# ttanida/rgrg

Measured on AMD Instinct MI355X. Metric: images/sec full 29-region report gen, 512x512 CXR, greedy max_len=128, higher is better.
Workload: dtype bf16; 1 GPU; full_model.generate() batch=32/GPU, 29 regions, greedy max_len=128, bf16 autocast: 16-bit detector, 16-bit decode GEMMs + K/V cache, hipGraph-captured decode step (BASELINE configs[2]); global_batch=32, parallelism=single GPU, weights=seeded random init (rgrg_amd.synth, profile bench), hipGraph_decode=True

## Files before the change

include/rgrg_hip.h:

```cpp
#ifndef RGRG_HIP_H_
#define RGRG_HIP_H_

#include <stdint.h>

#ifdef __cplusplus
extern "C" {
#endif

#define RGRG_OK 0
#define RGRG_EINVAL (-1)
#define RGRG_EHIP (-2)
#define RGRG_ESTATE (-3)

#define RGRG_ACT_NONE 0
#define RGRG_ACT_RELU 1
#define RGRG_ACT_GELU_NEW 2

const char* rgrg_last_error(void);
int rgrg_abi_version(void);
int rgrg_device_arch(int dev, char* buf, int buflen);

int rgrg_linear_f32(const float* A, const float* W, const float* scale, const float* shift, const float* R,
                    float* Y, int M, int N, int K, int ldy, int act, int splitk, float* ws, void* stream);
int rgrg_conv2d_nhwc_f32(const float* X, const float* W, const float* scale, const float* shift, const float* R,
// ... 30 lines not shown
typedef struct rgrg_decoder_layer_weights {
    const float *ln1_g, *ln1_b, *ln2_g, *ln2_b;
    const float *c_attn_w, *c_attn_b;
    const float *attn_proj_w, *attn_proj_b;
    const float *c_fc_w, *c_fc_b;
    const float *mlp_proj_w, *mlp_proj_b;
} rgrg_decoder_layer_weights;

typedef struct rgrg_decoder_weights {
    int n_layer, d_model, n_head, vocab;
    const float* wte;
    const float *lnf_g, *lnf_b;
    const float *fst0_w, *fst0_b, *fst2_w, *fst2_b;
    const float *ukv_w, *ukv_b;
    const rgrg_decoder_layer_weights* layers;
} rgrg_decoder_weights;

typedef struct rgrg_decoder rgrg_decoder;

int rgrg_decoder_create(const rgrg_decoder_weights* w, int max_seqs, int max_len, rgrg_decoder** out);
int rgrg_decoder_create_with_cache(const rgrg_decoder_weights* w, int max_seqs, int max_len, void* kv_cache, size_t kv_cache_bytes,
                                   rgrg_decoder** out);
size_t rgrg_decoder_kv_cache_bytes(int n_layer, int max_seqs, int max_len);
void rgrg_decoder_destroy(rgrg_decoder* d);
int rgrg_decoder_generate(rgrg_decoder* d, const float* feats, int S, int max_length, int64_t* out_ids,
                          int out_ld, int* out_len, int use_graph, void* stream);
int rgrg_decoder_sample(rgrg_decoder* d, const float* feats, int S, int max_length, float temperature, int top_k, float top_p,
                        uint64_t seed, int64_t* out_ids, int out_ld, float* out_logprobs, int* out_len, int use_graph,
                        void* stream);
int rgrg_sample_logits_f32(const float* logits, int64_t ld, int S, int V, float temperature, int top_k, float top_p,
                           uint64_t seed, int step, int row0, int* out_tok, float* out_logprob, void* stream);
int rgrg_decoder_beam_search(rgrg_decoder* d, const float* feats, int S, int num_beams, int max_length,
                             int early_stopping, float length_penalty, int num_return_sequences, int64_t* out_ids,
                             int out_ld, int* out_len, void* stream);
int rgrg_decoder_set_precision(rgrg_decoder* d, int mode);
int rgrg_decoder_set_kv_format(rgrg_decoder* d, int fmt);
int rgrg_decoder_kv_format_in_use(rgrg_decoder* d, int rows);
int rgrg_decoder_set_lm_positions(rgrg_decoder* d, const int64_t* pos, int64_t n);
int rgrg_decoder_lm_forward(rgrg_decoder* d, const float* feats, const int64_t* input_ids, const float* attention_mask,
                            int S, int T, float* logits_out, float* loss_out, void* stream);
int rgrg_decoder_lm_loss_grad(rgrg_decoder* d, const float* feats, const int64_t* input_ids, const float* attention_mask,
                              int S, int T, float loss_scale, float dropout_p, uint64_t dropout_seed, float* loss_out,
                              float* grad_ukv_w, float* grad_ukv_b, float* grad_fst0_w, float* grad_fst0_b, float* grad_fst2_w,
                              float* grad_fst2_b, void* stream);
int rgrg_decoder_time_train_gemms(rgrg_decoder* d, int S, int T, int iters, float* ms_per_step, double* flops_per_step,
                                  int* launches_per_step);
int rgrg_dropout_mask_f32(uint64_t seed, uint32_t stream_id, float p, int64_t n, int row_len, float* out, void* stream);
int rgrg_decoder_forward_cached(rgrg_decoder* d, const float* feats, const int64_t* input_ids, const int64_t* position_ids,
                                const float* attention_mask,
                                int S, int T, int past_len, float* logits_out, void* stream);
int rgrg_decoder_cache_plane(rgrg_decoder* d, int layer, int kv, void** ptr, int* max_seqs, int* slots, int* is_bf16);
int rgrg_decoder_take_id_error(rgrg_decoder* d, int* pending);
int rgrg_decoder_refresh_trainable(rgrg_decoder* d, void* stream);
int rgrg_transpose_pad_f32(const float* src, float* dst, int rows, int cols, int rows_padded, void* stream);
int rgrg_colsum_f32(const float* src, float* out, int rows, int cols, void* stream);
int rgrg_relu_backward_f32(float* d, const float* h, int64_t n, void* stream);
int rgrg_bce_with_logits_masked_backward_f32(const float* logits, const uint8_t* mask, const uint8_t* target, float pos_weight,
                                             int n, float scale, float* dlogits, int ld, void* stream);
int rgrg_adamw_step_f32(float* param, const float* grad, float* exp_avg, float* exp_avg_sq, int64_t n, float lr, float beta1,
                        float beta2, float eps, float weight_decay, int step, float grad_scale, void* stream);
int rgrg_adamw_multi_step_f32(const void* items, int n_items, float lr, float beta1, float beta2, float eps,
                              float weight_decay, int step, float grad_scale, void* stream);
int rgrg_f32_to_bf16(const float* src, uint16_t* dst, int64_t n, int fp16, void* stream);
int rgrg_bf16_to_f32(const uint16_t* src, float* dst, int64_t n, int fp16, void* stream);
int rgrg_conv2d_nhwc_bf16(const uint16_t* X16, const uint16_t* Wb, const float* shift, const uint16_t* R16, float* Y,
                          uint16_t* Y16, int B, int H, int Wd, int Cin, int Cout, int KH, int KW, int stride, int pad,
                          int act, int fp16, void* stream);
int rgrg_linear_bf16w_f32(const float* A, const uint16_t* Wb, const float* shift, const float* R, float* Y, int M,
                          int N, int K, int ldy, int act, int fp16, void* stream);
int rgrg_linear_bf16_f32(const uint16_t* A16, const uint16_t* Wb, const float* shift, const float* R, float* Y,
                         uint16_t* Y16, int M, int N, int K, int ldy, int act, int fp16, void* stream);
int rgrg_debug_linear_bf16_tile(const uint16_t* A16, const uint16_t* Wb, const float* shift, const float* R, float* Y,
                                int M, int N, int K, int ldy, int act, int tile, int lda, int ldw, int fp16, void* stream);
int rgrg_debug_linear_bf16_train(const uint16_t* A16, const uint16_t* Wb, const float* shift, const float* R, float* Y,
                                 uint16_t* Y16, uint16_t* Ypre16, const uint16_t* G16, int M, int N, int K, int ldy, int act,
                                 int tile, int fp16, void* stream);
int rgrg_debug_linear_bf16_argmax(const uint16_t* A16, const uint16_t* Wb, const float* shift, int M, int N, int K,
                                  float* cand_val, int* cand_idx, int fp16, void* stream);
int rgrg_debug_ln_fold16(const float* w, const float* gain, const float* beta, const float* bias, uint16_t* wb, float* colsum,
                         float* shift, int N, int K, int fp16, void* stream);
int rgrg_debug_linear_bf16_ln(const uint16_t* A16, const uint16_t* Wb, const float* shift, const float* R, float* Y,
                              uint16_t* Yb16, float* stats_out, const float* ln_stats, const float* ln_colsum, int M, int N,
                              int K, int ldy, int act, int fp16, void* stream);
int rgrg_debug_linear_bf16_ln_kp(const uint16_t* A16, const uint16_t* Wb, const float* shift, const float* R, float* Y,
                                 uint16_t* Y16, uint16_t* Yb16, float* stats_out, const float* ln_stats, const float* ln_colsum,
                                 int M, int N, int K, int ldy, int act, int fp16, int kp, void* stream);
int rgrg_debug_attn_decode(const float* qkv, int ld_qkv, void* kcache, void* vcache, const int* step_dev, float* out,
                           uint16_t* out16, int S, int H, int T_slots, const int* src, const float* kmask, int kv16, int fp16,
                           int ni, int frag_out, int max_workgroups, void* stream);
int rgrg_debug_attn_decode_kv8(const float* qkv, int ld_qkv, uint8_t* kcache, uint8_t* vcache, const int* step_dev, float* out,
                               uint16_t* out16, int S, int H, int T_slots, const int* src, const float* kmask, int fp16,
                               int max_workgroups, void* stream);
int rgrg_debug_attn_prefill(const float* qkv, const float* ukv, int ld_ukv, int kcol, const float* am, float* out, uint16_t* out16,
                            float* lse, int S, int H, int T, int variant, uint64_t seed, uint32_t stream_id, float p, int fp16,
                            void* stream);
int rgrg_debug_attn_backward_f32(const float* qkv, const float* ukv, int ld_ukv, int kcol, const float* am, const float* d_att,
                                 const float* att, const float* lse, float* delta, float* d_qkv, float* d_ukv, uint16_t* d_qkv16,
                                 int S, int H, int T, uint64_t seed, uint32_t stream_id, float p, int fp16, float ukv_scale,
                                 void* stream);
int rgrg_debug_attn_train16(int backward, const uint16_t* qkv16, const uint16_t* ukv16, int ld_ukv, int kcol, const float* am,
                            uint16_t* att16, float* lse, const uint16_t* d_att16, uint16_t* d_qkv16, float* d_ukv, int S, int H,
                            int T, uint64_t seed, uint32_t stream_id, float p, float ukv_scale, int fp16, void* stream);
int rgrg_box_match_f32(const float* gt, const int* gt_count, int G, const float* boxes, int64_t box_image_stride,
                       const int* box_count, int B, int N, float high, float low, int allow_low_quality, int* matched,
                       int* ws_best_per_gt, void* stream);
int rgrg_balanced_sample(const int* matched, const int64_t* gt_labels, int G, const int* box_count, const float* keys,
                         uint64_t seed, int stage, int B, int n, int batch, int max_pos, uint32_t* ws_keys, uint8_t* mask,
                         int* list, int* count, void* stream);
int rgrg_rpn_loss_sampled_f32(const float* rpn_out, int ld, int anchors_per_cell, const int* matched, const float* gt, int G,
                              const float* anchors, const uint8_t* mask, const int* list, const int* count, int B, int A,
                              int batch, float* out2, void* stream);
int rgrg_roi_add_gt_f32(const float* props, const int* counts, int P, const float* gt, const int* gt_count, int G, int B,
                        float* boxes, int* box_count, void* stream);
int rgrg_roi_gather_samples_f32(const float* boxes, const int* matched, const float* gt, const int64_t* gt_labels,
                                const int* gt_count, int G, const int* list, const int* count, int B, int N, int K, float wx,
                                float wy, float ww, float wh, float* props_s, int* offsets, int64_t* labels_flat,
                                float* reg_targets, void* stream);
int rgrg_fastrcnn_loss_f32(const float* pred, int ld, int num_classes, const int64_t* labels, const float* reg_targets, int N,
                           float* out2, void* stream);

int rgrg_decoder_copy_last_logits(rgrg_decoder* d, float* dst, int S, void* stream);
int rgrg_decoder_time_step_parts(rgrg_decoder* d, int S, int nkeys, int iters, int one_range, float* ms_gemm, float* ms_attn,
                                 double* gemm_flops, double* gemm_weight_bytes, double* kv_bytes, int* gemm_launches);
int rgrg_decoder_trace_step(rgrg_decoder* d, int S, int nkeys, int iters, float* recs, int max_recs, int* n_out);
int rgrg_decoder_attention_only(rgrg_decoder* d, int S, int nkeys, int iters, void* stream);
int rgrg_decoder_row_limit(rgrg_decoder* d);
int rgrg_debug_chain(int n, int mode, int blocks, float* us_per_kernel);

#ifdef __cplusplus
}
#endif
#endif
```

rgrg_amd/_hip.py:

```python
from __future__ import annotations

import ctypes as C
import os
from typing import Optional

from . import build as _build

c_float_p = C.c_void_p
_i, _f, _p = C.c_int, C.c_float, C.c_void_p

ACT_NONE, ACT_RELU, ACT_GELU_NEW = 0, 1, 2
ABI_VERSION = 24


class RgrgHipError(RuntimeError):
    pass


class DecoderLayerWeights(C.Structure):
    _fields_ = [(n, _p) for n in ("ln1_g", "ln1_b", "ln2_g", "ln2_b", "c_attn_w", "c_attn_b", "attn_proj_w",
                                  "attn_proj_b", "c_fc_w", "c_fc_b", "mlp_proj_w", "mlp_proj_b")]


class DecoderWeights(C.Structure):
    _fields_ = [("n_layer", _i), ("d_model", _i), ("n_head", _i), ("vocab", _i), ("wte", _p), ("lnf_g", _p),
                ("lnf_b", _p), ("fst0_w", _p), ("fst0_b", _p), ("fst2_w", _p), ("fst2_b", _p), ("ukv_w", _p),
                ("ukv_b", _p), ("layers", C.POINTER(DecoderLayerWeights))]


SIGNATURES = {
    "rgrg_last_error": (C.c_char_p, []),
    "rgrg_abi_version": (_i, []),
    "rgrg_device_arch": (_i, [_i, C.c_char_p, _i]),
    "rgrg_linear_f32": (_i, [_p, _p, _p, _p, _p, _p, _i, _i, _i, _i, _i, _i, _p, _p]),
    "rgrg_conv2d_nhwc_f32": (_i, [_p, _p, _p, _p, _p, _p, _i, _i, _i, _i, _i, _i, _i, _i, _i, _i, _i, _p, _p]),
    "rgrg_stem_conv7x7_f32": (_i, [_p, _p, _p, _p, _p, _i, _i, _i, _p]),
    "rgrg_maxpool3x3s2_nhwc_f32": (_i, [_p, _p, _i, _i, _i, _i, _p]),
    "rgrg_rpn_proposals_f32": (_i, [_p, _p, _p, _p, _p, _i, _i, _i, _i, _i, _f, _f, _f, _f, _p]),
    "rgrg_roi_align_avgpool_f32": (_i, [_p, _p, _p, _p, _p, _i, _i, _i, _i, _i, _i, _f, _p]),
    "rgrg_roi_align_avgpool_bf16maps": (_i, [_p, _p, _p, _p, _p, _i, _i, _i, _i, _i, _i, _f, _i, _p]),
    "rgrg_top1_per_class_f32": (_i, [_p, _i, _p, _p, _p, _p, _p, _p, _p, _i, _i, _i, _f, _f, _p]),
    "rgrg_select_regions_f32": (_i, [_p, _p, _f, _p, _p, _p, _i, _p]),
    "rgrg_bce_with_logits_masked_f32": (_i, [_p, _p, _p, C.c_float, _i, _p, _p]),
    "rgrg_preprocess_u8_f32": (_i, [_p, _i, _i, _i, _i, _i, C.c_float, C.c_float, _p, _p]),
    "rgrg_gather_rows_f32": (_i, [_p, _p, _p, _i, _i, _p]),
    "rgrg_decoder_create": (_i, [C.POINTER(DecoderWeights), _i, _i, C.POINTER(_p)]),
    "rgrg_decoder_create_with_cache": (_i, [C.POINTER(DecoderWeights), _i, _i, _p, C.c_size_t, C.POINTER(_p)]),
    "rgrg_decoder_kv_cache_bytes": (C.c_size_t, [_i, _i, _i]),
    "rgrg_decoder_destroy": (None, [_p]),
    "rgrg_decoder_generate": (_i, [_p, _p, _i, _i, _p, _i, C.POINTER(_i), _i, _p]),
    "rgrg_decoder_sample": (_i, [_p, _p, _i, _i, _f, _i, _f, C.c_uint64, _p, _i, _p, C.POINTER(_i), _i, _p]),
    "rgrg_sample_logits_f32": (_i, [_p, C.c_int64, _i, _i, _f, _i, _f, C.c_uint64, _i, _i, _p, _p, _p]),
    "rgrg_decoder_beam_search": (_i, [_p, _p, _i, _i, _i, _i, _f, _i, _p, _i, C.POINTER(_i), _p]),
    "rgrg_decoder_set_precision": (_i, [_p, _i]),
    "rgrg_decoder_set_kv_format": (_i, [_p, _i]),
    "rgrg_decoder_kv_format_in_use": (_i, [_p, _i]),
    "rgrg_decoder_lm_forward": (_i, [_p, _p, _p, _p, _i, _i, _p, _p, _p]),
    "rgrg_decoder_lm_loss_grad": (_i, [_p, _p, _p, _p, _i, _i, C.c_float, C.c_float, C.c_uint64, _p, _p, _p, _p, _p, _p, _p, _p]),
    "rgrg_dropout_mask_f32": (_i, [C.c_uint64, C.c_uint32, C.c_float, C.c_int64, _i, _p, _p]),
    "rgrg_decoder_refresh_trainable": (_i, [_p, _p]),
    "rgrg_decoder_take_id_error": (_i, [_p, C.POINTER(_i)]),
    "rgrg_decoder_forward_cached": (_i, [_p, _p, _p, _p, _p, _i, _i, _i, _p, _p]),
    "rgrg_decoder_cache_plane": (_i, [_p, _i, _i, C.POINTER(C.c_void_p), C.POINTER(_i), C.POINTER(_i), C.POINTER(_i)]),
    "rgrg_transpose_pad_f32": (_i, [_p, _p, _i, _i, _i, _p]),
    "rgrg_colsum_f32": (_i, [_p, _p, _i, _i, _p]),
    "rgrg_relu_backward_f32": (_i, [_p, _p, C.c_int64, _p]),
    "rgrg_bce_with_logits_masked_backward_f32": (_i, [_p, _p, _p, C.c_float, _i, C.c_float, _p, _i, _p]),
    "rgrg_adamw_step_f32": (_i, [_p, _p, _p, _p, C.c_int64, C.c_float, C.c_float, C.c_float, C.c_float, C.c_float, _i, C.c_float, _p]),
    "rgrg_adamw_multi_step_f32": (_i, [_p, _i, C.c_float, C.c_float, C.c_float, C.c_float, C.c_float, _i, C.c_float, _p]),
    "rgrg_f32_to_bf16": (_i, [_p, _p, C.c_int64, _i, _p]),
    "rgrg_bf16_to_f32": (_i, [_p, _p, C.c_int64, _i, _p]),
    "rgrg_conv2d_nhwc_bf16": (_i, [_p, _p, _p, _p, _p, _p, _i, _i, _i, _i, _i, _i, _i, _i, _i, _i, _i, _p]),
    "rgrg_linear_bf16w_f32": (_i, [_p, _p, _p, _p, _p, _i, _i, _i, _i, _i, _i, _p]),
    "rgrg_linear_bf16_f32": (_i, [_p, _p, _p, _p, _p, _p, _i, _i, _i, _i, _i, _i, _p]),
    "rgrg_debug_linear_bf16_tile": (_i, [_p, _p, _p, _p, _p, _i, _i, _i, _i, _i, _i, _i, _i, _i, _p]),
    "rgrg_debug_linear_bf16_train": (_i, [_p, _p, _p, _p, _p, _p, _p, _p, _i, _i, _i, _i, _i, _i, _i, _p]),
    "rgrg_debug_linear_bf16_argmax": (_i, [_p, _p, _p, _i, _i, _i, _p, _p, _i, _p]),
    "rgrg_debug_ln_fold16": (_i, [_p, _p, _p, _p, _p, _p, _p, _i, _i, _i, _p]),
    "rgrg_debug_linear_bf16_ln": (_i, [_p, _p, _p, _p, _p, _p, _p, _p, _p, _i, _i, _i, _i, _i, _i, _p]),
    "rgrg_debug_linear_bf16_ln_kp": (_i, [_p, _p, _p, _p, _p, _p, _p, _p, _p, _p, _i, _i, _i, _i, _i, _i, _i, _p]),
    "rgrg_debug_attn_decode": (_i, [_p, _i, _p, _p, _p, _p, _p, _i, _i, _i, _p, _p, _i, _i, _i, _i, _i, _p]),
    "rgrg_debug_attn_decode_kv8": (_i, [_p, _i, _p, _p, _p, _p, _p, _i, _i, _i, _p, _p, _i, _i, _p]),
    "rgrg_debug_attn_prefill": (_i, [_p, _p, _i, _i, _p, _p, _p, _p, _i, _i, _i, _i, C.c_uint64, C.c_uint32, _f, _i, _p]),
    "rgrg_debug_attn_backward_f32": (_i, [_p, _p, _i, _i, _p, _p, _p, _p, _p, _p, _p, _p, _i, _i, _i, C.c_uint64, C.c_uint32, _f,
                                          _i, _f, _p]),
    "rgrg_debug_attn_train16": (_i, [_i, _p, _p, _i, _i, _p, _p, _p, _p, _p, _p, _i, _i, _i, C.c_uint64, C.c_uint32, _f, _f, _i, _p]),
    "rgrg_decoder_copy_last_logits": (_i, [_p, _p, _i, _p]),
    "rgrg_box_match_f32": (_i, [_p, _p, _i, _p, C.c_int64, _p, _i, _i, _f, _f, _i, _p, _p, _p]),
    "rgrg_balanced_sample": (_i, [_p, _p, _i, _p, _p, C.c_uint64, _i, _i, _i, _i, _i, _p, _p, _p, _p, _p]),
    "rgrg_rpn_loss_sampled_f32": (_i, [_p, _i, _i, _p, _p, _i, _p, _p, _p, _p, _i, _i, _i, _p, _p]),
    "rgrg_roi_add_gt_f32": (_i, [_p, _p, _i, _p, _p, _i, _i, _p, _p, _p]),
    "rgrg_roi_gather_samples_f32": (_i, [_p, _p, _p, _p, _p, _i, _p, _p, _i, _i, _i, _f, _f, _f, _f, _p, _p, _p, _p, _p]),
    "rgrg_fastrcnn_loss_f32": (_i, [_p, _i, _i, _p, _p, _i, _p, _p]),
    "rgrg_decoder_trace_step": (_i, [_p, _i, _i, _i, _p, _i, C.POINTER(_i)]),
    "rgrg_decoder_attention_only": (_i, [_p, _i, _i, _i, _p]),
    "rgrg_decoder_row_limit": (_i, [_p]),
    "rgrg_decoder_set_lm_positions": (_i, [_p, _p, C.c_int64]),
    "rgrg_decoder_time_step_parts": (_i, [_p, _i, _i, _i, _i, C.POINTER(_f), C.POINTER(_f), C.POINTER(C.c_double),
                                          C.POINTER(C.c_double), C.POINTER(C.c_double), C.POINTER(_i)]),
    "rgrg_decoder_time_train_gemms": (_i, [_p, _i, _i, _i, C.POINTER(_f), C.POINTER(C.c_double), C.POINTER(_i)]),
    "rgrg_debug_chain": (_i, [_i, _i, _i, C.POINTER(_f)]),
}

_lib: Optional[C.CDLL] = None


def library_path() -> str:
    return _build.LIB_PATH


def load() -> C.CDLL:
    global _lib
    if _lib is not None:
        return _lib
    path = library_path()
    if _build.is_stale():
        try:
            _build.build_library()
        except Exception as e:
            if not os.path.exists(path):
                raise RgrgHipError(f"librgrg_hip.so is missing and could not be built: {e}") from e
    try:
        lib = C.CDLL(path)
    except OSError as e:
        raise RgrgHipError(f"cannot load {path}: {e} (the RGRG HIP path has no CPU fallback)") from e
    for name, (res, args) in SIGNATURES.items():
        fn = getattr(lib, name)
        fn.restype = res
        fn.argtypes = args
    got = lib.rgrg_abi_version()
    if got != ABI_VERSION:
        raise RgrgHipError(f"{path} has ABI version {got}, this package expects {ABI_VERSION}: rebuild it "
                           "(python -m rgrg_amd.build)")
    _lib = lib
    return lib


def autocast_mode() -> int:
    import torch
    if not torch.is_autocast_enabled("cuda"):
        return 0
    dt = torch.get_autocast_dtype("cuda")
    return 1 if dt == torch.bfloat16 else (2 if dt == torch.float16 else 0)


def check(rc: int, what: str = "") -> None:
    if rc != 0:
        msg = load().rgrg_last_error()
        raise RgrgHipError(f"{what} failed (code {rc}): {msg.decode() if msg else '?'}")


def ptr(t) -> Optional[int]:
    if t is None:
        return None
    assert t.is_contiguous(), "rgrg_hip expects dense tensors"
    return t.data_ptr()
```

rgrg_amd/csrc/decoder.hip:

```cpp
#include <math.h>
#include <stdlib.h>

#include <algorithm>
#include <type_traits>
#include <cmath>
#include <vector>

#include "decoder_internal.h"

namespace rgrg {

int skinny_max_rows() {
    static int v = -1;
    if (v < 0) { const char* e = getenv("RGRG_SKINNY_MAX_ROWS"); v = e ? atoi(e) : SKINNY_MAX_ROWS;
        if (v > SKINNY_MAX_ROWS) v = SKINNY_MAX_ROWS; if (v < 32) v = 32; }
    return v;
}

__global__ __launch_bounds__(256) void pack_weights_kernel(const float* __restrict__ W, float* __restrict__ P, int N,
                                                           int K, int NT) {
    const size_t total = (size_t)NT * (K / 8) * 64;
    for (size_t o = (size_t)blockIdx.x * blockDim.x + threadIdx.x; o < total; o += (size_t)gridDim.x * blockDim.x) {
        const int l = (int)(o & 63);
        const size_t t = o >> 6;
// ... 363 lines not shown
    __shared__ float pm[16], pl[16];
    __shared__ __attribute__((aligned(16))) float pacc[16][64];
    const int lane = threadIdx.x & 63, wave = threadIdx.x >> 6;
    const int s = blockIdx.x / H, hd = blockIdx.x - s * H;
    const int t = *step, nkeys = t + 2, slot = t + 1;
    const int g = lane >> 4, d4 = lane & 15;
    const float* row = qkv + (size_t)s * ld_qkv;
    const int D = H * 64;
    const int* srow = HAS_SRC ? src + (size_t)s * T : nullptr;
    constexpr int ATT_CHUNK = 16 * ATT_NI;
    const f32x4 q4 = *reinterpret_cast<const f32x4*>(row + hd * 64 + d4 * 4);
    const f32x4 k4 = *reinterpret_cast<const f32x4*>(row + D + hd * 64 + d4 * 4);
    const f32x4 v4 = *reinterpret_cast<const f32x4*>(row + 2 * D + hd * 64 + d4 * 4);
    float m = -INFINITY, l = 0.f;
    f32x4 acc = {0.f, 0.f, 0.f, 0.f};
#define ATT_CHUNK_CALL(NI_, BASE_) attn_chunk<HAS_SRC, NI_, HAS_MASK>(kc, vc, srow, s, hd, H, T, BASE_, nkeys, slot, wave, g, d4, q4, k4, v4, m, l, acc, kmask)
    if constexpr (ATT_NI == 9) {
        int base = 0;
        for (; nkeys - base > ATT_CHUNK; base += ATT_CHUNK) ATT_CHUNK_CALL(9, base);
        switch ((nkeys - base + 15) >> 4) {
            case 1: ATT_CHUNK_CALL(1, base); break;
            case 2: ATT_CHUNK_CALL(2, base); break;
            case 3: ATT_CHUNK_CALL(3, base); break;
            case 4: ATT_CHUNK_CALL(4, base); break;
            case 5: ATT_CHUNK_CALL(5, base); break;
            case 6: ATT_CHUNK_CALL(6, base); break;
            case 7: ATT_CHUNK_CALL(7, base); break;
            case 8: ATT_CHUNK_CALL(8, base); break;
            default: ATT_CHUNK_CALL(9, base); break;
        }
    } else {
        for (int base = 0; base < nkeys; base += ATT_CHUNK) ATT_CHUNK_CALL(ATT_NI, base);
    }
#undef ATT_CHUNK_CALL
    if (wave == 0 && g == 0) {
        *reinterpret_cast<f32x4*>(kc + (((size_t)s * H + hd) * T + slot) * 64 + d4 * 4) = k4;
        *reinterpret_cast<f32x4*>(vc + (((size_t)s * H + hd) * T + slot) * 64 + d4 * 4) = v4;
    }
    const int grp = wave * 4 + g;
    if (d4 == 0) { pm[grp] = m; pl[grp] = l; }
    *reinterpret_cast<f32x4*>(&pacc[grp][d4 * 4]) = acc;
    __syncthreads();
    if (threadIdx.x < 64) {
        float M = pm[0];
#pragma unroll
        for (int k = 1; k < 16; ++k) M = fmaxf(M, pm[k]);
        float L = 0.f, o = 0.f;
#pragma unroll
        for (int k = 0; k < 16; ++k) {
            const float wgt = expf(pm[k] - M);
            L += pl[k] * wgt;
            o += pacc[k][threadIdx.x] * wgt;
        }
        out[frag_out ? frag_off(s, hd * 64 + threadIdx.x, D) : (size_t)s * D + hd * 64 + threadIdx.x] = o / L;
    }
}

typedef unsigned short u16;
typedef unsigned int u32x4 __attribute__((ext_vector_type(4)));
template <bool F16>
__device__ __forceinline__ float pair_lo(unsigned u) {
    if constexpr (F16) return f16_bits_to_f32(u & 0xffffu);
    else return __uint_as_float(u << 16);
}
template <bool F16>
__device__ __forceinline__ float pair_hi(unsigned u) {
    if constexpr (F16) return f16_bits_to_f32(u >> 16);
    else return __uint_as_float(u & 0xffff0000u);
}

struct Kv16Row {
    f32x4 q0, q1, k0, k1, v0, v1;
};
template <bool F16>
__device__ __forceinline__ u32x4 kv16_pack_round(const f32x4& lo, const f32x4& hi) {
    u32x4 o;
    o[0] = to16<F16>(lo[0]) | (to16<F16>(lo[1]) << 16);
    o[1] = to16<F16>(lo[2]) | (to16<F16>(lo[3]) << 16);
    o[2] = to16<F16>(hi[0]) | (to16<F16>(hi[1]) << 16);
    o[3] = to16<F16>(hi[2]) | (to16<F16>(hi[3]) << 16);
    return o;
}

template <int NI, bool HAS_SRC, bool FIRST, bool F16>
__device__ __forceinline__ void kv16_wave_chunk(const __amdgpu_buffer_rsrc_t kc, const __amdgpu_buffer_rsrc_t vc, const int* __restrict__ srow,
                                                int s, int hd, int H, int T, int base, int nkeys, int slot, int g, int d8,
                                                Kv16Row& r, float (&q)[8], u32x4& kn16, u32x4& vn16, float& m, float& l, float (&acc)[8]) {
    int rowi[NI];
#pragma unroll
    for (int i = 0; i < NI; ++i) rowi[i] = HAS_SRC ? srow[min(base + i * 8 + g, nkeys - 1)] : s;
    u32x4 kk[NI], vv[NI];
#pragma unroll
    for (int i = 0; i < NI; ++i) {
        const int jc = min(base + i * 8 + g, nkeys - 1);
        const unsigned off = ((unsigned)((rowi[i] * H + hd) * T + jc) * 64u + (unsigned)d8 * 8u) * 2u;
        kk[i] = __builtin_bit_cast(u32x4, __builtin_amdgcn_raw_buffer_load_b128(kc, (int)off, 0, 2));
        vv[i] = __builtin_bit_cast(u32x4, __builtin_amdgcn_raw_buffer_load_b128(vc, (int)off, 0, 2));
    }
    __builtin_amdgcn_sched_barrier(0);
    if constexpr (FIRST) {
#pragma unroll
        for (int e = 0; e < 4; ++e)
            asm volatile("" : "+v"(r.q0[e]), "+v"(r.q1[e]), "+v"(r.k0[e]), "+v"(r.k1[e]), "+v"(r.v0[e]), "+v"(r.v1[e]));
#pragma unroll
        for (int e = 0; e < 4; ++e) { q[e] = r.q0[e]; q[4 + e] = r.q1[e]; }
        kn16 = kv16_pack_round<F16>(r.k0, r.k1);
        vn16 = kv16_pack_round<F16>(r.v0, r.v1);
    }
    float sc[NI];
    float cmax = -INFINITY;
#pragma unroll
    for (int i = 0; i < NI; ++i) {
        const int j = base + i * 8 + g;
        if (j == slot) { kk[i] = kn16; vv[i] = vn16; }
        float dot = 0.f;
#pragma unroll
        for (int e = 0; e < 4; ++e)
            dot += q[2 * e] * pair_lo<F16>(kk[i][e]) + q[2 * e + 1] * pair_hi<F16>(kk[i][e]);
        dot += dpp_get<0xB1, 0xf>(dot);
        dot += dpp_get<0x4E, 0xf>(dot);
        dot += dpp_get<0x141, 0xf>(dot);
        sc[i] = j < nkeys ? dot / 8.0f : -INFINITY;
        cmax = fmaxf(cmax, sc[i]);
    }
    const float m_new = fmaxf(m, cmax);
    const float scale = (m == -INFINITY) ? 0.f : expf(m - m_new);
    const bool any = m_new != -INFINITY;
    l *= scale;
#pragma unroll
    for (int e = 0; e < 8; ++e) acc[e] *= scale;
#pragma unroll
    for (int i = 0; i < NI; ++i) {
        const int j = base + i * 8 + g;
        const float pj = (j < nkeys && any) ? expf(sc[i] - m_new) : 0.f;
        l += pj;
#pragma unroll
        for (int e = 0; e < 4; ++e) {
            const unsigned u = j < nkeys ? vv[i][e] : 0u;
            acc[2 * e] += pj * pair_lo<F16>(u);
            acc[2 * e + 1] += pj * pair_hi<F16>(u);
        }
    }
    m = m_new;
}

template <bool HAS_SRC, bool F16>
__global__ __launch_bounds__(256) void attn_decode_kv16_wave_kernel(const float* __restrict__ qkv, int ld_qkv,
                                                                    u16* __restrict__ kc, u16* __restrict__ vc,
                                                                    const int* __restrict__ step, float* __restrict__ out,
                                                                    int S, int H, int T, const int* __restrict__ src,
                                                                    u16* __restrict__ out16) {
    const int lane = threadIdx.x & 63;
    const int t = *step, nkeys = t + 2, slot = t + 1;
    const int g = lane >> 3, d8 = lane & 7;
    const int D = H * 64;
    const __amdgpu_buffer_rsrc_t rk = dx_rsrc(kc), rv = dx_rsrc(vc);
    for (int item = blockIdx.x * 4 + (threadIdx.x >> 6); item < S * H; item += gridDim.x * 4) {
    const int s = item / H, hd = item - s * H;
    const float* row = qkv + (size_t)s * ld_qkv;
    const int* srow = HAS_SRC ? src + (size_t)s * T : nullptr;
    Kv16Row r;
    r.q0 = *reinterpret_cast<const f32x4*>(row + hd * 64 + d8 * 8);
    r.q1 = *reinterpret_cast<const f32x4*>(row + hd * 64 + d8 * 8 + 4);
    r.k0 = *reinterpret_cast<const f32x4*>(row + D + hd * 64 + d8 * 8);
    r.k1 = *reinterpret_cast<const f32x4*>(row + D + hd * 64 + d8 * 8 + 4);
    r.v0 = *reinterpret_cast<const f32x4*>(row + 2 * D + hd * 64 + d8 * 8);
    r.v1 = *reinterpret_cast<const f32x4*>(row + 2 * D + hd * 64 + d8 * 8 + 4);
    float m = -INFINITY, l = 0.f, acc[8], q[8];
    u32x4 kn16, vn16;
#pragma unroll
    for (int e = 0; e < 8; ++e) acc[e] = 0.f;
#define KV16_CHUNK(NI_, FIRST_, BASE_) \
    kv16_wave_chunk<NI_, HAS_SRC, FIRST_, F16>(rk, rv, srow, s, hd, H, T, BASE_, nkeys, slot, g, d8, r, q, kn16, vn16, m, l, acc)
#define KV16_TAIL(FIRST_, BASE_, REM_)                                                                   \
    switch (((REM_) + 7) >> 3) {                                                                         \
        case 1: KV16_CHUNK(1, FIRST_, BASE_); break;                                                     \
        case 2: KV16_CHUNK(2, FIRST_, BASE_); break;                                                     \
        case 3: KV16_CHUNK(3, FIRST_, BASE_); break;                                                     \
        case 4: KV16_CHUNK(4, FIRST_, BASE_); break;                                                     \
        case 5: KV16_CHUNK(5, FIRST_, BASE_); break;                                                     \
        case 6: KV16_CHUNK(6, FIRST_, BASE_); break;                                                     \
        case 7: KV16_CHUNK(7, FIRST_, BASE_); break;                                                     \
        case 8: KV16_CHUNK(8, FIRST_, BASE_); break;                                                     \
        default: KV16_CHUNK(9, FIRST_, BASE_); break;                                                    \
    }
    if (nkeys > 72) {
        KV16_CHUNK(9, true, 0);
        int base = 72;
        for (; nkeys - base > 72; base += 72) KV16_CHUNK(9, false, base);
        KV16_TAIL(false, base, nkeys - base)
    } else {
        KV16_TAIL(true, 0, nkeys)
    }
#undef KV16_TAIL
#undef KV16_CHUNK
    if (g == 0) {
        const size_t o = (((size_t)s * H + hd) * T + slot) * 64 + d8 * 8;
        *reinterpret_cast<u32x4*>(kc + o) = kn16;
        *reinterpret_cast<u32x4*>(vc + o) = vn16;
    }
    float M = fmaxf(m, dpp_get<0x128, 0xf>(m));
    M = fmaxf(M, __shfl_xor(M, 16, 64));
    M = fmaxf(M, __shfl_xor(M, 32, 64));
    const float wgt = (m == -INFINITY) ? 0.f : expf(m - M);
    l *= wgt;
    l += dpp_get<0x128, 0xf>(l);
    l += __shfl_xor(l, 16, 64);
    l += __shfl_xor(l, 32, 64);
#pragma unroll
    for (int e = 0; e < 8; ++e) {
        float o = acc[e] * wgt;
        o += dpp_get<0x128, 0xf>(o);
        o += __shfl_xor(o, 16, 64);
        o += __shfl_xor(o, 32, 64);
        acc[e] = o / l;
    }
    if (g == 0) {
        const size_t o = (size_t)s * D + hd * 64 + d8 * 8;
        if (out16) {
            u32x4 pk;
#pragma unroll
            for (int i = 0; i < 4; ++i) pk[i] = to16<F16>(acc[2 * i]) | (to16<F16>(acc[2 * i + 1]) << 16);
            *reinterpret_cast<u32x4*>(out16 + o) = pk;
        } else {
            *reinterpret_cast<f32x4*>(out + o) = f32x4{acc[0], acc[1], acc[2], acc[3]};
            *reinterpret_cast<f32x4*>(out + o + 4) = f32x4{acc[4], acc[5], acc[6], acc[7]};
        }
    }
    }
}

template <typename KV>
__global__ __launch_bounds__(256) void kv_slot0_kernel(const float* __restrict__ ukv, int ld, KV* __restrict__ kv_all,
                                                       size_t layer_stride, size_t kv_stride, int S, int H, int T,
                                                       int L, int row_mul, int f16) {
    const int D = H * 64;
    const size_t total = (size_t)L * 2 * S * D;
    for (size_t i = (size_t)blockIdx.x * blockDim.x + threadIdx.x; i < total; i += (size_t)gridDim.x * blockDim.x) {
        const int d = (int)(i % D);
        size_t r = i / D;
        const int s = (int)(r % S);
        r /= S;
        const int kv = (int)(r & 1), l = (int)(r >> 1);
        const int hd = d >> 6, e = d & 63;
        const float val = ukv[(size_t)s * ld + ((size_t)l * 2 + kv) * D + d];
        const size_t o = (size_t)l * layer_stride + (size_t)kv * kv_stride + (((size_t)s * row_mul * H + hd) * T) * 64 + e;
        if constexpr (sizeof(KV) == 1) kv_all[o] = (KV)f32_to_e4m3_bits(val);
        else if constexpr (sizeof(KV) == 2) kv_all[o] = (KV)to16_rt(val, f16);
        else kv_all[o] = val;
    }
}

constexpr int ARGMAX_U = 13;
__global__ __launch_bounds__(256) void argmax_update_kernel(const float* __restrict__ cand_val, const int* __restrict__ cand_idx,
                                                            int NT, long long* __restrict__ ids, int ld_ids,
                                                            int* __restrict__ finished, int* __restrict__ step,
                                                            int* __restrict__ done_len, int* __restrict__ sync, int S) {
    __shared__ float bv[4];
    __shared__ int bi[4];
    const int row = blockIdx.x, tid = threadIdx.x, lane = tid & 63, wave = tid >> 6;
    const int t = *step;
    const float* cv = cand_val + (size_t)row * NT;
    const int* cx = cand_idx + (size_t)row * NT;
    float v[ARGMAX_U];
    int ci[ARGMAX_U];
#pragma unroll
    for (int u = 0; u < ARGMAX_U; ++u) {
        const int i = min(tid + 256 * u, NT - 1);
        v[u] = cv[i];
        ci[u] = cx[i];
    }
    float best = -INFINITY;
    int idx = 0x7fffffff;
#pragma unroll
    for (int u = 0; u < ARGMAX_U; ++u)
        if (tid + 256 * u < NT && (v[u] > best || (v[u] == best && ci[u] < idx))) { best = v[u]; idx = ci[u]; }
    for (int i = tid + 256 * ARGMAX_U; i < NT; i += 256) {
        const float w = cv[i];
        const int wi = cx[i];
        if (w > best || (w == best && wi < idx)) { best = w; idx = wi; }
    }
    for (int o = 32; o > 0; o >>= 1) {
// ... 174 lines not shown
    return n > skinny_max_rows() ? skinny_max_rows() : n;
}
static int decode_row_limit(const rgrg_decoder* d) { return d->bf16_gemms ? skinny_max_rows16(d->w16_fused) : skinny_max_rows(); }
static bool kv_is_bf16(const rgrg_decoder* d, int rows) { return d->bf16_gemms && rows > decode_row_limit(d); }
static KvFormat kv_format(const rgrg_decoder* d, int rows) {
    if (!kv_is_bf16(d, rows)) return KV_F32;
    return d->kv8 ? KV_E4M3 : (d->f16() ? KV_F16 : KV_BF16);
}

int linear(rgrg_decoder* d, const Lin& l, const float* X, const float* R, float* Y, int M, int ldy, int act,
           bool count, const unsigned short* X16, unsigned short* Y16, const GemmLnFold* ln) {
    if (M <= skinny_max_rows() && l.packed && !l.direct) {
        SkinnyArgs a{X, l.packed, l.b, R, Y, d->part, M, l.K, l.N, l.NT, l.KS, ldy, act};
        int rc = launch_skinny_any(a, d->stream);
        if (rc) return rc;
        if (l.KS > 1) {
            const int total = M * l.N;
            hipLaunchKernelGGL(skinny_reduce_kernel, dim3((total + 255) / 256), dim3(256), 0, d->stream, a);
            RGRG_LAUNCH_CHECK();
        }
        if (count) {
            d->gemm_bytes_per_step += (size_t)l.N * l.K * sizeof(float);
            d->gemm_flops_per_step += 2.0 * M * l.N * l.K;
            d->gemm_launches_per_step += 1;
        }
        return RGRG_OK;
    }
    if (count) {
        d->gemm_flops_per_step += 2.0 * M * l.N * l.K;
        d->gemm_launches_per_step += 1;
    }
    if (d->bf16_gemms && l.wb && l.K % 256 == 0) {
        if (count) d->gemm_bytes_per_step += (size_t)l.N * l.K * 2;
        if (ln && ln->ln_colsum) {
            if (!l.wb_ln || !X16) { set_error("decoder: folded LayerNorm weights missing"); return RGRG_EINVAL; }
            GemmLnFold f = *ln;
            f.ln_colsum = l.cs16;
            f.kp = (d->kp_gemms == 1 || d->kp_gemms == 3) ? 1 : 0;
            return launch_gemm_bf16w_ex(nullptr, X16, l.wb_ln, l.c2_16, R, Y16 ? nullptr : Y, Y16, M, l.N, l.K, ldy, act, d->stream, d->f16(), &f);
        }
        if (ln && ln->Yb16 && d->sk_ws && M <= d->rows) {
            int ks = l.K >= 2048 ? d->sk_mlp : d->sk_attn;
            if (ks < 0) ks = (d->step_rows > 0 && d->step_rows <= 256) ? (l.K >= 2048 ? 4 : 2) : 1;
            if (ks > 1) {
                GemmLnFold f = *ln;
                const size_t r0 = d->xn16 ? (size_t)(reinterpret_cast<const unsigned short*>(ln->Yb16) - d->xn16) / (size_t)d->D : 0;
                const size_t tile0 = (r0 / 64) * (size_t)(l.N / 64);
                f.ksplit = ks; f.sk_ws = d->sk_ws + tile0 * 4 * 4096; f.sk_cnt = d->sk_cnt + tile0;
                return launch_gemm_bf16w_ex(nullptr, X16, l.wb, l.b, R, Y16 ? nullptr : Y, Y16, M, l.N, l.K, ldy, act, d->stream, d->f16(), &f);
            }
        }
        if (ln && ln->Yb16 && X16 && (d->kp_gemms == 1 || d->kp_gemms == 2)) {
            GemmLnFold f = *ln;
            f.kp = 1;
            return launch_gemm_bf16w_ex(nullptr, X16, l.wb, l.b, R, Y16 ? nullptr : Y, Y16, M, l.N, l.K, ldy, act, d->stream, d->f16(), &f);
        }
        return launch_gemm_bf16w_ex(X16 ? nullptr : X, X16, l.wb, l.b, R, Y16 ? nullptr : Y, Y16, M, l.N, l.K, ldy, act, d->stream, d->f16(), ln);
    }
    if (count) d->gemm_bytes_per_step += (size_t)l.N * l.K * sizeof(float);
    return launch_gemm_dense(X, l.w, l.b, R, Y, M, l.N, l.K, ldy, act, d->gemm_ws, d->gemm_ws_floats, d->stream);
}


static bool lm_head_cand_path(const rgrg_decoder* d, int S) {
    return S > decode_row_limit(d) && kv_is_bf16(d, S) && d->xn16 && d->lm_head.wb && d->lm_head.K % 256 == 0 &&
           gemm_bf16_cand_epilogue_ok(S, d->lm_head.N, d->lm_head.K);
}

struct AttnDecodeLaunch {
    const float* qkv; int ld_qkv;
    void *kc, *vc;
    size_t plane_elems;
    const int* step;
    float* out; unsigned short* out16;
    int S, H, T;
    const int* src;
    const float* kmask;
    KvFormat fmt;
    int f16;
    int ni;
    int frag_out;
    int max_wgs;
    hipStream_t st;
};
static int launch_attn_decode(const AttnDecodeLaunch& a) {
    if (a.kmask && (a.fmt != KV_F32 || a.src)) {
        set_error("decode attention: the padding mask exists only in the fp32 kernel without an ancestor table (%s)",
                  a.fmt == KV_E4M3 ? "e4m3 K/V cache" : a.fmt != KV_F32 ? "16-bit K/V cache" : "beam search");
        return RGRG_EINVAL;
    }
    if (a.fmt != KV_F32) {
        const size_t plane_bytes = a.plane_elems * (a.fmt == KV_E4M3 ? 1 : sizeof(u16));
        if ((a.H & 3) != 0) {
            set_error("decode attention: %d heads - the %s K/V cache kernel takes 4 heads per workgroup, the head count must be a multiple of 4",
                      a.H, a.fmt == KV_E4M3 ? "e4m3" : "16-bit");
            return RGRG_EINVAL;
        }
        if (plane_bytes >= ((size_t)1 << 31)) {
            set_error("decoder: the %s K/V cache plane of one layer (%zu bytes) exceeds the 2 GiB the attention kernel addresses: "
                      "lower the batch or max_length", a.fmt == KV_E4M3 ? "e4m3" : "16-bit", plane_bytes);
            return RGRG_EINVAL;
        }
        const int wgs = a.S * a.H / 4;
        const dim3 wgrid(a.max_wgs > 0 ? std::min(wgs, a.max_wgs) : wgs), wblk(256);
        if (a.fmt == KV_E4M3)
            return launch_attn_decode_kv8(a.qkv, a.ld_qkv, static_cast<uint8_t*>(a.kc), static_cast<uint8_t*>(a.vc), a.step, a.out, a.out16,
                                          a.S, a.H, a.T, a.src, a.f16, (int)wgrid.x, a.st);
#define KV16_LAUNCH(SRC_, F16_) hipLaunchKernelGGL((attn_decode_kv16_wave_kernel<SRC_, F16_>), wgrid, wblk, 0, a.st, a.qkv, a.ld_qkv, \
                                                  static_cast<u16*>(a.kc), static_cast<u16*>(a.vc), a.step, a.out, a.S, a.H, a.T, a.src, a.out16)
        if (a.src) { if (a.f16) KV16_LAUNCH(true, true); else KV16_LAUNCH(true, false); }
        else { if (a.f16) KV16_LAUNCH(false, true); else KV16_LAUNCH(false, false); }
#undef KV16_LAUNCH
    } else {
        const dim3 grid(a.S * a.H), blk(256);
        const int ni = a.ni ? a.ni : (a.S * a.H <= 4096 ? 9 : 2);
        if (ni != 9 && ni != 2) { set_error("decode attention: %d keys per group, the kernel is built for 9 and 2", ni); return RGRG_EINVAL; }
#define ATT_LAUNCH(SRC_, NI_, MASK_) hipLaunchKernelGGL((attn_decode_kernel<SRC_, NI_, MASK_>), grid, blk, 0, a.st, a.qkv, a.ld_qkv, static_cast<float*>(a.kc), \
                                                       static_cast<float*>(a.vc), a.step, a.out, a.S, a.H, a.T, a.src, a.frag_out, a.kmask)
        if (a.kmask) {
            if (ni == 9) ATT_LAUNCH(false, 9, true); else ATT_LAUNCH(false, 2, true);
        } else if (ni == 9) { if (a.src) ATT_LAUNCH(true, 9, false); else ATT_LAUNCH(false, 9, false); }
        else { if (a.src) ATT_LAUNCH(true, 2, false); else ATT_LAUNCH(false, 2, false); }
#undef ATT_LAUNCH
    }
    RGRG_LAUNCH_CHECK();
    return RGRG_OK;
}

static int launch_attention(rgrg_decoder* d, int l, int S, const int* src, unsigned short* att16, int frag_out = 0, int r0 = 0) {
    const int D = d->D;
    AttnDecodeLaunch a{};
    a.ld_qkv = 3 * D; a.step = d->step; a.S = S; a.H = d->H; a.T = d->T; a.src = src; a.kmask = d->key_mask_cur;
    a.frag_out = frag_out; a.st = d->stream; a.plane_elems = d->kv_kv_stride;
    a.fmt = kv_format(d, S);
    if (a.fmt != KV_F32) {
        static const int cap = [] { const char* e = getenv("RGRG_ATTN_WGS_PER_CU"); return e ? atoi(e) : 0; }();
        const size_t esz = a.fmt == KV_E4M3 ? 1 : sizeof(u16);
        unsigned char* kcr = reinterpret_cast<unsigned char*>(d->kv) + ((size_t)l * d->kv_layer_stride + (size_t)r0 * d->H * d->T * 64) * esz;
        a.f16 = d->f16(); a.max_wgs = cap > 0 ? cap * 256 : 0;
        a.qkv = d->qkv + (size_t)r0 * 3 * D; a.kc = kcr; a.vc = kcr + d->kv_kv_stride * esz;
        a.out = d->att + (size_t)r0 * D; a.out16 = att16;
    } else {
        float* kc = d->kv + (size_t)l * d->kv_layer_stride;
        a.qkv = d->qkv; a.kc = kc; a.vc = kc + d->kv_kv_stride; a.out = d->att;
    }
    return launch_attn_decode(a);
}

static int direct_linear(rgrg_decoder* d, const Lin& l, DirectArgs a, int mode, int M, bool count, bool cand = false) {
    if (!l.direct) { set_error("direct_linear: layer was not packed for the fused plan"); return RGRG_EINVAL; }
    if (l.lnf && mode == DX_PLAIN && !a.Xf) { set_error("direct_linear: missing operand"); return RGRG_EINVAL; }
    a.P = l.packed; a.bias = l.lnf ? l.c2 : l.b; a.c1 = l.c1;
    a.M = M; a.K = l.K; a.N = l.N; a.NT = l.NT; a.KS = l.KS;
    if (l.KS > 1) a.part_out = d->part;
    if (cand) { a.cand_val = d->cand_val; a.cand_idx = d->cand_idx; }
    const int mt = (M + PAD_ROWS - 1) / PAD_ROWS;
    const int w16 = (d->bf16_gemms && d->w16_fused && mt > 1 && l.packed16 && l.packed16_f16 == d->f16() && (!l.lnf || l.c1_16)) ? (d->f16() ? 2 : 1) : 0;
    if (w16) { a.P = reinterpret_cast<const float*>(l.packed16); if (l.lnf) a.c1 = l.c1_16; }
    const dim3 grid(l.NT, l.KS), blk(64 * SK_WAVES);
    hipStream_t st = d->stream;
    if (l.lnf && mode == DX_COMBINE4 && l.NT > 512 && mt == 1 && l.K == DK_SLICE) {
        hipLaunchKernelGGL((rgrg_lm_head_wave_f32<DX_COMBINE4>), dim3(256), blk, LMH_LDS, st, a);
    } else if (!l.lnf && mode == DX_PLAIN && l.KS == 1 && mt == 1 && l.NT <= 64 && M > 16 && !cand) {
        hipLaunchKernelGGL(rgrg_skinny_direct_half_f32, dim3(l.NT, 2), blk, 0, st, a);
    } else {
#define DX_LAUNCH(MT_, MODE_, LNF_)                                                                                          \
    do {                                                                                                                      \
        if constexpr (MT_ > 1) {                                                                                              \
            if (w16 == 1) { hipLaunchKernelGGL((rgrg_skinny_direct_f32<MT_, MODE_, LNF_, 1>), grid, blk, 0, st, a); break; }  \
            if (w16 == 2) { hipLaunchKernelGGL((rgrg_skinny_direct_f32<MT_, MODE_, LNF_, 2>), grid, blk, 0, st, a); break; }  \
        }                                                                                                                     \
        hipLaunchKernelGGL((rgrg_skinny_direct_f32<MT_, MODE_, LNF_>), grid, blk, 0, st, a);                                  \
    } while (0)
#define DX_MODES(MT_)                                                                        \
    do {                                                                                     \
        if (!l.lnf && mode == DX_PLAIN) DX_LAUNCH(MT_, DX_PLAIN, false);                     \
        else if (l.lnf && mode == DX_PLAIN) DX_LAUNCH(MT_, DX_PLAIN, true);                  \
        else if (l.lnf && mode == DX_COMBINE4) DX_LAUNCH(MT_, DX_COMBINE4, true);            \
        else if (l.lnf && mode == DX_EMBED) DX_LAUNCH(MT_, DX_EMBED, true);                  \
        else if (l.lnf && mode == DX_EMBED_TOK) DX_LAUNCH(MT_, DX_EMBED_TOK, true);          \
        else if (l.lnf && mode == DX_EMBED_TOKPOS) DX_LAUNCH(MT_, DX_EMBED_TOKPOS, true);    \
        else { set_error("direct_linear: unsupported mode %d (lnf %d)", mode, (int)l.lnf); return RGRG_EINVAL; } \
    } while (0)
        if (mt == 1) DX_MODES(1);
        else if (mt == 2) DX_MODES(2);
        else if (mt == 3) DX_MODES(3);
        else if (mt == 4) DX_MODES(4);
        else { set_error("direct_linear: %d rows exceed 4 row tiles", M); return RGRG_EINVAL; }
#undef DX_MODES
#undef DX_LAUNCH
    }
    RGRG_LAUNCH_CHECK();
    if (count) {
        d->gemm_bytes_per_step += (size_t)l.N * l.K * (w16 ? 2 : sizeof(float));
        d->gemm_flops_per_step += 2.0 * M * l.N * l.K;
        d->gemm_launches_per_step += 1;
    }
    return RGRG_OK;
}

static int enqueue_layer_gemms(rgrg_decoder* d, int l, int S, bool count, const int* tok_override, const float* cur, float* nxt,
                               int part) {
    const LayerW& w = d->layers[l];
    const int D = d->D;
    int rc;
    if (part == 0) {
        DirectArgs a{};
        a.xout = nxt; a.Y = d->qkv; a.ldy = 3 * D; a.act = RGRG_ACT_NONE;
        int mode;
        if (l == 0) {
            a.wte = d->wte; a.ids = d->ids; a.ld_ids = d->max_len; a.step = d->step; a.tok_override = tok_override;
            a.pos_override = d->pos_override_cur;
            mode = tok_override ? (d->pos_override_cur ? DX_EMBED_TOKPOS : DX_EMBED_TOK) : DX_EMBED;
        } else {
// ... 6 lines not shown
    p.Xf = d->att; p.Rf = nxt; p.Yf = nxt; p.act = RGRG_ACT_NONE;
    p.zero_acc = d->part;
    if ((rc = direct_linear(d, w.attn_proj, p, DX_PLAIN, S, count))) return rc;
    DirectArgs f{};
    f.Xf = nxt; f.Yf = d->ff; f.act = RGRG_ACT_GELU_NEW;
    if ((rc = direct_linear(d, w.c_fc, f, DX_PLAIN, S, count))) return rc;
    DirectArgs m{};
    m.Xf = d->ff; m.act = RGRG_ACT_NONE;
    return direct_linear(d, w.mlp_proj, m, DX_PLAIN, S, count);
}

static int enqueue_step_fused(rgrg_decoder* d, int S, bool count, const int* tok_override, const int* src, bool beam) {
    if (count) { d->gemm_bytes_per_step = 0; d->gemm_flops_per_step = 0.0; d->gemm_launches_per_step = 0; }
    hipStream_t st = d->stream;
    int rc;
    float* cur = d->x;
    float* nxt = d->x2;
    for (int l = 0; l < d->n_layer; ++l) {
        if ((rc = enqueue_layer_gemms(d, l, S, count, tok_override, cur, nxt, 0))) return rc;
        if ((rc = launch_attention(d, l, S, src, nullptr, 1))) return rc;
        if ((rc = enqueue_layer_gemms(d, l, S, count, tok_override, cur, nxt, 1))) return rc;
        float* tmp = cur; cur = nxt; nxt = tmp;
    }
    DirectArgs h{};
    h.Xf = cur; h.part = d->part; h.Y = d->logits; h.ldy = d->ld_logits; h.act = RGRG_ACT_NONE;
    if ((rc = direct_linear(d, d->lm_head, h, DX_COMBINE4, S, count, !beam))) return rc;
    if (beam) return RGRG_OK;
    hipLaunchKernelGGL(argmax_update_kernel, dim3(S), dim3(256), 0, st, d->cand_val, d->cand_idx, d->lm_head.NT, d->ids,
                       d->max_len, d->finished, d->step, d->done_len, d->sync, S);
    RGRG_LAUNCH_CHECK();
    return RGRG_OK;
}

static int range_bounds(int S, int want, int (&bounds)[MAX_CHAINS + 1]) {
    int nr = want < 1 ? 1 : (want > MAX_CHAINS ? MAX_CHAINS : want);
    const int tiles = (S + 63) / 64;
    for (; nr > 1; --nr) {
        int least = S;
        for (int i = 0; i <= nr; ++i) {
            bounds[i] = std::min(S, ((tiles * i + nr - 1) / nr) * 64);
            if (i) least = std::min(least, bounds[i] - bounds[i - 1]);
        }
        if (least > SKINNY_MAX_ROWS) break;
    }
    if (nr <= 1) { nr = 1; bounds[0] = 0; bounds[1] = S; }
    return nr;
}
template <class F>
static int run_row_ranges(rgrg_decoder* d, int S, int chains, F&& fn) {
    int bounds[MAX_CHAINS + 1];
    const int nr = range_bounds(S, chains < 0 ? -chains : chains, bounds);
    if (nr <= 1) return fn(0, S);
    if (chains > 0) {
        RGRG_HIP(hipEventRecord(d->ev_fork, d->stream));
        for (int i = 1; i < nr; ++i) RGRG_HIP(hipStreamWaitEvent(d->streams_x[i - 1], d->ev_fork, 0));
    }
    int rc = RGRG_OK;
    for (int i = 0; i < nr && !rc; ++i) {
        if (bounds[i + 1] <= bounds[i]) continue;
        if (chains > 0 && i > 0) std::swap(d->stream, d->streams_x[i - 1]);
        rc = fn(bounds[i], bounds[i + 1] - bounds[i]);
        if (chains > 0 && i > 0) std::swap(d->stream, d->streams_x[i - 1]);
    }
    if (chains > 0)
        for (int i = 1; i < nr; ++i) {
            RGRG_HIP(hipEventRecord(d->ev_join[i - 1], d->streams_x[i - 1]));
            RGRG_HIP(hipStreamWaitEvent(d->stream, d->ev_join[i - 1], 0));
        }
    return rc;
}
static int step_chains(const rgrg_decoder* d, int S, bool greedy, bool fold) {
    return (greedy && fold && S >= 512 && (d->chains < 0 || d->streams_x[0])) ? d->chains : 1;
}

static int trace_mark(rgrg_decoder* d, int r0, int tag) {
    if (!d->trace) return RGRG_OK;
    hipEvent_t e;
    RGRG_HIP(hipEventCreate(&e));
    RGRG_HIP(hipEventRecord(e, d->stream));
    d->trace->push_back({e, r0, tag});
    return RGRG_OK;
}

int enqueue_step(rgrg_decoder* d, int S, bool count, const int* tok_override, const int* src, bool beam) {
    if (S <= decode_row_limit(d)) return enqueue_step_fused(d, S, count, tok_override, src, beam);
    if (count) { d->gemm_bytes_per_step = 0; d->gemm_flops_per_step = 0.0; d->gemm_launches_per_step = 0; }
    d->step_rows = S;
    hipStream_t st = d->stream;
    const int D = d->D;
    int rc;
    unsigned short* xn16 = (kv_is_bf16(d, S) && d->xn16) ? d->xn16 : nullptr;
    unsigned short* att16 = xn16 ? d->att16 : nullptr;
    unsigned short* ff16 = xn16 ? d->ff16 : nullptr;
    const bool fold = xn16 && d->ln_fold && d->ln_stat && d->layers[0].c_attn.wb_ln && D == 1024;
    static const float cons_tag = 0.f;
    GemmLnFold prod{}, cons{};
    prod.Yb16 = xn16; prod.stats_out = d->ln_stat;
    cons.ln_stats = d->ln_stat; cons.ln_colsum = &cons_tag;
    const GemmLnFold* pf = fold ? &prod : nullptr;
    const GemmLnFold* cf = fold ? &cons : nullptr;
    auto run_rows = [&](int r0, int rows) -> int {
        hipStream_t rs = d->stream;
        const size_t o = (size_t)r0 * D;
        float* x = d->x + o; float* xn = d->xn + o;
        unsigned short* xn16r = xn16 ? xn16 + o : nullptr;
        unsigned short* att16r = att16 ? att16 + o : nullptr;
        unsigned short* ff16r = ff16 ? ff16 + 4 * o : nullptr;
        float* statr = d->ln_stat ? d->ln_stat + (size_t)r0 * 32 : nullptr;
        GemmLnFold prod_r = prod, cons_r = cons;
        prod_r.Yb16 = xn16r; prod_r.stats_out = statr; cons_r.ln_stats = statr;
        const GemmLnFold* pfr = fold ? &prod_r : nullptr;
        const GemmLnFold* cfr = fold ? &cons_r : nullptr;
        hipLaunchKernelGGL(embed_ln_kernel, dim3(rows), dim3(256), 0, rs, d->wte, d->ids + (size_t)r0 * d->max_len, d->max_len, d->step,
                           d->layers[0].ln1_g, d->layers[0].ln1_b, x, xn, D, tok_override ? tok_override + r0 : nullptr, xn16r, d->f16(),
                           d->pos_override_cur ? d->pos_override_cur + r0 : nullptr, fold ? statr : (float*)nullptr);
        RGRG_LAUNCH_CHECK();
        int rc2;
        if ((rc2 = trace_mark(d, r0, 1000))) return rc2;
        for (int l = 0; l < d->n_layer; ++l) {
            const LayerW& w = d->layers[l];
            const float* ng = (l + 1 < d->n_layer) ? d->layers[l + 1].ln1_g : d->lnf_g;
            const float* nb = (l + 1 < d->n_layer) ? d->layers[l + 1].ln1_b : d->lnf_b;
            if ((rc2 = linear(d, w.c_attn, xn, nullptr, d->qkv + 3 * o, rows, 3 * D, RGRG_ACT_NONE, count, xn16r, nullptr, cfr))) return rc2;
            if ((rc2 = trace_mark(d, r0, l * 8 + 0))) return rc2;
            if ((rc2 = launch_attention(d, l, rows, src ? src + (size_t)r0 * d->T : nullptr, att16r, 0, r0))) return rc2;
            if ((rc2 = trace_mark(d, r0, l * 8 + 1))) return rc2;
            if ((rc2 = linear(d, w.attn_proj, d->att + o, x, x, rows, D, RGRG_ACT_NONE, count, att16r, nullptr, pfr))) return rc2;
            if ((rc2 = trace_mark(d, r0, l * 8 + 2))) return rc2;
            if (!fold) {
                if ((rc2 = launch_ln_rows(x, w.ln2_g, w.ln2_b, xn, D, xn16r, d->f16(), rows, rs))) return rc2;
            }
            if ((rc2 = linear(d, w.c_fc, xn, nullptr, d->ff + 4 * o, rows, 4 * D, RGRG_ACT_GELU_NEW, count, xn16r, ff16r, cfr))) return rc2;
            if ((rc2 = trace_mark(d, r0, l * 8 + 3))) return rc2;
            if ((rc2 = linear(d, w.mlp_proj, d->ff + 4 * o, x, x, rows, D, RGRG_ACT_NONE, count, ff16r, nullptr, pfr))) return rc2;
            if ((rc2 = trace_mark(d, r0, l * 8 + 4))) return rc2;
            if (!fold || l + 1 == d->n_layer) {
                if ((rc2 = launch_ln_rows(x, ng, nb, xn, D, xn16r, d->f16(), rows, rs))) return rc2;
                if ((rc2 = trace_mark(d, r0, 1001))) return rc2;
            }
        }
        return RGRG_OK;
    };
    if ((rc = run_row_ranges(d, S, step_chains(d, S, !beam && !tok_override && !src, fold), run_rows))) return rc;
    if (!beam && xn16 && lm_head_cand_path(d, S)) {
        GemmLnFold ce{};
        ce.cand_val = d->cand_val; ce.cand_idx = d->cand_idx;
        if ((rc = linear(d, d->lm_head, d->xn, nullptr, nullptr, S, d->ld_logits, RGRG_ACT_NONE, count, xn16, nullptr, &ce))) return rc;
        if ((rc = trace_mark(d, 0, 1002))) return rc;
        hipLaunchKernelGGL(argmax_update_kernel, dim3(S), dim3(256), 0, st, d->cand_val, d->cand_idx, (d->lm_head.N + 255) / 256, d->ids,
                           d->max_len, d->finished, d->step, d->done_len, d->sync, S);
        RGRG_LAUNCH_CHECK();
        return trace_mark(d, 0, 1003);
    }
    if ((rc = linear(d, d->lm_head, d->xn, nullptr, d->logits, S, d->ld_logits, RGRG_ACT_NONE, count, xn16))) return rc;
    if (beam) return RGRG_OK;
    const int cand_nt = (d->V + 31) / 32;
    hipLaunchKernelGGL(logits_candidates_kernel, dim3(4, S), dim3(256), 0, st, d->logits, d->ld_logits, d->V,
                       cand_nt, d->cand_val, d->cand_idx);
    RGRG_LAUNCH_CHECK();
    hipLaunchKernelGGL(argmax_update_kernel, dim3(S), dim3(256), 0, st, d->cand_val, d->cand_idx, cand_nt, d->ids,
                       d->max_len, d->finished, d->step, d->done_len, d->sync, S);
    RGRG_LAUNCH_CHECK();
    return RGRG_OK;
}

int enqueue_prefill(rgrg_decoder* d, const float* feats, int S, int row_mul) {
    hipStream_t st = d->stream;
    const int D = d->D;
    hipLaunchKernelGGL(decode_reset_kernel, dim3(64), dim3(256), 0, st, d->ids, d->max_len, d->finished, d->step,
                       d->done_len, d->sync, S, d->max_len);
    RGRG_LAUNCH_CHECK();
    RGRG_HIP(hipMemcpyAsync(d->feats, feats, (size_t)S * D * sizeof(float), hipMemcpyDeviceToDevice, st));
    int rc;
    if ((rc = linear(d, d->fst0, d->feats, nullptr, d->h1, S, D, RGRG_ACT_RELU, false))) return rc;
    if ((rc = linear(d, d->fst2, d->h1, nullptr, d->img, S, D, RGRG_ACT_NONE, false))) return rc;
    if ((rc = linear(d, d->ukv, d->img, nullptr, d->ukv_out, S, d->ld_ukv, RGRG_ACT_NONE, false))) return rc;
    const KvFormat fmt = kv_format(d, S * row_mul);
    if (fmt == KV_E4M3)
        hipLaunchKernelGGL(kv_slot0_kernel<uint8_t>, dim3(1024), dim3(256), 0, st, d->ukv_out, d->ld_ukv,
                           reinterpret_cast<uint8_t*>(d->kv), d->kv_layer_stride, d->kv_kv_stride, S, d->H, d->T, d->n_layer, row_mul, 0);
    else if (fmt != KV_F32)
        hipLaunchKernelGGL(kv_slot0_kernel<u16>, dim3(1024), dim3(256), 0, st, d->ukv_out, d->ld_ukv,
                           reinterpret_cast<u16*>(d->kv), d->kv_layer_stride, d->kv_kv_stride, S, d->H, d->T, d->n_layer, row_mul, d->f16());
    else
        hipLaunchKernelGGL(kv_slot0_kernel<float>, dim3(1024), dim3(256), 0, st, d->ukv_out, d->ld_ukv, d->kv,
                           d->kv_layer_stride, d->kv_kv_stride, S, d->H, d->T, d->n_layer, row_mul, 0);
    RGRG_LAUNCH_CHECK();
    return RGRG_OK;
}

}

using namespace rgrg;

extern "C" size_t rgrg_decoder_kv_cache_bytes(int n_layer, int max_seqs, int max_len) {
    return (size_t)n_layer * 2 * (size_t)max_seqs * 16 * (size_t)(max_len + 1) * 64 * sizeof(float);
}

extern "C" int rgrg_decoder_create(const rgrg_decoder_weights* w, int max_seqs, int max_len, rgrg_decoder** out) {
    return rgrg_decoder_create_with_cache(w, max_seqs, max_len, nullptr, 0, out);
}

extern "C" int rgrg_decoder_create_with_cache(const rgrg_decoder_weights* w, int max_seqs, int max_len, void* kv_cache, size_t kv_cache_bytes,
                                              rgrg_decoder** out) {
    RGRG_CHECK_ARG(w && out && max_seqs > 0 && max_seqs < 65536 && max_len >= 2 && max_len <= 1024);
    RGRG_CHECK_ARG(w->d_model == 1024 && w->n_head == 16 && w->n_layer > 0 && w->vocab > 0 && w->layers);
    int rc = init_gemm_attrs();
    if (rc) return rc;
    if ((rc = init_skinny_attrs())) return rc;
    RGRG_HIP(hipDeviceSynchronize());
    rgrg_decoder* d = new rgrg_decoder();
    d->n_layer = w->n_layer; d->D = w->d_model; d->H = w->n_head; d->V = w->vocab;
    d->max_seqs = max_seqs; d->max_len = max_len; d->T = max_len + 1;
    d->rows = ((max_seqs + PAD_ROWS - 1) / PAD_ROWS) * PAD_ROWS;
    d->wte = w->wte; d->lnf_g = w->lnf_g; d->lnf_b = w->lnf_b;
    const int D = d->D;
#define TRY(x) do { rc = (x); if (rc) { rgrg_decoder_destroy(d); return rc; } } while (0)
    if (hipStreamCreateWithFlags(&d->stream, hipStreamNonBlocking) != hipSuccess ||
        hipEventCreateWithFlags(&d->ev_in, hipEventDisableTiming) != hipSuccess) {
        set_error("decoder: stream/event creation failed");
        delete d;
        return RGRG_EHIP;
    }
    if (const char* e = getenv("RGRG_GEMM_KP")) d->kp_gemms = atoi(e);
    if (const char* e = getenv("RGRG_W16_FUSED")) d->w16_fused = atoi(e) != 0;
    if (const char* e = getenv("RGRG_DECODE_CHAINS")) {
        const int v = atoi(e);
        d->chains = (v >= -MAX_CHAINS && v <= MAX_CHAINS && v != 0 && v != -1) ? v : 1;
    }
    if (d->chains > 1) {
        bool ok = hipEventCreateWithFlags(&d->ev_fork, hipEventDisableTiming) == hipSuccess;
        for (int i = 0; ok && i < d->chains - 1; ++i)
            ok = hipStreamCreateWithFlags(&d->streams_x[i], hipStreamNonBlocking) == hipSuccess &&
                 hipEventCreateWithFlags(&d->ev_join[i], hipEventDisableTiming) == hipSuccess;
        if (!ok) {
            set_error("decoder: stream/event creation failed");
            rgrg_decoder_destroy(d);
            return RGRG_EHIP;
        }
    }
    if (hipHostMalloc((void**)&d->h_id_error, sizeof(int), 0) == hipSuccess) *d->h_id_error = 0;
    if (hipHostMalloc((void**)&d->h_done, 3 * sizeof(int), 0) != hipSuccess ||
        hipEventCreateWithFlags(&d->ev_poll[0], hipEventDisableTiming) != hipSuccess ||
        hipEventCreateWithFlags(&d->ev_poll[1], hipEventDisableTiming) != hipSuccess) {
        set_error("decoder: hipHostMalloc failed");
        delete d;
        return RGRG_EHIP;
    }
    TRY(make_lin(d, d->fst0, w->fst0_w, w->fst0_b, D, D, true));
    TRY(make_lin(d, d->fst2, w->fst2_w, w->fst2_b, D, D, true));
    TRY(make_lin(d, d->ukv, w->ukv_w, w->ukv_b, w->n_layer * 2 * D, D, true));
    TRY(make_lin(d, d->lm_head, w->wte, nullptr, w->vocab, D, true, true, w->lnf_g, w->lnf_b));
    d->layers.resize(w->n_layer);
    for (int l = 0; l < w->n_layer; ++l) {
        const rgrg_decoder_layer_weights& s = w->layers[l];
        LayerW& t = d->layers[l];
        t.ln1_g = s.ln1_g; t.ln1_b = s.ln1_b; t.ln2_g = s.ln2_g; t.ln2_b = s.ln2_b;
        TRY(make_lin(d, t.c_attn, s.c_attn_w, s.c_attn_b, 3 * D, D, true, true, s.ln1_g, s.ln1_b));
        TRY(make_lin(d, t.attn_proj, s.attn_proj_w, s.attn_proj_b, D, D, true, true));
        TRY(make_lin(d, t.c_fc, s.c_fc_w, s.c_fc_b, 4 * D, D, true, true, s.ln2_g, s.ln2_b));
        TRY(make_lin(d, t.mlp_proj, s.mlp_proj_w, s.mlp_proj_b, D, 4 * D, true, true));
    }
    const size_t R = d->rows;
    d->ld_logits = d->lm_head.NT * d->lm_head.ntile;
    d->ld_ukv = d->ukv.N;
    TRY(dmalloc(d, (void**)&d->feats, R * D * 4, true));
    TRY(dmalloc(d, (void**)&d->h1, R * D * 4, true));
    TRY(dmalloc(d, (void**)&d->img, R * D * 4, true));
    TRY(dmalloc(d, (void**)&d->ukv_out, R * d->ld_ukv * 4, true));
    TRY(dmalloc(d, (void**)&d->x, R * D * 4, true));
    TRY(dmalloc(d, (void**)&d->x2, R * D * 4, true));
    TRY(dmalloc(d, (void**)&d->xn, R * D * 4, true));
    TRY(dmalloc(d, (void**)&d->qkv, R * 3 * D * 4, true));
    TRY(dmalloc(d, (void**)&d->att, R * D * 4, true));
    TRY(dmalloc(d, (void**)&d->ff, R * 4 * D * 4, true));
    TRY(dmalloc(d, (void**)&d->logits, R * d->ld_logits * 4, true));
    TRY(dmalloc(d, (void**)&d->part, (size_t)(SKINNY_MAX_ROWS / PAD_ROWS) * 8 * PAD_ROWS * D * 4, true));
    d->kv_kv_stride = (size_t)d->max_seqs * d->H * d->T * 64;
    d->kv_layer_stride = 2 * d->kv_kv_stride;
    if (kv_cache) {
        if (kv_cache_bytes < (size_t)d->n_layer * d->kv_layer_stride * 4) {
            set_error("decoder: the caller's K/V cache holds %zu bytes, %zu needed", kv_cache_bytes, (size_t)d->n_layer * d->kv_layer_stride * 4);
            rgrg_decoder_destroy(d);
            return RGRG_EINVAL;
        }
        d->kv = static_cast<float*>(kv_cache);
    } else {
        TRY(dmalloc(d, (void**)&d->kv, (size_t)d->n_layer * d->kv_layer_stride * 4, true));
    }
    TRY(dmalloc(d, (void**)&d->ids, R * max_len * sizeof(long long), true));
    TRY(dmalloc(d, (void**)&d->next, R * 4, true));
    TRY(dmalloc(d, (void**)&d->finished, R * 4, true));
    TRY(dmalloc(d, (void**)&d->step, 4, true));
    TRY(dmalloc(d, (void**)&d->done_len, 4, true));
    TRY(dmalloc(d, (void**)&d->sync, 64, true));
    TRY(dmalloc(d, (void**)&d->id_error, 8, true));
    TRY(dmalloc(d, (void**)&d->cand_val, R * d->lm_head.NT * 4, true));
    TRY(dmalloc(d, (void**)&d->cand_idx, R * d->lm_head.NT * 4, true));
    TRY(dmalloc(d, (void**)&d->src_a, R * d->T * 4, true));
    TRY(dmalloc(d, (void**)&d->src_b, R * d->T * 4, true));
    TRY(dmalloc(d, (void**)&d->beam_tok, R * 4, true));
    TRY(dmalloc(d, (void**)&d->row_pos, R * 4, true));
    TRY(dmalloc(d, (void**)&d->beam_parent, R * 4, true));
    TRY(dmalloc(d, (void**)&d->beam_scores, R * 4, true));
    TRY(dmalloc(d, (void**)&d->row_max, R * 4, true));
    TRY(dmalloc(d, (void**)&d->row_logsum, R * 4, true));
    TRY(dmalloc(d, (void**)&d->top_val, R * BEAM_K * 4, true));
    TRY(dmalloc(d, (void**)&d->top_tok, R * BEAM_K * 4, true));
// ... 156 lines not shown
    d->logits_stale_rows = 0;
    d->logits_valid = false;
    if (past_len == 0 && feats && (rc = enqueue_prefill(d, feats, S))) return rc;
    if (attention_mask) {
        if (!d->key_mask && (rc = dmalloc(d, (void**)&d->key_mask, (size_t)d->rows * d->T * sizeof(float), true))) return rc;
        hipLaunchKernelGGL(key_mask_kernel, dim3((S * d->T + 255) / 256), dim3(256), 0, st, attention_mask, past_len + T, S, d->T, d->key_mask);
        RGRG_LAUNCH_CHECK();
    }
    for (int j = 0; j < T; ++j) {
        hipLaunchKernelGGL(forward_cached_tokens_kernel, dim3((S + 255) / 256), dim3(256), 0, st,
                           reinterpret_cast<const long long*>(input_ids), reinterpret_cast<const long long*>(position_ids), T, j, S, d->V,
                           d->beam_tok, d->row_pos, d->step, past_len + j);
        RGRG_LAUNCH_CHECK();
        d->pos_override_cur = position_ids ? d->row_pos : nullptr;
        d->key_mask_cur = attention_mask ? d->key_mask : nullptr;
        rc = enqueue_step(d, S, false, d->beam_tok, nullptr, true);
        d->pos_override_cur = nullptr;
        d->key_mask_cur = nullptr;
        if (rc) return rc;
        RGRG_HIP(hipMemcpy2DAsync(logits_out + (size_t)j * d->V, (size_t)T * d->V * sizeof(float), d->logits,
                                  (size_t)d->ld_logits * sizeof(float), (size_t)d->V * sizeof(float), S, hipMemcpyDeviceToDevice, st));
    }
    hipLaunchKernelGGL(set_int_kernel, dim3(1), dim3(64), 0, st, d->step, past_len + T);
    RGRG_LAUNCH_CHECK();
    RGRG_HIP(hipEventRecord(d->ev_in, st));
    RGRG_HIP(hipStreamWaitEvent(caller, d->ev_in, 0));
    d->logits_valid = true;
    return RGRG_OK;
}

extern "C" int rgrg_decoder_cache_plane(rgrg_decoder* d, int layer, int kv, void** ptr, int* max_seqs, int* slots, int* is_bf16) {
    RGRG_CHECK_ARG(d && ptr && layer >= 0 && layer < d->n_layer && (kv == 0 || kv == 1));
    *ptr = d->kv + (size_t)layer * d->kv_layer_stride + (size_t)kv * d->kv_kv_stride;
    if (max_seqs) *max_seqs = d->max_seqs;
    if (slots) *slots = d->T;
    if (is_bf16) *is_bf16 = 0;
    return RGRG_OK;
}

extern "C" int rgrg_decoder_take_id_error(rgrg_decoder* d, int* pending) {
    RGRG_CHECK_ARG(d && pending);
    RGRG_HIP(hipStreamSynchronize(d->stream));
    *pending = (d->h_id_error && *d->h_id_error) ? 1 : 0;
    if (*pending) {
        *d->h_id_error = 0;
        RGRG_HIP(hipMemsetAsync(d->id_error, 0, 2 * sizeof(int), d->stream));
    }
    return RGRG_OK;
}

extern "C" int rgrg_decoder_refresh_trainable(rgrg_decoder* d, void* stream) {
    RGRG_CHECK_ARG(d);
    hipStream_t caller = as_stream(stream), st = d->stream;
    RGRG_HIP(hipEventRecord(d->ev_in, caller));
    RGRG_HIP(hipStreamWaitEvent(st, d->ev_in, 0));
    Lin* ls[] = {&d->fst0, &d->fst2, &d->ukv};
    for (Lin* l : ls) {
        if (l->packed) {
            hipLaunchKernelGGL(pack_weights_kernel, dim3(2048), dim3(256), 0, st, l->w, l->packed, l->N, l->K, l->NT);
            RGRG_LAUNCH_CHECK();
        }
        if (l->wT) {
            int rc = launch_transpose_pad(l->w, l->wT, l->N, l->K, pad256(l->N), st);
            if (rc) return rc;
        }
    }
    RGRG_HIP(hipEventRecord(d->ev_in, st));
    RGRG_HIP(hipStreamWaitEvent(caller, d->ev_in, 0));
    return RGRG_OK;
}

extern "C" int rgrg_debug_attn_decode(const float* qkv, int ld_qkv, void* kcache, void* vcache, const int* step_dev, float* out,
                                      uint16_t* out16, int S, int H, int T_slots, const int* src, const float* kmask, int kv16,
                                      int fp16, int ni, int frag_out, int max_workgroups, void* stream) {
    RGRG_CHECK_ARG(qkv && kcache && vcache && step_dev && S > 0 && H > 0 && T_slots >= 2 && ld_qkv >= 3 * H * 64);
    RGRG_CHECK_ARG(out || (kv16 && out16));
    RGRG_CHECK_ARG(kv16 || (!out16 && max_workgroups == 0));
    RGRG_CHECK_ARG(!kv16 || (ni == 0 && frag_out == 0));
    AttnDecodeLaunch a{};
    a.qkv = qkv; a.ld_qkv = ld_qkv; a.kc = kcache; a.vc = vcache; a.plane_elems = (size_t)S * H * T_slots * 64;
    a.step = step_dev; a.out = out; a.out16 = out16; a.S = S; a.H = H; a.T = T_slots; a.src = src; a.kmask = kmask;
    a.fmt = kv16 ? (fp16 ? KV_F16 : KV_BF16) : KV_F32; a.f16 = fp16 ? 1 : 0; a.ni = ni; a.frag_out = frag_out ? 1 : 0; a.max_wgs = max_workgroups;
    a.st = as_stream(stream);
    return launch_attn_decode(a);
}

extern "C" int rgrg_debug_attn_decode_kv8(const float* qkv, int ld_qkv, uint8_t* kcache, uint8_t* vcache, const int* step_dev, float* out,
                                          uint16_t* out16, int S, int H, int T_slots, const int* src, const float* kmask, int fp16,
                                          int max_workgroups, void* stream) {
    RGRG_CHECK_ARG(qkv && kcache && vcache && step_dev && S > 0 && H > 0 && T_slots >= 2 && ld_qkv >= 3 * H * 64 && (out || out16));
    AttnDecodeLaunch a{};
    a.qkv = qkv; a.ld_qkv = ld_qkv; a.kc = kcache; a.vc = vcache; a.plane_elems = (size_t)S * H * T_slots * 64;
    a.step = step_dev; a.out = out; a.out16 = out16; a.S = S; a.H = H; a.T = T_slots; a.src = src; a.kmask = kmask;
    a.fmt = KV_E4M3; a.f16 = fp16 ? 1 : 0; a.max_wgs = max_workgroups; a.st = as_stream(stream);
    return launch_attn_decode(a);
}

extern "C" int rgrg_debug_ln_fold16(const float* w, const float* gain, const float* beta, const float* bias, uint16_t* wb,
                                    float* colsum, float* shift, int N, int K, int fp16, void* stream) {
    RGRG_CHECK_ARG(w && gain && beta && wb && colsum && shift && N > 0 && K > 0);
    hipLaunchKernelGGL(ln_fold16_kernel, dim3((N + 3) / 4), dim3(256), 0, as_stream(stream), w, gain, beta, bias, wb, colsum, shift, N, K,
                       fp16 ? 1 : 0);
    RGRG_LAUNCH_CHECK();
    return RGRG_OK;
}

static int set_precision_impl(rgrg_decoder* d, int mode);
extern "C" int rgrg_decoder_set_precision(rgrg_decoder* d, int mode) {
    RGRG_CHECK_ARG(d && mode >= 0 && mode <= 2);
    if (mode == d->bf16_gemms) return RGRG_OK;
    const int prev = d->bf16_gemms;
    const int rc = set_precision_impl(d, mode);
    if (rc) {
        auto stale = [](Lin& l) { l.wb_f16 = -1; l.wb_ln_f16 = -1; l.wTb_f16 = -1; };
        stale(d->lm_head); stale(d->ukv); stale(d->fst2);
        for (auto& w : d->layers) { stale(w.c_attn); stale(w.attn_proj); stale(w.c_fc); stale(w.mlp_proj); }
        d->bf16_gemms = 0;
        (void)prev;
        for (auto& g : d->graphs) (void)hipGraphExecDestroy(g.exec);
        d->graphs.clear();
    }
    return rc;
}
static int set_precision_impl(rgrg_decoder* d, int mode) {
    d->logits_valid = false;
    const int prev = d->bf16_gemms;
    d->bf16_gemms = mode;
    if (mode) {
        int rc = init_gemm_bf16_attrs();
        if (rc) { d->bf16_gemms = prev; return rc; }
        auto mk = [&](Lin& l) -> int {
            if (l.wb && l.wb_f16 == d->f16()) return RGRG_OK;
            if (!l.wb) {
                int r = dmalloc(d, &l.wb, (size_t)l.N * l.K * 2, false);
                if (r) return r;
            }
            l.wb_f16 = d->f16();
            return convert_f32_to_bf16(l.w, l.wb, (size_t)l.N * l.K, d->stream, d->f16());
        };
        int rc2;
        RGRG_HIP(hipStreamSynchronize(d->stream));
        if (!d->xn16) {
            if ((rc2 = dmalloc(d, (void**)&d->xn16, (size_t)d->rows * d->D * 2, false)) ||
                (rc2 = dmalloc(d, (void**)&d->att16, (size_t)d->rows * d->D * 2, false)) ||
                (rc2 = dmalloc(d, (void**)&d->ff16, (size_t)d->rows * 4 * d->D * 2, false)))
                return rc2;
        }
        if ((rc2 = mk(d->lm_head))) return rc2;
        for (auto& w : d->layers) {
            if ((rc2 = mk(w.c_attn)) || (rc2 = mk(w.attn_proj)) || (rc2 = mk(w.c_fc)) || (rc2 = mk(w.mlp_proj))) return rc2;
        }
        if (d->w16_fused && d->rows > PAD_ROWS) {
            auto mk16 = [&](Lin& l) -> int {
                if (!l.direct || !l.packed || (l.packed16 && l.packed16_f16 == d->f16())) return RGRG_OK;
                const size_t n = (size_t)l.NT * 16 * l.K;
                int r;
                if (!l.packed16 && (r = dmalloc(d, &l.packed16, n * 2, false))) return r;
                if (l.lnf && !l.c1_16 && (r = dmalloc(d, (void**)&l.c1_16, (size_t)l.NT * 16 * sizeof(float), false))) return r;
                if ((r = convert_f32_to_bf16(l.packed, l.packed16, n, d->stream, d->f16()))) return r;
                if (l.lnf)
                    hipLaunchKernelGGL(packed16_colsum_kernel, dim3(l.NT), dim3(64), 0, d->stream, (const unsigned short*)l.packed16, l.c1_16, l.NT * 16, l.K,
                                       d->f16());
                l.packed16_f16 = d->f16();
                return RGRG_OK;
            };
            if ((rc2 = mk16(d->lm_head))) return rc2;
// ... 7 lines not shown
                if (l.wb_ln && l.wb_ln_f16 == d->f16()) return RGRG_OK;
                int r;
                if (!l.wb_ln && ((r = dmalloc(d, &l.wb_ln, (size_t)l.N * l.K * 2, false)) ||
                                 (r = dmalloc(d, (void**)&l.cs16, (size_t)l.N * sizeof(float), false)) ||
                                 (r = dmalloc(d, (void**)&l.c2_16, (size_t)l.N * sizeof(float), false))))
                    return r;
                l.wb_ln_f16 = d->f16();
                hipLaunchKernelGGL(ln_fold16_kernel, dim3((l.N + 3) / 4), dim3(256), 0, d->stream, l.w, g, be, l.b,
                                   reinterpret_cast<unsigned short*>(l.wb_ln), l.cs16, l.c2_16, l.N, l.K, d->f16());
                RGRG_LAUNCH_CHECK();
                return RGRG_OK;
            };
            if (!d->ln_stat && (rc2 = dmalloc(d, (void**)&d->ln_stat, (size_t)d->rows * 32 * sizeof(float), true))) return rc2;
            if (!d->sk_ws) {
                const size_t tiles = (size_t)((d->rows + 63) / 64) * (d->D / 64);
                const size_t small_rows = (size_t)((std::min(d->rows, 256) + 127) / 128) * 2;
                const size_t slabs = std::max(tiles * 4, small_rows * (size_t)(4 * d->D / 64) * 2), tickets = std::max(tiles, small_rows * (size_t)(4 * d->D / 64));
                if ((rc2 = dmalloc(d, (void**)&d->sk_ws, slabs * 4096 * sizeof(float), false)) ||
                    (rc2 = dmalloc(d, (void**)&d->sk_cnt, tickets * sizeof(unsigned), true)))
                    return rc2;
                const char* e1 = getenv("RGRG_SK_MLP");
                const char* e2 = getenv("RGRG_SK_ATTN");
                d->sk_mlp = e1 ? atoi(e1) : -1;
                d->sk_attn = e2 ? atoi(e2) : -1;
                if (d->sk_mlp == 0) d->sk_mlp = 1;
                if (d->sk_attn == 0) d->sk_attn = 1;
                if (d->sk_mlp > 4) d->sk_mlp = 4;
                if (d->sk_attn > 4) d->sk_attn = 4;
            }
            for (auto& w : d->layers) {
                if ((rc2 = mkln(w.c_attn, w.ln1_g, w.ln1_b)) || (rc2 = mkln(w.c_fc, w.ln2_g, w.ln2_b))) return rc2;
            }
        }
        RGRG_HIP(hipStreamSynchronize(d->stream));
    }
    for (auto& g : d->graphs) (void)hipGraphExecDestroy(g.exec);
    d->graphs.clear();
    return RGRG_OK;
}

extern "C" int rgrg_decoder_set_kv_format(rgrg_decoder* d, int fmt) {
    RGRG_CHECK_ARG(d && (fmt == 0 || fmt == 1));
    if (fmt == d->kv8) return RGRG_OK;
    RGRG_HIP(hipStreamSynchronize(d->stream));
    d->kv8 = fmt;
    d->logits_valid = false;
    for (auto& g : d->graphs) (void)hipGraphExecDestroy(g.exec);
    d->graphs.clear();
    return RGRG_OK;
}

extern "C" int rgrg_decoder_kv_format_in_use(rgrg_decoder* d, int rows) { return d && rows > 0 ? (int)kv_format(d, rows) : -1; }

extern "C" int rgrg_decoder_copy_last_logits(rgrg_decoder* d, float* dst, int S, void* stream) {
    RGRG_CHECK_ARG(d && dst && S > 0 && S <= d->max_seqs);
    if (!d->logits_valid) {
        set_error("decoder: no logits of a completed step to copy - the last generate / beam / cached call failed, or a timing hook or a "
                  "precision change has reused the decoder's work space since");
        return RGRG_EINVAL;
    }
    if (d->logits_stale_rows > 0) {
        const int rows = d->logits_stale_rows;
        RGRG_CHECK_ARG(S <= rows);
        int rc = linear(d, d->lm_head, d->xn, nullptr, d->logits, rows, d->ld_logits, RGRG_ACT_NONE, false, d->xn16);
        if (rc) return rc;
        RGRG_HIP(hipStreamSynchronize(d->stream));
        d->logits_stale_rows = 0;
    }
    RGRG_HIP(hipMemcpy2DAsync(dst, (size_t)d->V * 4, d->logits, (size_t)d->ld_logits * 4, (size_t)d->V * 4, S,
                              hipMemcpyDeviceToDevice, as_stream(stream)));
    RGRG_HIP(hipStreamSynchronize(as_stream(stream)));
    return RGRG_OK;
}

extern "C" int rgrg_decoder_row_limit(rgrg_decoder* d) { return d ? decode_row_limit(d) : -1; }

extern "C" int rgrg_decoder_attention_only(rgrg_decoder* d, int S, int nkeys, int iters, void* stream) {
    RGRG_CHECK_ARG(d && S > decode_row_limit(d) && S <= d->rows && nkeys >= 2 && nkeys <= d->T && iters > 0);
    hipStream_t keep = d->stream;
    d->stream = as_stream(stream);
    hipLaunchKernelGGL(set_int_kernel, dim3(1), dim3(64), 0, d->stream, d->step, nkeys - 2);
    int rc = RGRG_OK;
    unsigned short* att16 = (kv_is_bf16(d, S) && d->xn16) ? d->att16 : nullptr;
    for (int it = 0; it < iters && !rc; ++it)
        for (int l = 0; l < d->n_layer && !rc; ++l) rc = launch_attention(d, l, S, nullptr, att16, 0, 0);
    hipLaunchKernelGGL(set_int_kernel, dim3(1), dim3(64), 0, d->stream, d->step, 0);
    d->stream = keep;
    return rc;
}

extern "C" int rgrg_decoder_trace_step(rgrg_decoder* d, int S, int nkeys, int iters, float* recs, int max_recs, int* n_out) {
    RGRG_CHECK_ARG(d && S > decode_row_limit(d) && S <= d->rows && nkeys >= 2 && nkeys <= d->T && recs && n_out && iters >= 0);
    d->logits_valid = false;
    std::vector<rgrg_decoder::TraceMark> marks;
    hipEvent_t base;
    RGRG_HIP(hipEventCreate(&base));
    int rc = RGRG_OK;
    for (int it = 0; it <= iters && !rc; ++it) {
        hipLaunchKernelGGL(set_int_kernel, dim3(1), dim3(64), 0, d->stream, d->step, nkeys - 2);
        if (it == iters) { d->trace = &marks; RGRG_HIP(hipEventRecord(base, d->stream)); }
        rc = enqueue_step(d, S, false);
    }
    d->trace = nullptr;
    (void)hipStreamSynchronize(d->stream);
    int n = 0;
    for (auto& m : marks) {
        float ms = 0.f;
        if (!rc && n < max_recs && hipEventElapsedTime(&ms, base, m.ev) == hipSuccess) {
            recs[3 * n] = (float)m.r0; recs[3 * n + 1] = (float)m.tag; recs[3 * n + 2] = ms;
            ++n;
        }
        (void)hipEventDestroy(m.ev);
    }
    (void)hipEventDestroy(base);
    hipLaunchKernelGGL(set_int_kernel, dim3(1), dim3(64), 0, d->stream, d->step, 0);
    (void)hipStreamSynchronize(d->stream);
    *n_out = n;
    return rc;
}

extern "C" int rgrg_decoder_time_step_parts(rgrg_decoder* d, int S, int nkeys, int iters, int one_range, float* ms_gemm, float* ms_attn,
                                            double* gemm_flops, double* gemm_weight_bytes, double* kv_bytes,
                                            int* gemm_launches) {
    RGRG_CHECK_ARG(d && S > 0 && S <= d->max_seqs && nkeys >= 2 && nkeys <= d->T && iters > 0 && ms_gemm && ms_attn);
    d->logits_valid = false;
    const int keep_chains = d->chains;
    if (one_range) d->chains = 1;
    struct Restore { rgrg_decoder* d; int c; ~Restore() { d->chains = c; } } restore{d, keep_chains};
    hipEvent_t e0, e1;
    RGRG_HIP(hipEventCreate(&e0));
    RGRG_HIP(hipEventCreate(&e1));
    const int D = d->D;
    const bool fused = d->lm_head.direct && S <= decode_row_limit(d);
    const bool bf = kv_is_bf16(d, S);
    d->step_rows = S;
    unsigned short* xn16 = (bf && d->xn16) ? d->xn16 : nullptr;
    unsigned short* att16 = xn16 ? d->att16 : nullptr;
    unsigned short* ff16 = xn16 ? d->ff16 : nullptr;
    const bool fold = xn16 && d->ln_fold && d->ln_stat && d->layers[0].c_attn.wb_ln && D == 1024;
    static const float cons_tag = 0.f;
    GemmLnFold prod{}, cons{};
    prod.Yb16 = xn16; prod.stats_out = d->ln_stat;
    cons.ln_stats = d->ln_stat; cons.ln_colsum = &cons_tag;
    const GemmLnFold* pf = fold ? &prod : nullptr;
    const GemmLnFold* cf = fold ? &cons : nullptr;
    int rc = RGRG_OK;
    float tg = 0.f, ta = 0.f;
    d->gemm_bytes_per_step = 0; d->gemm_flops_per_step = 0.0; d->gemm_launches_per_step = 0;
    for (int it = -1; it < iters && !rc; ++it) {
        const bool c = it == -1;
        if (it == 0) RGRG_HIP(hipEventRecord(e0, d->stream));
        rc = run_row_ranges(d, S, fused ? 1 : step_chains(d, S, true, fold), [&](int r0, int rows) -> int {
            const size_t o = (size_t)r0 * D;
            GemmLnFold prod_r = prod, cons_r = cons;
            prod_r.Yb16 = xn16 ? xn16 + o : nullptr;
            prod_r.stats_out = d->ln_stat ? d->ln_stat + (size_t)r0 * 32 : nullptr;
            cons_r.ln_stats = prod_r.stats_out;
            const GemmLnFold* pfr = pf ? &prod_r : nullptr;
            const GemmLnFold* cfr = cf ? &cons_r : nullptr;
            unsigned short* xn16r = xn16 ? xn16 + o : nullptr;
            unsigned short* att16r = att16 ? att16 + o : nullptr;
            unsigned short* ff16r = ff16 ? ff16 + 4 * o : nullptr;
            int rc2 = RGRG_OK;
            for (int l = 0; l < d->n_layer && !rc2; ++l) {
                const LayerW& w = d->layers[l];
                if (fused) {
                    if ((rc2 = enqueue_layer_gemms(d, l ? l : 1, S, c, nullptr, d->x, d->x2, 0))) break;
                    if ((rc2 = enqueue_layer_gemms(d, l, S, c, nullptr, d->x, d->x2, 1))) break;
                    continue;
                }
                if ((rc2 = linear(d, w.c_attn, d->xn + o, nullptr, d->qkv + 3 * o, rows, 3 * D, RGRG_ACT_NONE, c, xn16r, nullptr, cfr))) break;
                if ((rc2 = linear(d, w.attn_proj, d->att + o, d->x + o, d->h1 + o, rows, D, RGRG_ACT_NONE, c, att16r, nullptr, pfr))) break;
                if ((rc2 = linear(d, w.c_fc, d->xn + o, nullptr, d->ff + 4 * o, rows, 4 * D, RGRG_ACT_GELU_NEW, c, xn16r, ff16r, cfr))) break;
                if ((rc2 = linear(d, w.mlp_proj, d->ff + 4 * o, d->x + o, d->h1 + o, rows, D, RGRG_ACT_NONE, c, ff16r, nullptr, pfr))) break;
            }
            return rc2;
        });
        if (!rc && fused) {
            DirectArgs h{};
            h.Xf = d->x; h.part = d->part; h.Y = d->logits; h.ldy = d->ld_logits; h.act = RGRG_ACT_NONE;
            rc = direct_linear(d, d->lm_head, h, DX_COMBINE4, S, c, true);
        } else if (!rc) {
            if (xn16 && lm_head_cand_path(d, S)) {
                GemmLnFold ce{};
                ce.cand_val = d->cand_val; ce.cand_idx = d->cand_idx;
                rc = linear(d, d->lm_head, d->xn, nullptr, nullptr, S, d->ld_logits, RGRG_ACT_NONE, c, xn16, nullptr, &ce);
            } else {
                rc = linear(d, d->lm_head, d->xn, nullptr, d->logits, S, d->ld_logits, RGRG_ACT_NONE, c, xn16);
            }
        }
    }
    if (!rc) {
        RGRG_HIP(hipEventRecord(e1, d->stream));
        RGRG_HIP(hipEventSynchronize(e1));
        RGRG_HIP(hipEventElapsedTime(&tg, e0, e1));
        hipLaunchKernelGGL(set_int_kernel, dim3(1), dim3(64), 0, d->stream, d->step, nkeys - 2);
        for (int it = -1; it < iters && !rc; ++it) {
            if (it == 0) RGRG_HIP(hipEventRecord(e0, d->stream));
            rc = run_row_ranges(d, S, fused ? 1 : step_chains(d, S, true, fold), [&](int r0, int rows) -> int {
                int rc2 = RGRG_OK;
                for (int l = 0; l < d->n_layer && !rc2; ++l)
                    rc2 = launch_attention(d, l, rows, nullptr, att16 ? att16 + (size_t)r0 * D : nullptr, fused ? 1 : 0, r0);
                return rc2;
            });
        }
        if (!rc) {
            RGRG_HIP(hipEventRecord(e1, d->stream));
            RGRG_HIP(hipEventSynchronize(e1));
            RGRG_HIP(hipEventElapsedTime(&ta, e0, e1));
        }
        hipLaunchKernelGGL(set_int_kernel, dim3(1), dim3(64), 0, d->stream, d->step, 0);
        (void)hipStreamSynchronize(d->stream);
    }
    (void)hipEventDestroy(e0);
    (void)hipEventDestroy(e1);
    if (rc) return rc;
    *ms_gemm = tg;
    *ms_attn = ta;
    if (gemm_flops) *gemm_flops = d->gemm_flops_per_step;
    if (gemm_weight_bytes) *gemm_weight_bytes = (double)d->gemm_bytes_per_step;
    if (kv_bytes) *kv_bytes = (double)d->n_layer * 2.0 * S * D * nkeys * (kv_format(d, S) == KV_E4M3 ? 1.0 : bf ? 2.0 : 4.0);
    if (gemm_launches) *gemm_launches = d->gemm_launches_per_step;
    return RGRG_OK;
}
```

rgrg_amd/csrc/decoder_internal.h:

```cpp
#pragma once
#include <vector>

#include "internal.h"

namespace rgrg {

constexpr int MAX_CHAINS = 4;
constexpr int PAD_ROWS = 32;
constexpr int SKINNY_MAX_ROWS = 128;
constexpr int BOS_ID = 50256, EOS_ID = 50256, PAD_ID = 50256;
constexpr int BEAM_K = 32;
enum KvFormat { KV_F32 = 0, KV_BF16 = 1, KV_F16 = 2, KV_E4M3 = 3 };
constexpr int KV8_CHUNK_KEYS = 144;

struct StepBook {
    long long* ids;
    int ld_ids;
    int *finished, *step, *done_len, *sync;
    int S;
};
#ifdef __HIPCC__
__device__ __forceinline__ int record_step_token(const StepBook& bk, int row, int t, int tok, bool* was_finished = nullptr) {
    int fin = bk.finished[row];
    if (was_finished) *was_finished = fin != 0;
// ... 52 lines not shown
    rgrg::Lin fst0, fst2, ukv, lm_head;
    std::vector<rgrg::LayerW> layers;
    float *feats, *h1, *img, *ukv_out, *x, *x2, *xn, *qkv, *att, *ff, *logits, *part, *kv, *cand_val, *gemm_ws;
    size_t gemm_ws_floats;
    int* cand_idx;
    size_t kv_layer_stride, kv_kv_stride;
    int ld_logits, ld_ukv;
    long long* ids;
    int *next, *finished, *step, *done_len, *sync;
    int *src_a, *src_b, *beam_tok, *beam_parent, *cand_tok, *cand_beam, *top_tok;
    float *beam_scores, *row_max, *row_logsum, *top_val, *cand_score;
    float *wide_val = nullptr, *wide_score = nullptr;
    int* wide_tok = nullptr;
    size_t wide_cap = 0;
    void* sample_prm = nullptr;
    float* sample_lp = nullptr;
    int* h_done;
    hipEvent_t ev_poll[2] = {nullptr, nullptr};
    int* id_error = nullptr;
    int* h_id_error = nullptr;
    hipStream_t stream;
    hipEvent_t ev_in;
    std::vector<rgrg::GraphEntry> graphs;
    std::vector<void*> allocs;
    size_t gemm_bytes_per_step = 0;
    double gemm_flops_per_step = 0.0;
    struct TfWork {
        float *x = nullptr, *xn = nullptr, *qkv = nullptr, *att = nullptr, *ff = nullptr, *logits = nullptr, *ws = nullptr,
              *row_loss = nullptr;
        int* row_valid = nullptr;
        size_t rows = 0, ws_floats = 0;
        const long long* pos = nullptr;
        int pos_rows = 1;
        void free() {
            float** fs[] = {&x, &xn, &qkv, &att, &ff, &logits, &ws, &row_loss};
            for (float** f : fs) { if (*f) (void)hipFree(*f); *f = nullptr; }
            if (row_valid) (void)hipFree(row_valid);
            row_valid = nullptr;
            rows = 0;
            ws_floats = 0;
        }
    } tf;
    struct TrWork {
        float *xs = nullptr, *qkv = nullptr, *ffpre = nullptr, *ff = nullptr, *dx = nullptr, *dbig = nullptr, *dxn = nullptr,
              *logits = nullptr, *dukv = nullptr, *t1 = nullptr, *t2 = nullptr, *dimg = nullptr, *dh1 = nullptr, *row_lse = nullptr,
              *att = nullptr, *lse = nullptr, *delta = nullptr;
        int* count = nullptr;
        size_t rows = 0, seqs = 0;
        unsigned short *xn16 = nullptr, *att16 = nullptr, *ff16 = nullptr, *ffpre16 = nullptr, *dx16 = nullptr, *dff16 = nullptr,
                       *dqkv16 = nullptr, *dl16 = nullptr;
        unsigned short *qkv16 = nullptr, *datt16 = nullptr, *ukv16 = nullptr;
        bool a16 = false;
        bool h16 = false;
        size_t chunk = 0;
        bool seen_a16 = false, seen_a32 = false, seen_h16 = false, seen_h32 = false, seen_h16_a32 = false;
        bool have_wT = false;
        void* a16_scratch = nullptr;
        size_t a16_bytes = 0;
        void free() {
            float** fs[] = {&xs, &qkv, &ffpre, &ff, &dx, &dbig, &dxn, &logits, &dukv, &t1, &t2, &dimg, &dh1, &row_lse, &att, &lse, &delta};
            for (float** f : fs) { if (*f) (void)hipFree(*f); *f = nullptr; }
            if (count) (void)hipFree(count);
            count = nullptr;
            unsigned short** hs[] = {&xn16, &att16, &ff16, &ffpre16, &dx16, &dff16, &dqkv16, &dl16, &qkv16, &datt16, &ukv16};
            for (unsigned short** h : hs) { if (*h) (void)hipFree(*h); *h = nullptr; }
            rows = seqs = 0;
            chunk = 0;
        }
    } tr;
    int bf16_gemms = 0;
    int f16() const { return bf16_gemms == 2 ? 1 : 0; }
    unsigned short *xn16 = nullptr, *att16 = nullptr, *ff16 = nullptr;
    float* sk_ws = nullptr;
    unsigned* sk_cnt = nullptr;
    int sk_attn = 0, sk_mlp = 0;
    int step_rows = 0;
    float* ln_stat = nullptr;
    bool ln_fold = true;
    float* key_mask = nullptr;
    const float* key_mask_cur = nullptr;
    struct TraceMark { hipEvent_t ev; int r0; int tag; };
    std::vector<TraceMark>* trace = nullptr;
    bool w16_fused = true;
    int kp_gemms = 2;
    int gemm_launches_per_step = 0;
    const int* pos_override_cur = nullptr;
    int* row_pos = nullptr;
    int logits_stale_rows = 0;
    bool logits_valid = false;
    hipStream_t streams_x[rgrg::MAX_CHAINS - 1] = {};
    hipEvent_t ev_fork = nullptr, ev_join[rgrg::MAX_CHAINS - 1] = {};
    int kv8 = 0;
    int chains = 4;
};

namespace rgrg {

inline int pad256(int n) { return (n + 255) / 256 * 256; }

int dmalloc(rgrg_decoder* d, void** p, size_t bytes, bool zero);
int skinny_max_rows();
int linear(rgrg_decoder* d, const Lin& l, const float* X, const float* R, float* Y, int M, int ldy, int act,
           bool count, const unsigned short* X16 = nullptr, unsigned short* Y16 = nullptr, const GemmLnFold* ln = nullptr);
int launch_ln_rows(const float* x, const float* g, const float* b, float* xn, int D, unsigned short* xn16, int f16, int rows,
                   hipStream_t st);
int enqueue_step(rgrg_decoder* d, int S, bool count, const int* tok_override = nullptr, const int* src = nullptr,
                 bool beam = false);
int enqueue_prefill(rgrg_decoder* d, const float* feats, int S, int row_mul = 1);
int decode_begin(rgrg_decoder* d, void* stream);
int launch_attn_decode_kv8(const float* qkv, int ld_qkv, uint8_t* kc, uint8_t* vc, const int* step, float* out, unsigned short* out16,
                           int S, int H, int T, const int* src, int f16, int workgroups, hipStream_t st);
int run_decode_loop(rgrg_decoder* d, const float* feats, int S, int limit, int graph_key, int (*step)(rgrg_decoder*, int, bool),
                    int use_graph, int64_t* out_ids, int out_ld, float* out_logprobs, int* out_len);

}
```

rgrg_amd/csrc/gemm_bf16.hip:

```cpp
#include "internal.h"

namespace rgrg {

typedef short bf16x8 __attribute__((ext_vector_type(8)));
typedef short bf16x4 __attribute__((ext_vector_type(4)));
typedef unsigned short u16;

struct GemmBf16Params {
    const float* A;
    const u16* A16;
    const u16* Wb;
    const float* shift;
    const float* R;
    float* Y;
    u16* Y16;
    int M, N, K, ldy, act;
    int lda = 0, ldw = 0;
    int cH = 0, cW = 0, cCin = 0, cKH = 0, cKW = 0, cStride = 1, cPad = 0, cOH = 0, cOW = 0;
    const u16* R16 = nullptr;
    int f16 = 0;
    u16* Yb16 = nullptr;
    float* stats_out = nullptr;
    const float* ln_stats = nullptr;
    const float* ln_colsum = nullptr;
    u16* Ypre16 = nullptr;
    const u16* G16 = nullptr;
    int gm = 0;
    int ksplit = 0;
    float* sk_ws = nullptr;
    unsigned* sk_cnt = nullptr;
    float* cand_val = nullptr;
    int* cand_idx = nullptr;
    int dbg = 0;
};

constexpr float LN_EPS16 = 1e-5f;

constexpr int BK16 = 64;
constexpr int LDB = (BK16 * 2 + 16) / 2;

template <bool F16>
__device__ __forceinline__ f32x16 mfma16(const bf16x8& a, const bf16x8& b, const f32x16& c) {
    if constexpr (F16) return __builtin_amdgcn_mfma_f32_32x32x16_f16(__builtin_bit_cast(f16x8, a), __builtin_bit_cast(f16x8, b), c, 0, 0, 0);
    else return __builtin_amdgcn_mfma_f32_32x32x16_bf16(a, b, c, 0, 0, 0);
}

template <int BM, int BN, int THREADS, bool A16, bool F16>
__global__ __launch_bounds__(THREADS) void gemm_bf16w_kernel(const GemmBf16Params p, const int mtiles, const int ntiles) {
    constexpr int WAVES = THREADS / 64, WN = WAVES / 2;
    constexpr int TM = BM / 2, TN = BN / WN;
    constexpr int MI = TM / 32, NI = TN / 32;
    constexpr int AL = BM * 8 / THREADS, BL = BN * 8 / THREADS;
    constexpr int RSTEP = THREADS / 8;
    constexpr int NS = 4;
    extern __shared__ __attribute__((aligned(16))) u16 smem16[];
    u16* As = smem16;
    u16* Bs = smem16 + 2 * BM * LDB;
    const int tid = threadIdx.x, lane = tid & 63, wave = tid >> 6;
    const int wm = wave / WN, wn = wave % WN;
    const int total = mtiles * ntiles;
    int t = blockIdx.x;
    if ((total & 7) == 0) t = (t & 7) * (total >> 3) + (t >> 3);
    const int tn = t / mtiles, tm = t - tn * mtiles;
    const int m0 = tm * BM, n0 = tn * BN;
    const int kchunk = tid & 7, lrow = tid >> 3;
    const int nk = p.K / BK16;

    const float* aptr[AL];
    const u16* aptr16[AL];
    const u16* bptr[BL];
#pragma unroll
    for (int i = 0; i < AL; ++i) {
        const int m = min(m0 + lrow + RSTEP * i, p.M - 1);
        aptr[i] = A16 ? nullptr : p.A + (size_t)m * p.K + kchunk * 4;
        aptr16[i] = A16 ? p.A16 + (size_t)m * p.K + kchunk * 8 : nullptr;
    }
#pragma unroll
    for (int i = 0; i < BL; ++i) {
        const int n = min(n0 + lrow + RSTEP * i, p.N - 1);
        bptr[i] = p.Wb + (size_t)n * p.K + kchunk * 8;
    }

    f32x4 ra[NS][AL][2];
    bf16x8 ra16[NS][AL];
    bf16x8 rb[NS][BL];
#define RGRG_LOAD_TILE(S, KT)                                                                    \
    {                                                                                            \
        const int koff = (KT) * BK16;                                                            \
        _Pragma("unroll") for (int i = 0; i < AL; ++i) {                                         \
            if constexpr (A16) {                                                                 \
                ra16[S][i] = *reinterpret_cast<const bf16x8*>(aptr16[i] + koff);                 \
            } else {                                                                             \
                ra[S][i][0] = *reinterpret_cast<const f32x4*>(aptr[i] + koff);                   \
                ra[S][i][1] = *reinterpret_cast<const f32x4*>(aptr[i] + koff + 32);              \
            }                                                                                    \
        }                                                                                        \
        _Pragma("unroll") for (int i = 0; i < BL; ++i)                                           \
            rb[S][i] = *reinterpret_cast<const bf16x8*>(bptr[i] + koff);                         \
    }
#define RGRG_STORE_ITEM(S, BUF, I)                                                               \
    {                                                                                            \
        if ((I) < AL) {                                                                          \
            constexpr int i = (I) < AL ? (I) : 0;                                                \
            if constexpr (A16) {                                                                 \
                *reinterpret_cast<bf16x8*>(&As[((BUF) * BM + lrow + RSTEP * i) * LDB + kchunk * 8]) = ra16[S][i]; \
            } else {                                                                             \
                bf16x4 lo, hi;                                                                   \
// ... 96 lines not shown
        }
}

typedef __attribute__((address_space(3))) void* lds_ptr_t;

__device__ __forceinline__ __amdgpu_buffer_rsrc_t bf16_rsrc(const void* p) {
    return __builtin_amdgcn_make_buffer_rsrc(const_cast<void*>(p), 0, 0x7fffffff, 0x00020000);
}

template <int N>
__device__ __forceinline__ void wait_vmcnt() {
    static_assert(N >= 0 && N < 64, "vmcnt is a 6-bit field");
    asm volatile("s_waitcnt vmcnt(%0)" ::"n"(N) : "memory");
}

__device__ __forceinline__ float gelu_new_fast(float x) {
    const float u = x * (1.0f + 0.044715f * x * x);
    return x * __builtin_amdgcn_rcpf(1.0f + __builtin_amdgcn_exp2f(-2.302208198f * u));
}
__device__ __forceinline__ float gelu_new_grad_fast(float x) {
    const float x2 = x * x;
    const float u = x * (1.0f + 0.044715f * x2);
    const float sg = __builtin_amdgcn_rcpf(1.0f + __builtin_amdgcn_exp2f(-2.302208198f * u));
    return sg + 2.0f * x * sg * (1.0f - sg) * 0.7978845608028654f * (1.0f + 0.134145f * x2);
}
__device__ __forceinline__ float apply_act_fast(float v, int act) {
    if (act == RGRG_ACT_RELU) return v > 0.f ? v : 0.f;
    if (act == RGRG_ACT_GELU_NEW) return gelu_new_fast(v);
    return v;
}

template <int BM, int LA, int LB, int TAG>
__device__ __forceinline__ void glds_issue(const u16* abase, const u16* wbase, unsigned char* sb,
                                           const int (&va)[LA], const int (&vb)[LB], int koff_a, int koff_w) {
    const __amdgpu_buffer_rsrc_t ra = bf16_rsrc(abase), rb = bf16_rsrc(wbase);
#pragma unroll
    for (int j = 0; j < LA; ++j)
        __builtin_amdgcn_raw_ptr_buffer_load_lds(ra, (lds_ptr_t)(sb + j * 4096), 16, va[j], koff_a, 0, 0);
#pragma unroll
    for (int j = 0; j < LB; ++j)
        __builtin_amdgcn_raw_ptr_buffer_load_lds(rb, (lds_ptr_t)(sb + BM * 128 + j * 4096), 16, vb[j], koff_w, 0, 0);
}

template <int MI, int NI, bool F16>
__device__ __forceinline__ void glds_compute(const unsigned char* sa, const unsigned char* sw, const int (&foff)[4],
                                             f32x16 (&acc)[MI][NI]) {
    bf16x8 a[2][MI], b[2][NI];
#pragma unroll
    for (int mi = 0; mi < MI; ++mi) a[0][mi] = *reinterpret_cast<const bf16x8*>(sa + mi * 4096 + foff[0]);
#pragma unroll
    for (int ni = 0; ni < NI; ++ni) b[0][ni] = *reinterpret_cast<const bf16x8*>(sw + ni * 4096 + foff[0]);
#pragma unroll
    for (int ks = 0; ks < 4; ++ks) {
        if (ks + 1 < 4) {
#pragma unroll
            for (int mi = 0; mi < MI; ++mi) a[(ks + 1) & 1][mi] = *reinterpret_cast<const bf16x8*>(sa + mi * 4096 + foff[ks + 1]);
#pragma unroll
            for (int ni = 0; ni < NI; ++ni) b[(ks + 1) & 1][ni] = *reinterpret_cast<const bf16x8*>(sw + ni * 4096 + foff[ks + 1]);
        }
#pragma unroll
        for (int mi = 0; mi < MI; ++mi)
#pragma unroll
            for (int ni = 0; ni < NI; ++ni)
                acc[mi][ni] = mfma16<F16>(a[ks & 1][mi], b[ks & 1][ni], acc[mi][ni]);
    }
    __builtin_amdgcn_sched_group_barrier(0x100, 2 * (MI + NI), 0);
    __builtin_amdgcn_sched_group_barrier(0x008, MI * NI, 0);
    __builtin_amdgcn_sched_group_barrier(0x100, MI + NI, 0);
    __builtin_amdgcn_sched_group_barrier(0x008, MI * NI, 0);
    __builtin_amdgcn_sched_group_barrier(0x100, MI + NI, 0);
    __builtin_amdgcn_sched_group_barrier(0x008, MI * NI, 0);
    __builtin_amdgcn_sched_group_barrier(0x008, MI * NI, 0);
}

template <int BM, int BN, int NST, bool CONV, bool F16, int LNF>
__global__ __launch_bounds__(256) void gemm_bf16_glds_kernel(const GemmBf16Params p, const int mtiles, const int ntiles) {
    constexpr int BK = 64;
    constexpr int MI = BM / 64, NI = BN / 64;
    constexpr int LA = BM / 32, LB = BN / 32;
    constexpr int LPW = LA + LB;
    constexpr int STAGE = (BM + BN) * 128;
    static_assert((NST - 2) * LPW < 64, "counted vmcnt out of range");
    static_assert(NST >= 2 && NST <= 4, "tail is written for up to 3 trailing tiles");
    extern __shared__ __attribute__((aligned(16))) unsigned char glds_smem[];
    const int tid = threadIdx.x, lane = tid & 63;
    const int wave = __builtin_amdgcn_readfirstlane(tid >> 6);
    const int wm = wave >> 1, wn = wave & 1;
    const int ks = (!CONV && p.ksplit > 1) ? p.ksplit : 1;
    int t = blockIdx.x;
    {
        const int total = mtiles * ntiles * ks, q = total >> 3, r = total & 7, x = t & 7, i = t >> 3;
        t = (x < r ? x * (q + 1) : r * (q + 1) + (x - r) * q) + i;
    }
    const int slice = t % ks, tile = t / ks;
    t = tile;
    int tn, tm;
    if (p.gm <= 0 || p.gm >= mtiles) {
        tn = t / mtiles; tm = t - tn * mtiles;
    } else {
        const int gsz = p.gm * ntiles, g = t / gsz, r = t - g * gsz;
        const int rows = min(p.gm, mtiles - g * p.gm);
        tn = r / rows; tm = g * p.gm + (r - tn * rows);
    }
    const int m0 = tm * BM, n0 = tn * BN;
    const int nk = p.K / BK / ks;
    const int lda = p.lda ? p.lda : p.K, ldw = p.ldw ? p.ldw : p.K;
    const u16* abase = CONV ? p.A16 - 128 : p.A16 + (size_t)m0 * lda + (size_t)slice * nk * BK;
    const u16* wbase = p.Wb + (size_t)n0 * ldw + (size_t)slice * nk * BK;
    const int lrow = lane >> 3, lch = lane & 7;
    int va[LA], vb[LB];
    int cy0[LA], cx0[LA], cpix[LA], cswz[LA];
#pragma unroll
    for (int j = 0; j < LA; ++j) {
        const int row = (j * 4 + wave) * 8 + lrow;
        if constexpr (CONV) {
            const int m = min(m0 + row, p.M - 1);
            const int b = m / (p.cOH * p.cOW), rem = m - b * (p.cOH * p.cOW);
            const int oy = rem / p.cOW, ox = rem - oy * p.cOW;
            cy0[j] = oy * p.cStride - p.cPad;
            cx0[j] = ox * p.cStride - p.cPad;
            cpix[j] = b * p.cH * p.cW;
            cswz[j] = (lch ^ ((row >> 1) & 7)) << 4;
            va[j] = 0;
        } else {
            va[j] = min(row, p.M - 1 - m0) * lda * 2 + ((lch ^ ((row >> 1) & 7)) << 4);
        }
    }
#pragma unroll
    for (int j = 0; j < LB; ++j) {
        const int row = (j * 4 + wave) * 8 + lrow;
        vb[j] = min(row, p.N - 1 - n0) * ldw * 2 + ((lch ^ ((row >> 1) & 7)) << 4);
    }
#define RGRG_GLDS_ISSUE(STAGE_, KT_)                                                                                   \
    {                                                                                                                  \
        if constexpr (CONV) {                                                                                          \
            const int kbeg_ = (KT_) * BK, tap_ = kbeg_ / p.cCin, c0_ = kbeg_ - tap_ * p.cCin;                          \
            const int kh_ = tap_ / p.cKW, kw_ = tap_ - kh_ * p.cKW;                                                    \
            _Pragma("unroll") for (int j = 0; j < LA; ++j) {                                                           \
                const int iy_ = cy0[j] + kh_, ix_ = cx0[j] + kw_;                                                      \
                const bool in_ = (unsigned)iy_ < (unsigned)p.cH && (unsigned)ix_ < (unsigned)p.cW;                     \
                va[j] = (in_ ? 256 + (cpix[j] + iy_ * p.cW + ix_) * p.cCin * 2 + c0_ * 2 : 0) + cswz[j];               \
            }                                                                                                          \
            glds_issue<BM, LA, LB, LNF * 64 + NST * 4 + 2 + (F16 ? 1 : 0)>(abase, wbase, glds_smem + (STAGE_) * STAGE + wave * 1024, va, vb, 0, (KT_) * (BK * 2)); \
        } else {                                                                                                       \
            glds_issue<BM, LA, LB, LNF * 64 + NST * 4 + (F16 ? 1 : 0)>(abase, wbase, glds_smem + (STAGE_) * STAGE + wave * 1024, va, vb, (KT_) * (BK * 2),       \
                                            (KT_) * (BK * 2));                                                         \
        }                                                                                                              \
    }
    const int frow = lane & 31, fh = lane >> 5, fsw = (frow >> 1) & 7;
    int foff[4];
#pragma unroll
    for (int ks = 0; ks < 4; ++ks) foff[ks] = frow * 128 + (((2 * ks + fh) ^ fsw) << 4);

    f32x16 acc[MI][NI];
#pragma unroll
    for (int mi = 0; mi < MI; ++mi)
#pragma unroll
        for (int ni = 0; ni < NI; ++ni)
#pragma unroll
            for (int r = 0; r < 16; ++r) acc[mi][ni][r] = 0.f;

    const int ccol = lane & 31, crow4 = 4 * (lane >> 5);
    float sh_pre[MI][NI], cs_pre[MI][NI];
#pragma unroll
    for (int mi = 0; mi < MI; ++mi)
#pragma unroll
        for (int ni = 0; ni < NI; ++ni) {
            const int colc = min(n0 + wn * (BN / 2) + ni * 32 + ccol, p.N - 1);
            sh_pre[mi][ni] = p.shift ? p.shift[colc] : 0.f;
            cs_pre[mi][ni] = LNF == 2 ? p.ln_colsum[colc] : 0.f;
        }
    constexpr bool PRE_R = MI * NI == 1 && LNF != 2;
    float rv_pre[16];
#pragma unroll
    for (int r = 0; r < 16; ++r) rv_pre[r] = 0.f;
    if constexpr (PRE_R) {
        if (p.R) {
            const int colc = min(n0 + wn * (BN / 2) + ccol, p.N - 1);
            const int rbase = m0 + wm * (BM / 2) + crow4;
#pragma unroll
            for (int r = 0; r < 16; ++r) {
                const int row = min(rbase + (r & 3) + 8 * (r >> 2), p.M - 1);
                rv_pre[r] = p.R[(size_t)row * p.ldy + colc];
            }
        }
    }

    constexpr int TPR = 256 / BM, PER = 16 / TPR;
    f32x4 lsq[PER / 2];
    if constexpr (LNF == 2) {
        const int srow = min(m0 + tid / TPR, p.M - 1);
        const f32x4* sp = reinterpret_cast<const f32x4*>(p.ln_stats + ((size_t)srow * 16 + (tid % TPR) * PER) * 2);
#pragma unroll
        for (int j = 0; j < PER / 2; ++j) lsq[j] = sp[j];
    }

#define RGRG_GLDS_COMPUTE(STAGE_)                                                                         \
    glds_compute<MI, NI, F16>(glds_smem + (STAGE_) * STAGE + wm * (BM / 2) * 128,                         \
                         glds_smem + (STAGE_) * STAGE + BM * 128 + wn * (BN / 2) * 128, foff, acc)

#pragma unroll
    for (int s = 0; s < NST - 1; ++s) RGRG_GLDS_ISSUE(s, s);
    int kt = 0, cur = 0, nxt = NST - 1;
    for (; kt + NST - 1 < nk; ++kt) {
        wait_vmcnt<(NST - 2) * LPW>();
        __builtin_amdgcn_s_barrier();
        __builtin_amdgcn_sched_barrier(0);
        RGRG_GLDS_ISSUE(nxt, kt + NST - 1);
        __builtin_amdgcn_sched_barrier(0);
        RGRG_GLDS_COMPUTE(cur);
        cur = cur + 1 == NST ? 0 : cur + 1;
        nxt = nxt + 1 == NST ? 0 : nxt + 1;
    }
#define RGRG_GLDS_TAIL(R)                                   \
    if constexpr (NST - 1 >= (R)) {                         \
        wait_vmcnt<((R) - 1) * LPW>();                      \
        __builtin_amdgcn_s_barrier();                       \
        __builtin_amdgcn_sched_barrier(0);                  \
        RGRG_GLDS_COMPUTE(cur);                             \
        cur = cur + 1 == NST ? 0 : cur + 1;                 \
    }
    RGRG_GLDS_TAIL(3) RGRG_GLDS_TAIL(2) RGRG_GLDS_TAIL(1)
#undef RGRG_GLDS_TAIL
#undef RGRG_GLDS_ISSUE
#undef RGRG_GLDS_COMPUTE

    if constexpr (!CONV) {
        if (ks > 1) {
            const __amdgpu_buffer_rsrc_t rs = bf16_rsrc(p.sk_ws + (size_t)tile * ks * (BM * BN));
            const int soff = slice * (BM * BN * 4);
#pragma unroll
            for (int mi = 0; mi < MI; ++mi)
#pragma unroll
                for (int ni = 0; ni < NI; ++ni)
#pragma unroll
                    for (int q = 0; q < 4; ++q)
                        __builtin_amdgcn_raw_buffer_store_b128(
                            __builtin_bit_cast(u32x4, f32x4{acc[mi][ni][4 * q], acc[mi][ni][4 * q + 1], acc[mi][ni][4 * q + 2], acc[mi][ni][4 * q + 3]}),
                            rs, (((mi * NI + ni) * 4 + q) * 256 + tid) * 16, soff, 16);
            asm volatile("s_waitcnt vmcnt(0)" ::: "memory");
            __syncthreads();
            unsigned* flag = reinterpret_cast<unsigned*>(glds_smem + NST * STAGE + BM * 8);
            if (tid == 0) *flag = __hip_atomic_fetch_add(p.sk_cnt + tile, 1u, __ATOMIC_RELAXED, __HIP_MEMORY_SCOPE_AGENT);
            __syncthreads();
            if (*flag != (unsigned)(ks - 1)) return;
            if (tid == 0) __hip_atomic_store(p.sk_cnt + tile, 0u, __ATOMIC_RELAXED, __HIP_MEMORY_SCOPE_AGENT);
#pragma unroll
            for (int mi = 0; mi < MI; ++mi)
#pragma unroll
                for (int ni = 0; ni < NI; ++ni)
#pragma unroll
                    for (int q = 0; q < 4; ++q) {
                        f32x4 tot = {0.f, 0.f, 0.f, 0.f};
                        for (int sl = 0; sl < ks; ++sl) {
                            f32x4 v = __builtin_bit_cast(f32x4, __builtin_amdgcn_raw_buffer_load_b128(rs, (((mi * NI + ni) * 4 + q) * 256 + tid) * 16,
                                                                                                         sl * (BM * BN * 4), 16));
                            if (sl == slice) v = f32x4{acc[mi][ni][4 * q], acc[mi][ni][4 * q + 1], acc[mi][ni][4 * q + 2], acc[mi][ni][4 * q + 3]};
                            tot += v;
                        }
#pragma unroll
                        for (int e = 0; e < 4; ++e) acc[mi][ni][4 * q + e] = tot[e];
                    }
        }
    }

    float2* row_stat = reinterpret_cast<float2*>(glds_smem + NST * STAGE);
    if constexpr (LNF == 2) {
        static_assert(PER == 4 || PER == 8, "slot reduction is written for 64- and 128-row tiles");
        float ls1 = 0.f, ls2 = 0.f;
#pragma unroll
        for (int j0 = 0; j0 < PER / 2; j0 += 2) {
            float g1 = 0.f, g2 = 0.f;
#pragma unroll
            for (int j = j0; j < j0 + 2; ++j) { g1 += lsq[j][0]; g2 += lsq[j][1]; g1 += lsq[j][2]; g2 += lsq[j][3]; }
            if (j0 == 0) { ls1 = g1; ls2 = g2; } else { ls1 += g1; ls2 += g2; }
        }
#pragma unroll
        for (int o = 1; o < TPR; o <<= 1) { ls1 += __shfl_xor(ls1, o, 64); ls2 += __shfl_xor(ls2, o, 64); }
        const float mean = ls1 * (1.0f / 1024.0f);
        const float var = fmaxf(ls2 * (1.0f / 1024.0f) - mean * mean, 0.f);
        if (tid % TPR == 0) row_stat[tid / TPR] = make_float2(mean, 1.0f / sqrtf(var + LN_EPS16));
        __syncthreads();
    }

    float blk1[MI], blk2[MI];
#pragma unroll
    for (int mi = 0; mi < MI; ++mi) { blk1[mi] = 0.f; blk2[mi] = 0.f; }
#pragma unroll
    for (int mi = 0; mi < MI; ++mi)
#pragma unroll
        for (int ni = 0; ni < NI; ++ni) {
            const int col = n0 + wn * (BN / 2) + ni * 32 + ccol;
            const int colc = min(col, p.N - 1);
            const int rbase = m0 + wm * (BM / 2) + mi * 32 + crow4;
            const float sh = sh_pre[mi][ni];
            float rv[16];
#pragma unroll
            for (int r = 0; r < 16; ++r) rv[r] = rv_pre[r];
            if (!PRE_R && LNF != 2 && p.R) {
#pragma unroll
                for (int r = 0; r < 16; ++r) {
                    const int row = min(rbase + (r & 3) + 8 * (r >> 2), p.M - 1);
                    rv[r] = p.R[(size_t)row * p.ldy + colc];
                }
            }
            if (LNF != 2 && p.R16) {
#pragma unroll
                for (int r = 0; r < 16; ++r) {
                    const int row = min(rbase + (r & 3) + 8 * (r >> 2), p.M - 1);
                    rv[r] = from16<F16>(p.R16[(size_t)row * p.ldy + colc]);
                }
            }
            float vv[16];
            if constexpr (LNF == 2) {
                const float cs = cs_pre[mi][ni];
                const int lrow0 = wm * (BM / 2) + mi * 32 + crow4;
#pragma unroll
                for (int r = 0; r < 16; ++r) {
                    const float2 st = row_stat[lrow0 + (r & 3) + 8 * (r >> 2)];
                    vv[r] = apply_act_fast(st.y * (acc[mi][ni][r] - st.x * cs) + sh + rv[r], p.act);
                }
            } else if constexpr (LNF == 0 && !CONV) {
                if (p.G16) {
#pragma unroll
                    for (int r = 0; r < 16; ++r) {
                        const int row = min(rbase + (r & 3) + 8 * (r >> 2), p.M - 1);
                        rv[r] = from16<F16>(p.G16[(size_t)row * p.ldy + colc]);
                    }
#pragma unroll
                    for (int r = 0; r < 16; ++r) vv[r] = (acc[mi][ni][r] + sh) * gelu_new_grad_fast(rv[r]);
                } else {
                    if (p.Ypre16 && col < p.N) {
#pragma unroll
                        for (int r = 0; r < 16; ++r) {
                            const int dr = (r & 3) + 8 * (r >> 2);
                            if (rbase + dr < p.M)
                                p.Ypre16[(size_t)rbase * p.ldy + col + (size_t)(dr * p.ldy)] = (u16)to16<F16>(acc[mi][ni][r] + sh + rv[r]);
                        }
                    }
#pragma unroll
                    for (int r = 0; r < 16; ++r) vv[r] = apply_act_fast(acc[mi][ni][r] + sh + rv[r], p.act);
                }
            } else {
#pragma unroll
                for (int r = 0; r < 16; ++r) vv[r] = apply_act_fast(acc[mi][ni][r] + sh + rv[r], p.act);
            }
            if (col < p.N) {
#pragma unroll
                for (int r = 0; r < 16; ++r) {
                    const int dr = (r & 3) + 8 * (r >> 2);
                    const float v = vv[r];
                    if (rbase + dr < p.M) {
                        const size_t o = (size_t)rbase * p.ldy + col + (size_t)(dr * p.ldy);
                        if (p.Y16) p.Y16[o] = (u16)to16<F16>(v);
                        else if (p.N > 8192) __builtin_nontemporal_store(v, &p.Y[o]);
                        else p.Y[o] = v;
                        if constexpr (LNF == 1) p.Yb16[o] = (u16)to16<F16>(v);
                    }
                }
            }
            if constexpr (LNF == 1) {
                float a1[16], a2[16];
#pragma unroll
                for (int r = 0; r < 16; ++r) { a1[r] = vv[r]; a2[r] = vv[r] * vv[r]; }
#define RGRG_BFLY(H, BIT)                                                                         \
                {                                                                                         \
                    const bool up = (lane & (BIT)) != 0;                                                  \
                    _Pragma("unroll") for (int i = 0; i < (H); ++i) {                                     \
                        const float s1 = up ? a1[i] : a1[i + (H)], s2 = up ? a2[i] : a2[i + (H)];         \
                        const float k1 = up ? a1[i + (H)] : a1[i], k2 = up ? a2[i + (H)] : a2[i];         \
                        a1[i] = k1 + __shfl_xor(s1, (BIT), 64);                                           \
                        a2[i] = k2 + __shfl_xor(s2, (BIT), 64);                                           \
                    }                                                                                     \
                }
                RGRG_BFLY(8, 16) RGRG_BFLY(4, 8) RGRG_BFLY(2, 4) RGRG_BFLY(1, 2)
#undef RGRG_BFLY
                a1[0] += __shfl_xor(a1[0], 1, 64);
                a2[0] += __shfl_xor(a2[0], 1, 64);
                blk1[mi] += a1[0];
                blk2[mi] += a2[0];
            }
        }
    if constexpr (LNF == 1) {
        float2* xch = reinterpret_cast<float2*>(glds_smem + NST * STAGE);
        const int r = (lane >> 1) & 15, lrow = (r & 3) + 8 * (r >> 2) + 4 * (lane >> 5);
        if constexpr (NI == 1) {
            if (wn == 1 && !(lane & 1)) {
#pragma unroll
                for (int mi = 0; mi < MI; ++mi) xch[(wave * MI + mi) * 32 + lrow] = make_float2(blk1[mi], blk2[mi]);
            }
            __syncthreads();
        }
        if (!(lane & 1) && (NI == 2 || wn == 0)) {
#pragma unroll
            for (int mi = 0; mi < MI; ++mi) {
                float s1 = blk1[mi], s2 = blk2[mi];
                if constexpr (NI == 1) {
                    const float2 o = xch[((wave + 1) * MI + mi) * 32 + lrow];
                    s1 += o.x; s2 += o.y;
                }
                const int row = m0 + wm * (BM / 2) + mi * 32 + lrow;
                const int slot = NI == 2 ? (n0 + wn * 64) / 64 : n0 / 64;
                if (row < p.M) *reinterpret_cast<float2*>(p.stats_out + ((size_t)row * 16 + slot) * 2) = make_float2(s1, s2);
            }
        }
    }
}

template <int TAG>
__device__ __forceinline__ void pp_dma4(const u16* base, unsigned char* dst, const int (&v)[4], int soff) {
    const __amdgpu_buffer_rsrc_t r = bf16_rsrc(base);
#pragma unroll
    for (int j = 0; j < 4; ++j) __builtin_amdgcn_raw_ptr_buffer_load_lds(r, (lds_ptr_t)(dst + j * 8192), 16, v[j], soff, 0, 0);
}
template <int TAG>
__device__ __forceinline__ void pp_dma2(const u16* base, unsigned char* dst, int v0, int v1, int soff) {
    const __amdgpu_buffer_rsrc_t r = bf16_rsrc(base);
    __builtin_amdgcn_raw_ptr_buffer_load_lds(r, (lds_ptr_t)dst, 16, v0, soff, 0, 0);
    __builtin_amdgcn_raw_ptr_buffer_load_lds(r, (lds_ptr_t)(dst + 1024), 16, v1, soff, 0, 0);
}
template <bool F16>
__global__ __launch_bounds__(512) void gemm_bf16_pp_kernel(const GemmBf16Params p, const int mtiles, const int ntiles) {
    constexpr int BM = 256, BN = 256, BK = 64, MI = 4, NI = 2;
    constexpr int STAGE = (BM + BN) * 128, WOFF = BM * 128;
    constexpr int TAG = F16 ? 901 : 900;
    extern __shared__ __attribute__((aligned(16))) unsigned char pp_smem[];
    const int tid = threadIdx.x, lane = tid & 63;
    const int wave = __builtin_amdgcn_readfirstlane(tid >> 6);
    const int g = wave >> 2, wq = wave & 3;
    int t = blockIdx.x;
// ... 242 lines not shown
            const int rbase = m0 + g * 128 + mi * 32 + crow4;
            const float sh = esh[ni];
            float rv[16], vv[16];
#pragma unroll
            for (int r = 0; r < 16; ++r) rv[r] = 0.f;
            if (p.R) {
#pragma unroll
                for (int r = 0; r < 16; ++r) {
                    const int row = min(rbase + (r & 3) + 8 * (r >> 2), p.M - 1);
                    rv[r] = p.R[(size_t)row * p.ldy + colc];
                }
            }
            if (p.G16) {
#pragma unroll
                for (int r = 0; r < 16; ++r) {
                    const int row = min(rbase + (r & 3) + 8 * (r >> 2), p.M - 1);
                    rv[r] = from16<F16>(p.G16[(size_t)row * p.ldy + colc]);
                }
#pragma unroll
                for (int r = 0; r < 16; ++r) vv[r] = (acc[mi][ni][r] + sh) * gelu_new_grad_fast(rv[r]);
            } else {
                if (p.Ypre16 && col < p.N) {
#pragma unroll
                    for (int r = 0; r < 16; ++r) {
                        const int dr = (r & 3) + 8 * (r >> 2);
                        if (rbase + dr < p.M)
                            p.Ypre16[(size_t)rbase * p.ldy + col + (size_t)(dr * p.ldy)] = (u16)to16<F16>(acc[mi][ni][r] + sh + rv[r]);
                    }
                }
#pragma unroll
                for (int r = 0; r < 16; ++r) vv[r] = apply_act_fast(acc[mi][ni][r] + sh + rv[r], p.act);
            }
            if (col < p.N) {
#pragma unroll
                for (int r = 0; r < 16; ++r) {
                    const int dr = (r & 3) + 8 * (r >> 2);
                    if (rbase + dr < p.M) {
                        const size_t o = (size_t)rbase * p.ldy + col + (size_t)(dr * p.ldy);
                        if (p.Y16) p.Y16[o] = (u16)to16<F16>(vv[r]);
                        else if (p.N > 8192) __builtin_nontemporal_store(vv[r], &p.Y[o]);
                        else p.Y[o] = vv[r];
                    }
                }
            }
        }
}

__global__ __launch_bounds__(256) void f32_to_bf16_kernel(const float* __restrict__ src, u16* __restrict__ dst, size_t n, int f16) {
    for (size_t i = (size_t)blockIdx.x * blockDim.x + threadIdx.x; i < n; i += (size_t)gridDim.x * blockDim.x)
        dst[i] = (u16)to16_rt(src[i], f16);
}

template <int BM, int BN, int THREADS>
static int launch_bf16_cfg(const GemmBf16Params& p, hipStream_t st) {
    constexpr size_t lds = (size_t)(2 * BM + 2 * BN) * LDB * sizeof(u16);
    const int mtiles = (p.M + BM - 1) / BM, ntiles = (p.N + BN - 1) / BN;
#define RGRG_W_LAUNCH(A16_, F16_) hipLaunchKernelGGL((gemm_bf16w_kernel<BM, BN, THREADS, A16_, F16_>), dim3(mtiles * ntiles), dim3(THREADS), lds, st, p, mtiles, ntiles)
    if (p.A16) { if (p.f16) RGRG_W_LAUNCH(true, true); else RGRG_W_LAUNCH(true, false); }
    else { if (p.f16) RGRG_W_LAUNCH(false, true); else RGRG_W_LAUNCH(false, false); }
#undef RGRG_W_LAUNCH
    RGRG_LAUNCH_CHECK();
    return RGRG_OK;
}

template <int BM, int BN, int THREADS>
static int bf16_attr() {
    RGRG_HIP(hipFuncSetAttribute(reinterpret_cast<const void*>(&gemm_bf16w_kernel<BM, BN, THREADS, false, false>),
                                 hipFuncAttributeMaxDynamicSharedMemorySize, 81920));
    RGRG_HIP(hipFuncSetAttribute(reinterpret_cast<const void*>(&gemm_bf16w_kernel<BM, BN, THREADS, true, false>),
                                 hipFuncAttributeMaxDynamicSharedMemorySize, 81920));
    RGRG_HIP(hipFuncSetAttribute(reinterpret_cast<const void*>(&gemm_bf16w_kernel<BM, BN, THREADS, false, true>),
                                 hipFuncAttributeMaxDynamicSharedMemorySize, 81920));
    RGRG_HIP(hipFuncSetAttribute(reinterpret_cast<const void*>(&gemm_bf16w_kernel<BM, BN, THREADS, true, true>),
                                 hipFuncAttributeMaxDynamicSharedMemorySize, 81920));
    return RGRG_OK;
}

template <int BM, int BN, int NST>
static int glds_attr() {
    constexpr int lds = NST * (BM + BN) * 128 + BM * 16;
#define RGRG_G_ATTR(...) RGRG_HIP(hipFuncSetAttribute(reinterpret_cast<const void*>(&gemm_bf16_glds_kernel<BM, BN, NST, __VA_ARGS__>), hipFuncAttributeMaxDynamicSharedMemorySize, lds))
    RGRG_G_ATTR(false, false, 0); RGRG_G_ATTR(true, false, 0); RGRG_G_ATTR(false, true, 0); RGRG_G_ATTR(true, true, 0);
    RGRG_G_ATTR(false, false, 1); RGRG_G_ATTR(false, true, 1); RGRG_G_ATTR(false, false, 2); RGRG_G_ATTR(false, true, 2);
#undef RGRG_G_ATTR
    return RGRG_OK;
}
template <int BM, int BN>
static int glds_attrs() {
    int rc;
    if ((rc = glds_attr<BM, BN, 2>()) || (rc = glds_attr<BM, BN, 3>())) return rc;
    return glds_attr<BM, BN, 4>();
}

static int gemm_gm_override();
#include "gemm_kp.inc"

constexpr int PP_LDS = 2 * (256 + 256) * 128;

int init_gemm_bf16_attrs() {
    static bool done = false;
    if (done) return RGRG_OK;
    int rc;
    if ((rc = bf16_attr<128, 128, 512>()) || (rc = bf16_attr<64, 64, 256>())) return rc;
    if ((rc = glds_attrs<128, 128>()) || (rc = glds_attrs<64, 64>()) || (rc = glds_attrs<128, 64>()) || (rc = glds_attrs<64, 128>())) return rc;
    RGRG_HIP(hipFuncSetAttribute(reinterpret_cast<const void*>(&gemm_bf16_pp_kernel<false>), hipFuncAttributeMaxDynamicSharedMemorySize, PP_LDS));
    RGRG_HIP(hipFuncSetAttribute(reinterpret_cast<const void*>(&gemm_bf16_pp_kernel<true>), hipFuncAttributeMaxDynamicSharedMemorySize, PP_LDS));
    if ((rc = kp_attr<128, 128, 2>()) || (rc = kp_attr<64, 64, 4>()) || (rc = kp_attr<64, 64, 3>()) || (rc = kp_attr<128, 64, 3>()) || (rc = kp_attr<64, 128, 3>()) || (rc = kp_attr<64, 64, 2>()) || (rc = pr_attrs())) return rc;
    done = true;
    return RGRG_OK;
}

static int gemm_gm_override() {
    static const int v = [] { const char* e = getenv("RGRG_GEMM_GM"); return e ? atoi(e) : 0; }();
    return v;
}

template <int BM, int BN, int NST>
static int launch_glds_cfg(const GemmBf16Params& p0, hipStream_t st) {
    GemmBf16Params p = p0;
    const int mtiles = (p.M + BM - 1) / BM, ntiles = (p.N + BN - 1) / BN;
    if (p.gm == 0) {
        const int o = gemm_gm_override();
        p.gm = o < 0 ? 0 : o > 0 ? o : (mtiles > 16 ? 8 : 0);
    }
    const int ks = (!p.cCin && p.ksplit > 1 && p.sk_ws && p.sk_cnt && (p.K / 64) % p.ksplit == 0 && p.K / 64 / p.ksplit >= NST - 1) ? p.ksplit : 1;
    p.ksplit = ks;
#define RGRG_G_LAUNCH(CONV_, F16_, LNF_) hipLaunchKernelGGL((gemm_bf16_glds_kernel<BM, BN, NST, CONV_, F16_, LNF_>), dim3(mtiles * ntiles * ks), dim3(256), NST * (BM + BN) * 128 + BM * 16, st, p, mtiles, ntiles)
    if (p.cCin) { if (p.f16) RGRG_G_LAUNCH(true, true, 0); else RGRG_G_LAUNCH(true, false, 0); }
    else if (p.Yb16) { if (p.f16) RGRG_G_LAUNCH(false, true, 1); else RGRG_G_LAUNCH(false, false, 1); }
    else if (p.ln_colsum) { if (p.f16) RGRG_G_LAUNCH(false, true, 2); else RGRG_G_LAUNCH(false, false, 2); }
    else { if (p.f16) RGRG_G_LAUNCH(false, true, 0); else RGRG_G_LAUNCH(false, false, 0); }
#undef RGRG_G_LAUNCH
    RGRG_LAUNCH_CHECK();
    return RGRG_OK;
}
template <int BM, int BN>
static int launch_glds_nst(const GemmBf16Params& p, int nst, hipStream_t st) {
    if (nst == 2) return launch_glds_cfg<BM, BN, 2>(p, st);
    if (nst == 3) return launch_glds_cfg<BM, BN, 3>(p, st);
    return launch_glds_cfg<BM, BN, 4>(p, st);
}

static bool pp_eligible(const GemmBf16Params& p) {
    return !p.cCin && !p.Yb16 && !p.ln_colsum && !p.R16 && p.K >= 256 && p.K % 64 == 0;
}
static int launch_pp(const GemmBf16Params& p0, hipStream_t st) {
    GemmBf16Params p = p0;
    const int mtiles = (p.M + 255) / 256, ntiles = (p.N + 255) / 256;
    if (p.gm == 0) {
        const int o = gemm_gm_override();
        p.gm = o < 0 ? 0 : o > 0 ? o : (mtiles > 8 ? 8 : 0);
    }
    { const char* e = getenv("RGRG_PP_DBG"); p.dbg = e ? atoi(e) : 0; }
    if (p.f16) hipLaunchKernelGGL(gemm_bf16_pp_kernel<true>, dim3(mtiles * ntiles), dim3(512), PP_LDS, st, p, mtiles, ntiles);
    else hipLaunchKernelGGL(gemm_bf16_pp_kernel<false>, dim3(mtiles * ntiles), dim3(512), PP_LDS, st, p, mtiles, ntiles);
    RGRG_LAUNCH_CHECK();
    return RGRG_OK;
}
static bool pp_enabled() {
    static const bool v = [] { const char* e = getenv("RGRG_GEMM_PP"); return !e || atoi(e) != 0; }();
    return v;
}

static bool pp_lm_head() {
    static const bool v = [] { const char* e = getenv("RGRG_GEMM_PP_LMHEAD"); return !e || atoi(e) != 0; }();
    return v;
}

static int launch_glds(const GemmBf16Params& p, int tile, hipStream_t st) {
    int shape = tile & 15, nst = tile >> 4;
    switch (shape) {
        case 6: return launch_kp_cfg<128, 128, 2>(p, st);
        case 7: return launch_kp_cfg<64, 64, 4>(p, st);
        case 8: return launch_kp_cfg<128, 64, 3>(p, st);
        case 9: return launch_kp_cfg<64, 128, 3>(p, st);
        case 10: return launch_kp_cfg<64, 64, 3>(p, st);
        case 11: return launch_kp_auto(p, st);
        case 12: return launch_pr(p, st);
        case 13: return launch_kp_cfg<64, 64, 2>(p, st);
    }
    if (shape == 5) {
        if (!pp_eligible(p)) { set_error("bf16 GEMM: the 256 x 256 kernel does not take this variant"); return RGRG_EINVAL; }
        return launch_pp(p, st);
    }
    if (shape == 0 && pp_enabled() && pp_eligible(p)) {
        const long tiles_pp = (long)((p.M + 255) / 256) * ((p.N + 255) / 256);
        if (p.M >= 2048 && tiles_pp >= 192) return launch_pp(p, st);
        if (p.M >= 512 && p.N >= 32768 && tiles_pp >= 512 && pp_lm_head()) return launch_pp(p, st);
    }
    if (shape == 0 && p.ln_colsum && p.M <= 320) {
        static const int o = [] { const char* e = getenv("RGRG_CONS_TILE_SMALLM"); return e ? atoi(e) : 0; }();
        if (o) { shape = o & 15; nst = o >> 4; }
    }
    if (shape == 0) {
        const long tiles_big = (long)((p.M + 127) / 128) * ((p.N + 127) / 128);
        if (p.N <= 64) { shape = 3; nst = 2; }
        else if (tiles_big >= 512) { shape = 1; nst = 2; }
        else if (p.K >= 8192 && tiles_big >= 192) { shape = 1; nst = 2; }
        else if (p.K > 1024) { shape = 2; nst = 4; }
        else if (tiles_big >= 256) { shape = 3; nst = 3; }
        else if (tiles_big >= 128) { shape = 2; nst = 3; }
        else { shape = 2; nst = 4; }
    }
    if (nst == 0) nst = 4;
    if (p.K / 64 < nst - 1) nst = 2;
    switch (shape) {
        case 1: return launch_glds_nst<128, 128>(p, nst, st);
        case 2: return launch_glds_nst<64, 64>(p, nst, st);
        case 3: return launch_glds_nst<128, 64>(p, nst, st);
        case 4: return launch_glds_nst<64, 128>(p, nst, st);
    }
    set_error("bf16 GEMM: unknown tile configuration %d", tile);
    return RGRG_EINVAL;
}

bool gemm_bf16_cand_epilogue_ok(int M, int N, int K) {
    static const bool on = [] { const char* e = getenv("RGRG_LMHEAD_CAND"); return !e || atoi(e) != 0; }();
    const long tiles_pp = (long)((M + 255) / 256) * ((N + 255) / 256);
    return on && pp_enabled() && pp_lm_head() && M >= 512 && N >= 32768 && tiles_pp >= 512 && K >= 256 && K % 64 == 0;
}

int launch_gemm_bf16w_ex(const float* A, const void* A16, const void* Wb, const float* shift, const float* R, float* Y, void* Y16,
                         int M, int N, int K, int ldy, int act, hipStream_t st, int f16, const GemmLnFold* ln) {
    RGRG_CHECK_ARG((A || A16) && Wb && (Y || Y16 || (ln && ln->cand_val)) && M > 0 && N > 0 && K > 0 && K % (4 * BK16) == 0 && ldy >= N);
    GemmBf16Params p{A, reinterpret_cast<const u16*>(A16), reinterpret_cast<const u16*>(Wb), shift, R, Y,
                     reinterpret_cast<u16*>(Y16), M, N, K, ldy, act};
    p.f16 = f16 ? 1 : 0;
    if (ln && (ln->Ypre16 || ln->G16)) {
        RGRG_CHECK_ARG(A16 && (size_t)128 * K * 2 < ((size_t)1 << 31) && !ln->Yb16 && !ln->ln_colsum);
        RGRG_CHECK_ARG(!(ln->Ypre16 && ln->G16) && (!ln->G16 || (!R && act == RGRG_ACT_NONE)));
        p.Ypre16 = reinterpret_cast<u16*>(ln->Ypre16); p.G16 = reinterpret_cast<const u16*>(ln->G16);
    } else if (ln && (ln->Yb16 || ln->ln_colsum)) {
        RGRG_CHECK_ARG(A16 && (size_t)128 * K * 2 < ((size_t)1 << 31));
        RGRG_CHECK_ARG((ln->Yb16 != nullptr) != (ln->ln_colsum != nullptr));
        RGRG_CHECK_ARG(!ln->Yb16 || (Y && ln->stats_out && N == 1024));
        RGRG_CHECK_ARG(!ln->ln_colsum || (ln->ln_stats && K == 1024 && !R));
        p.Yb16 = reinterpret_cast<u16*>(ln->Yb16); p.stats_out = ln->stats_out;
        p.ln_stats = ln->ln_stats; p.ln_colsum = ln->ln_colsum;
    }
    if (ln && ln->ksplit > 1) { p.ksplit = ln->ksplit; p.sk_ws = ln->sk_ws; p.sk_cnt = ln->sk_cnt; }
    if (ln && ln->cand_val) {
        RGRG_CHECK_ARG(A16 && ln->cand_idx && !R && act == RGRG_ACT_NONE && !Y16 && !ln->Yb16 && !ln->ln_colsum && !ln->Ypre16 && !ln->G16);
        p.cand_val = ln->cand_val; p.cand_idx = ln->cand_idx;
        return launch_glds(p, 5, st);
    }
    if (ln && ln->kp && A16 && (size_t)128 * K * 2 < ((size_t)1 << 31) && kp_eligible(p, 4)) return launch_glds(p, 11, st);
    if (A16 && (size_t)128 * K * 2 < ((size_t)1 << 31)) return launch_glds(p, 0, st);
    const long tiles_big = (long)((M + 127) / 128) * ((N + 127) / 128);
    return tiles_big >= 192 ? launch_bf16_cfg<128, 128, 512>(p, st) : launch_bf16_cfg<64, 64, 256>(p, st);
}

int launch_gemm_bf16w(const float* A, const void* Wb, const float* shift, const float* R, float* Y, int M, int N, int K,
                      int ldy, int act, hipStream_t st, int f16) {
    return launch_gemm_bf16w_ex(A, nullptr, Wb, shift, R, Y, nullptr, M, N, K, ldy, act, st, f16, nullptr);
}

__global__ __launch_bounds__(256) void bf16_to_f32_kernel(const u16* __restrict__ src, float* __restrict__ dst, size_t n, int f16) {
    for (size_t i = (size_t)blockIdx.x * blockDim.x + threadIdx.x; i < n; i += (size_t)gridDim.x * blockDim.x)
        dst[i] = from16_rt(src[i], f16);
}

int convert_f32_to_bf16(const float* src, void* dst, size_t n, hipStream_t st, int f16) {
    const int blocks = (int)((n + 255) / 256 < 4096 ? (n + 255) / 256 : 4096);
    hipLaunchKernelGGL(f32_to_bf16_kernel, dim3(blocks), dim3(256), 0, st, src, reinterpret_cast<u16*>(dst), n, f16 ? 1 : 0);
    RGRG_LAUNCH_CHECK();
    return RGRG_OK;
}

}

using namespace rgrg;

extern "C" int rgrg_f32_to_bf16(const float* src, uint16_t* dst, int64_t n, int fp16, void* stream) {
    RGRG_CHECK_ARG(src && dst && n > 0);
    return convert_f32_to_bf16(src, dst, (size_t)n, as_stream(stream), fp16);
}

extern "C" int rgrg_bf16_to_f32(const uint16_t* src, float* dst, int64_t n, int fp16, void* stream) {
    RGRG_CHECK_ARG(src && dst && n > 0);
    const int blocks = (int)(((size_t)n + 255) / 256 < 4096 ? ((size_t)n + 255) / 256 : 4096);
    hipLaunchKernelGGL(bf16_to_f32_kernel, dim3(blocks), dim3(256), 0, as_stream(stream), src, dst, (size_t)n, fp16 ? 1 : 0);
    RGRG_LAUNCH_CHECK();
    return RGRG_OK;
}

extern "C" int rgrg_linear_bf16w_f32(const float* A, const uint16_t* Wb, const float* shift, const float* R, float* Y,
                                     int M, int N, int K, int ldy, int act, int fp16, void* stream) {
    int rc = init_gemm_bf16_attrs();
    if (rc) return rc;
    return launch_gemm_bf16w(A, Wb, shift, R, Y, M, N, K, ldy, act, as_stream(stream), fp16);
}

extern "C" int rgrg_linear_bf16_f32(const uint16_t* A16, const uint16_t* Wb, const float* shift, const float* R, float* Y,
                                    uint16_t* Y16, int M, int N, int K, int ldy, int act, int fp16, void* stream) {
    int rc = init_gemm_bf16_attrs();
    if (rc) return rc;
    RGRG_CHECK_ARG(A16 && ((Y != nullptr) != (Y16 != nullptr)));
    return launch_gemm_bf16w_ex(nullptr, A16, Wb, shift, R, Y, Y16, M, N, K, ldy, act, as_stream(stream), fp16, nullptr);
}

extern "C" int rgrg_debug_linear_bf16_tile(const uint16_t* A16, const uint16_t* Wb, const float* shift, const float* R, float* Y,
                                           int M, int N, int K, int ldy, int act, int tile, int lda, int ldw, int fp16, void* stream) {
    int rc = init_gemm_bf16_attrs();
    if (rc) return rc;
    RGRG_CHECK_ARG(A16 && Wb && Y && M > 0 && N > 0 && K > 0 && K % 256 == 0 && ldy >= N && (size_t)128 * K * 2 < ((size_t)1 << 31));
    RGRG_CHECK_ARG((lda == 0 || lda >= K) && (ldw == 0 || ldw >= K));
    GemmBf16Params p{nullptr, A16, Wb, shift, R, Y, nullptr, M, N, K, ldy, act, lda, ldw};
    p.f16 = fp16 ? 1 : 0;
    return launch_glds(p, tile, as_stream(stream));
}

extern "C" int rgrg_debug_linear_bf16_train(const uint16_t* A16, const uint16_t* Wb, const float* shift, const float* R, float* Y,
                                            uint16_t* Y16, uint16_t* Ypre16, const uint16_t* G16, int M, int N, int K, int ldy,
                                            int act, int tile, int fp16, void* stream) {
    int rc = init_gemm_bf16_attrs();
    if (rc) return rc;
    RGRG_CHECK_ARG(A16 && Wb && ((Y != nullptr) != (Y16 != nullptr)) && M > 0 && N > 0 && K > 0 && K % 256 == 0 && ldy >= N);
    RGRG_CHECK_ARG((size_t)128 * K * 2 < ((size_t)1 << 31) && !(Ypre16 && G16) && (!G16 || (!R && act == RGRG_ACT_NONE)));
    GemmBf16Params p{nullptr, A16, Wb, shift, R, Y, Y16, M, N, K, ldy, act};
    p.f16 = fp16 ? 1 : 0;
    p.Ypre16 = Ypre16; p.G16 = G16;
    return launch_glds(p, tile, as_stream(stream));
}

extern "C" int rgrg_debug_linear_bf16_argmax(const uint16_t* A16, const uint16_t* Wb, const float* shift, int M, int N, int K,
                                             float* cand_val, int* cand_idx, int fp16, void* stream) {
    int rc = init_gemm_bf16_attrs();
    if (rc) return rc;
    RGRG_CHECK_ARG(A16 && Wb && cand_val && cand_idx && M > 0 && N > 0 && K >= 256 && K % 256 == 0);
    GemmLnFold f{};
    f.cand_val = cand_val; f.cand_idx = cand_idx;
    return launch_gemm_bf16w_ex(nullptr, A16, Wb, shift, nullptr, nullptr, nullptr, M, N, K, N, RGRG_ACT_NONE, as_stream(stream), fp16, &f);
}

extern "C" int rgrg_debug_linear_bf16_ln(const uint16_t* A16, const uint16_t* Wb, const float* shift, const float* R, float* Y,
                                         uint16_t* Yb16, float* stats_out, const float* ln_stats, const float* ln_colsum, int M,
                                         int N, int K, int ldy, int act, int fp16, void* stream) {
    int rc = init_gemm_bf16_attrs();
    if (rc) return rc;
    RGRG_CHECK_ARG(A16 && Wb && Y);
    GemmLnFold f{};
    f.Yb16 = Yb16; f.stats_out = stats_out; f.ln_stats = ln_stats; f.ln_colsum = ln_colsum;
    return launch_gemm_bf16w_ex(nullptr, A16, Wb, shift, R, Y, nullptr, M, N, K, ldy, act, as_stream(stream), fp16, &f);
}

extern "C" int rgrg_debug_linear_bf16_ln_kp(const uint16_t* A16, const uint16_t* Wb, const float* shift, const float* R, float* Y,
                                            uint16_t* Y16, uint16_t* Yb16, float* stats_out, const float* ln_stats, const float* ln_colsum,
                                            int M, int N, int K, int ldy, int act, int fp16, int kp, void* stream) {
    int rc = init_gemm_bf16_attrs();
    if (rc) return rc;
    RGRG_CHECK_ARG(A16 && Wb && ((Y != nullptr) != (Y16 != nullptr)));
    GemmLnFold f{};
    f.Yb16 = Yb16; f.stats_out = stats_out; f.ln_stats = ln_stats; f.ln_colsum = ln_colsum; f.kp = kp;
    return launch_gemm_bf16w_ex(nullptr, A16, Wb, shift, R, Y, Y16, M, N, K, ldy, act, as_stream(stream), fp16, &f);
}

extern "C" int rgrg_conv2d_nhwc_bf16(const uint16_t* X16, const uint16_t* Wb, const float* shift, const uint16_t* R16, float* Y,
                                     uint16_t* Y16, int B, int H, int Wd, int Cin, int Cout, int KH, int KW, int stride, int pad,
                                     int act, int fp16, void* stream) {
    int rc = init_gemm_bf16_attrs();
    if (rc) return rc;
    RGRG_CHECK_ARG(X16 && Wb && ((Y != nullptr) != (Y16 != nullptr)) && B > 0 && H > 0 && Wd > 0 && Cin > 0 && Cin % 64 == 0);
    RGRG_CHECK_ARG(Cout > 0 && KH > 0 && KW > 0 && stride > 0 && pad >= 0);
    RGRG_CHECK_ARG((size_t)B * H * Wd * Cin * 2 + 256 < ((size_t)1 << 31));
    GemmBf16Params p{};
    p.A16 = X16; p.Wb = Wb; p.shift = shift; p.R16 = R16; p.Y = Y; p.Y16 = Y16; p.f16 = fp16 ? 1 : 0;
    p.cH = H; p.cW = Wd; p.cCin = Cin; p.cKH = KH; p.cKW = KW; p.cStride = stride; p.cPad = pad;
    p.cOH = (H + 2 * pad - KH) / stride + 1;
    p.cOW = (Wd + 2 * pad - KW) / stride + 1;
    RGRG_CHECK_ARG(p.cOH > 0 && p.cOW > 0);
    p.M = B * p.cOH * p.cOW; p.N = Cout; p.K = KH * KW * Cin; p.ldy = Cout; p.act = act;
    RGRG_CHECK_ARG((size_t)128 * p.K * 2 < ((size_t)1 << 31));
    return launch_glds(p, 0, as_stream(stream));
}
```

rgrg_amd/csrc/internal.h:

```cpp
#pragma once
#include "common.h"

namespace rgrg {

int launch_gemm_dense(const float* A, const float* W, const float* shift, const float* R, float* Y, int M, int N, int K,
                      int ldy, int act, float* ws, size_t ws_floats, hipStream_t st);
int init_gemm_attrs();

struct GemmLnFold {
    void* Yb16 = nullptr;
    float* stats_out = nullptr;
    const float* ln_stats = nullptr;
    const float* ln_colsum = nullptr;
    void* Ypre16 = nullptr;
    const void* G16 = nullptr;
    int ksplit = 0;
    float* sk_ws = nullptr;
    unsigned* sk_cnt = nullptr;
    float* cand_val = nullptr;
    int* cand_idx = nullptr;
    int kp = 0;
};
int init_gemm_bf16_attrs();
bool gemm_bf16_cand_epilogue_ok(int M, int N, int K);
int launch_gemm_bf16w_ex(const float* A, const void* A16, const void* Wb, const float* shift, const float* R, float* Y, void* Y16,
                         int M, int N, int K, int ldy, int act, hipStream_t st, int f16, const GemmLnFold* ln = nullptr);
int launch_gemm_bf16w(const float* A, const void* Wb, const float* shift, const float* R, float* Y, int M, int N, int K,
                      int ldy, int act, hipStream_t st, int f16);
int convert_f32_to_bf16(const float* src, void* dst, size_t n, hipStream_t st, int f16);

int launch_gelu_apply(const float* pre, float* out, size_t n, hipStream_t st);
int launch_gelu_backward(float* d, const float* pre, size_t n, hipStream_t st);
int launch_relu_backward(float* d, const float* h, size_t n, hipStream_t st);
int launch_ln_backward(const float* dy, const float* x, const float* g, float* out, int rows, int D, int accumulate, hipStream_t st);
int launch_ce_backward(float* logits, size_t ld, int V, int row0, int rows, const long long* ids, const int* row_valid,
                       const float* row_lse, const int* n_scored, float scale, const int* id_error, hipStream_t st);
int launch_transpose_pad(const float* src, float* dst, int R, int Cc, int Rp, hipStream_t st);
int launch_colsum(const float* src, float* out, int R, int Cc, hipStream_t st);
int launch_attn_backward(const float* qkv, const float* ukv, int ld_ukv, int kcol, const float* am, const float* d_att,
                         const float* att, const float* lse, float* delta, float* d_qkv, float* d_ukv, int S, int H, int T,
                         DropoutParams drop, hipStream_t st, unsigned short* d_qkv16 = nullptr, int f16 = 0, float ukv_scale = 1.0f);
int launch_resid_dropout_ln16(const float* y, const unsigned short* y16, const float* resid, float* x, const float* g, const float* b,
                              unsigned short* xn16, DropoutParams drop, int f16, int rows, int D, hipStream_t st);
int launch_ln_backward16(const float* dy, const unsigned short* dy16, const float* x, const float* g, float* out, unsigned short* out16,
                         int rows, int D, int accumulate, DropoutParams drop, int f16, hipStream_t st);
int launch_ce_backward16(const float* logits, size_t ld, int V, int row0, int rows, const long long* ids, const int* row_valid,
                         const float* row_lse, const int* n_scored, float scale, const int* id_error, unsigned short* out16, int f16,
                         hipStream_t st);
int launch_dropout_add(const float* src, const float* resid, float* out, size_t n, DropoutParams drop, hipStream_t st);

bool attn16_supported(int T);
int launch_attn16_forward(const unsigned short* qkv16, const unsigned short* ukv16, int ld_ukv, int kcol, const float* am,
                          unsigned short* out16, float* lse, int S, int H, int T, DropoutParams drop, int f16, hipStream_t st);
int launch_attn16_backward(const unsigned short* qkv16, const unsigned short* ukv16, int ld_ukv, int kcol, const float* am,
                           const unsigned short* d_att16, const unsigned short* att16, const float* lse, unsigned short* d_qkv16,
                           float* d_ukv, int S, int H, int T, DropoutParams drop, float ukv_scale, int f16, hipStream_t st);


size_t sample_params_bytes();
int enqueue_sample_params(void* prm_dev, float temperature, int top_k, float top_p, unsigned long long seed, hipStream_t st);
int launch_sample_step(const float* logits, int ld, int S, int V, const void* prm_dev, long long* ids, int ld_ids, int* finished,
                       int* step, int* done_len, int* sync, float* lp, int ld_lp, hipStream_t st);

}
```

rgrg_amd/csrc/runtime.hip:

```cpp
#include <stdarg.h>
#include <string.h>

#include "common.h"

namespace rgrg {
static thread_local char g_err[512] = "";
void set_error(const char* fmt, ...) {
    va_list ap;
    va_start(ap, fmt);
    vsnprintf(g_err, sizeof(g_err), fmt, ap);
    va_end(ap);
}
}

extern "C" const char* rgrg_last_error(void) { return rgrg::g_err; }
extern "C" int rgrg_abi_version(void) { return 24; }
extern "C" int rgrg_device_arch(int dev, char* buf, int buflen) {
    RGRG_CHECK_ARG(buf && buflen > 1);
    hipDeviceProp_t prop;
    RGRG_HIP(hipGetDeviceProperties(&prop, dev));
    strncpy(buf, prop.gcnArchName, buflen - 1);
    buf[buflen - 1] = 0;
    return RGRG_OK;
}

#include <chrono>
namespace rgrg {
__global__ void chain_kernel(int* p, int n) {
    if (threadIdx.x == 0 && blockIdx.x == 0) p[0] += n;
}
}

extern "C" int rgrg_debug_chain(int n, int mode, int blocks, float* us_per_kernel) {
    RGRG_CHECK_ARG(n > 0 && us_per_kernel && blocks > 0);
    int* d = nullptr;
    RGRG_HIP(hipMalloc((void**)&d, 64));
    RGRG_HIP(hipMemset(d, 0, 64));
    hipStream_t st = nullptr;
    if (mode != 2) RGRG_HIP(hipStreamCreateWithFlags(&st, hipStreamNonBlocking));
    hipGraphExec_t exec = nullptr;
    if (mode == 1) {
        hipGraph_t g = nullptr;
        RGRG_HIP(hipStreamBeginCapture(st, hipStreamCaptureModeThreadLocal));
        for (int i = 0; i < n; ++i) hipLaunchKernelGGL(rgrg::chain_kernel, dim3(blocks), dim3(64), 0, st, d, 1);
        RGRG_HIP(hipStreamEndCapture(st, &g));
        RGRG_HIP(hipGraphInstantiate(&exec, g, nullptr, nullptr, 0));
        (void)hipGraphDestroy(g);
        RGRG_HIP(hipGraphLaunch(exec, st));
        RGRG_HIP(hipStreamSynchronize(st));
    } else {
        for (int i = 0; i < 16; ++i) hipLaunchKernelGGL(rgrg::chain_kernel, dim3(blocks), dim3(64), 0, st, d, 1);
        RGRG_HIP(hipStreamSynchronize(st));
    }
    auto t0 = std::chrono::steady_clock::now();
    if (mode == 1) {
        RGRG_HIP(hipGraphLaunch(exec, st));
    } else {
        for (int i = 0; i < n; ++i) hipLaunchKernelGGL(rgrg::chain_kernel, dim3(blocks), dim3(64), 0, st, d, 1);
    }
    RGRG_HIP(hipStreamSynchronize(st));
    auto t1 = std::chrono::steady_clock::now();
    *us_per_kernel = (float)(std::chrono::duration<double, std::micro>(t1 - t0).count() / n);
    if (exec) (void)hipGraphExecDestroy(exec);
    if (st) (void)hipStreamDestroy(st);
    (void)hipFree(d);
    return RGRG_OK;
}
```

Measured before the change: 86.18 images/sec.

## Write K/V straight into the 16-bit cache from the QKV GEMM epilogue

```diff
diff --git a/include/rgrg_hip.h b/include/rgrg_hip.h
--- a/include/rgrg_hip.h
+++ b/include/rgrg_hip.h
@@ -136,12 +136,17 @@
 int rgrg_debug_linear_bf16_ln(const uint16_t* A16, const uint16_t* Wb, const float* shift, const float* R, float* Y,
                               uint16_t* Yb16, float* stats_out, const float* ln_stats, const float* ln_colsum, int M, int N,
                               int K, int ldy, int act, int fp16, void* stream);
+int rgrg_debug_linear_bf16_ln_kv(const uint16_t* A16, const uint16_t* Wb, const float* shift, float* Y, const float* ln_stats,
+                                 const float* ln_colsum, uint16_t* kcache, uint16_t* vcache, const int* step_dev, int M, int H,
+                                 int T_slots, int K, int ldy, int fp16, void* stream);
 int rgrg_debug_linear_bf16_ln_kp(const uint16_t* A16, const uint16_t* Wb, const float* shift, const float* R, float* Y,
                                  uint16_t* Y16, uint16_t* Yb16, float* stats_out, const float* ln_stats, const float* ln_colsum,
                                  int M, int N, int K, int ldy, int act, int fp16, int kp, void* stream);
 int rgrg_debug_attn_decode(const float* qkv, int ld_qkv, void* kcache, void* vcache, const int* step_dev, float* out,
                            uint16_t* out16, int S, int H, int T_slots, const int* src, const float* kmask, int kv16, int fp16,
                            int ni, int frag_out, int max_workgroups, void* stream);
+int rgrg_debug_attn_decode_qonly(const float* q, int ld_q, const void* kcache, const void* vcache, const int* step_dev, float* out,
+                                 uint16_t* out16, int S, int H, int T_slots, int fp16, int max_workgroups, void* stream);
 int rgrg_debug_attn_decode_kv8(const float* qkv, int ld_qkv, uint8_t* kcache, uint8_t* vcache, const int* step_dev, float* out,
                                uint16_t* out16, int S, int H, int T_slots, const int* src, const float* kmask, int fp16,
                                int max_workgroups, void* stream);
diff --git a/rgrg_amd/_hip.py b/rgrg_amd/_hip.py
--- a/rgrg_amd/_hip.py
+++ b/rgrg_amd/_hip.py
@@ -10,7 +10,7 @@
 _i, _f, _p = C.c_int, C.c_float, C.c_void_p
 
 ACT_NONE, ACT_RELU, ACT_GELU_NEW = 0, 1, 2
-ABI_VERSION = 24
+ABI_VERSION = 25
 
 
 class RgrgHipError(RuntimeError):
@@ -80,6 +80,8 @@
     "rgrg_debug_linear_bf16_ln": (_i, [_p, _p, _p, _p, _p, _p, _p, _p, _p, _i, _i, _i, _i, _i, _i, _p]),
     "rgrg_debug_linear_bf16_ln_kp": (_i, [_p, _p, _p, _p, _p, _p, _p, _p, _p, _p, _i, _i, _i, _i, _i, _i, _i, _p]),
     "rgrg_debug_attn_decode": (_i, [_p, _i, _p, _p, _p, _p, _p, _i, _i, _i, _p, _p, _i, _i, _i, _i, _i, _p]),
+    "rgrg_debug_linear_bf16_ln_kv": (_i, [_p, _p, _p, _p, _p, _p, _p, _p, _p, _i, _i, _i, _i, _i, _i, _p]),
+    "rgrg_debug_attn_decode_qonly": (_i, [_p, _i, _p, _p, _p, _p, _p, _i, _i, _i, _i, _i, _p]),
     "rgrg_debug_attn_decode_kv8": (_i, [_p, _i, _p, _p, _p, _p, _p, _i, _i, _i, _p, _p, _i, _i, _p]),
     "rgrg_debug_attn_prefill": (_i, [_p, _p, _i, _i, _p, _p, _p, _p, _i, _i, _i, _i, C.c_uint64, C.c_uint32, _f, _i, _p]),
     "rgrg_debug_attn_backward_f32": (_i, [_p, _p, _i, _i, _p, _p, _p, _p, _p, _p, _p, _p, _i, _i, _i, C.c_uint64, C.c_uint32, _f,
diff --git a/rgrg_amd/csrc/decoder.hip b/rgrg_amd/csrc/decoder.hip
--- a/rgrg_amd/csrc/decoder.hip
+++ b/rgrg_amd/csrc/decoder.hip
@@ -469,7 +469,7 @@
     return o;
 }
 
-template <int NI, bool HAS_SRC, bool FIRST, bool F16>
+template <int NI, bool HAS_SRC, bool FIRST, bool F16, bool QONLY>
 __device__ __forceinline__ void kv16_wave_chunk(const __amdgpu_buffer_rsrc_t kc, const __amdgpu_buffer_rsrc_t vc, const int* __restrict__ srow,
                                                 int s, int hd, int H, int T, int base, int nkeys, int slot, int g, int d8,
                                                 Kv16Row& r, float (&q)[8], u32x4& kn16, u32x4& vn16, float& m, float& l, float (&acc)[8]) {
@@ -487,19 +487,25 @@
     __builtin_amdgcn_sched_barrier(0);
     if constexpr (FIRST) {
 #pragma unroll
-        for (int e = 0; e < 4; ++e)
-            asm volatile("" : "+v"(r.q0[e]), "+v"(r.q1[e]), "+v"(r.k0[e]), "+v"(r.k1[e]), "+v"(r.v0[e]), "+v"(r.v1[e]));
+        for (int e = 0; e < 4; ++e) {
+            if constexpr (QONLY) asm volatile("" : "+v"(r.q0[e]), "+v"(r.q1[e]));
+            else asm volatile("" : "+v"(r.q0[e]), "+v"(r.q1[e]), "+v"(r.k0[e]), "+v"(r.k1[e]), "+v"(r.v0[e]), "+v"(r.v1[e]));
+        }
 #pragma unroll
         for (int e = 0; e < 4; ++e) { q[e] = r.q0[e]; q[4 + e] = r.q1[e]; }
-        kn16 = kv16_pack_round<F16>(r.k0, r.k1);
-        vn16 = kv16_pack_round<F16>(r.v0, r.v1);
+        if constexpr (!QONLY) {
+            kn16 = kv16_pack_round<F16>(r.k0, r.k1);
+            vn16 = kv16_pack_round<F16>(r.v0, r.v1);
+        }
     }
     float sc[NI];
     float cmax = -INFINITY;
 #pragma unroll
     for (int i = 0; i < NI; ++i) {
         const int j = base + i * 8 + g;
-        if (j == slot) { kk[i] = kn16; vv[i] = vn16; }
+        if constexpr (!QONLY) {
+            if (j == slot) { kk[i] = kn16; vv[i] = vn16; }
+        }
         float dot = 0.f;
 #pragma unroll
         for (int e = 0; e < 4; ++e)
@@ -531,7 +537,7 @@
     m = m_new;
 }
 
-template <bool HAS_SRC, bool F16>
+template <bool HAS_SRC, bool F16, bool QONLY = false>
 __global__ __launch_bounds__(256) void attn_decode_kv16_wave_kernel(const float* __restrict__ qkv, int ld_qkv,
                                                                     u16* __restrict__ kc, u16* __restrict__ vc,
                                                                     const int* __restrict__ step, float* __restrict__ out,
@@ -549,16 +555,18 @@
     Kv16Row r;
     r.q0 = *reinterpret_cast<const f32x4*>(row + hd * 64 + d8 * 8);
     r.q1 = *reinterpret_cast<const f32x4*>(row + hd * 64 + d8 * 8 + 4);
-    r.k0 = *reinterpret_cast<const f32x4*>(row + D + hd * 64 + d8 * 8);
-    r.k1 = *reinterpret_cast<const f32x4*>(row + D + hd * 64 + d8 * 8 + 4);
-    r.v0 = *reinterpret_cast<const f32x4*>(row + 2 * D + hd * 64 + d8 * 8);
-    r.v1 = *reinterpret_cast<const f32x4*>(row + 2 * D + hd * 64 + d8 * 8 + 4);
+    if constexpr (!QONLY) {
+        r.k0 = *reinterpret_cast<const f32x4*>(row + D + hd * 64 + d8 * 8);
+        r.k1 = *reinterpret_cast<const f32x4*>(row + D + hd * 64 + d8 * 8 + 4);
+        r.v0 = *reinterpret_cast<const f32x4*>(row + 2 * D + hd * 64 + d8 * 8);
+        r.v1 = *reinterpret_cast<const f32x4*>(row + 2 * D + hd * 64 + d8 * 8 + 4);
+    }
     float m = -INFINITY, l = 0.f, acc[8], q[8];
     u32x4 kn16, vn16;
 #pragma unroll
     for (int e = 0; e < 8; ++e) acc[e] = 0.f;
 #define KV16_CHUNK(NI_, FIRST_, BASE_) \
-    kv16_wave_chunk<NI_, HAS_SRC, FIRST_, F16>(rk, rv, srow, s, hd, H, T, BASE_, nkeys, slot, g, d8, r, q, kn16, vn16, m, l, acc)
+    kv16_wave_chunk<NI_, HAS_SRC, FIRST_, F16, QONLY>(rk, rv, srow, s, hd, H, T, BASE_, nkeys, slot, g, d8, r, q, kn16, vn16, m, l, acc)
 #define KV16_TAIL(FIRST_, BASE_, REM_)                                                                   \
     switch (((REM_) + 7) >> 3) {                                                                         \
         case 1: KV16_CHUNK(1, FIRST_, BASE_); break;                                                     \
@@ -581,10 +589,12 @@
     }
 #undef KV16_TAIL
 #undef KV16_CHUNK
-    if (g == 0) {
-        const size_t o = (((size_t)s * H + hd) * T + slot) * 64 + d8 * 8;
-        *reinterpret_cast<u32x4*>(kc + o) = kn16;
-        *reinterpret_cast<u32x4*>(vc + o) = vn16;
+    if constexpr (!QONLY) {
+        if (g == 0) {
+            const size_t o = (((size_t)s * H + hd) * T + slot) * 64 + d8 * 8;
+            *reinterpret_cast<u32x4*>(kc + o) = kn16;
+            *reinterpret_cast<u32x4*>(vc + o) = vn16;
+        }
     }
     float M = fmaxf(m, dpp_get<0x128, 0xf>(m));
     M = fmaxf(M, __shfl_xor(M, 16, 64));
@@ -925,6 +935,7 @@
     int frag_out;
     int max_wgs;
     hipStream_t st;
+    bool q_only = false;
 };
 static int launch_attn_decode(const AttnDecodeLaunch& a) {
     if (a.kmask && (a.fmt != KV_F32 || a.src)) {
@@ -946,15 +957,22 @@
         }
         const int wgs = a.S * a.H / 4;
         const dim3 wgrid(a.max_wgs > 0 ? std::min(wgs, a.max_wgs) : wgs), wblk(256);
+        if (a.q_only && (a.fmt == KV_E4M3 || a.src)) {
+            set_error("decode attention: the q-only variant exists for the 16-bit K/V cache without an ancestor table (%s)",
+                      a.src ? "beam search" : "e4m3 K/V cache");
+            return RGRG_EINVAL;
+        }
         if (a.fmt == KV_E4M3)
             return launch_attn_decode_kv8(a.qkv, a.ld_qkv, static_cast<uint8_t*>(a.kc), static_cast<uint8_t*>(a.vc), a.step, a.out, a.out16,
                                           a.S, a.H, a.T, a.src, a.f16, (int)wgrid.x, a.st);
-#define KV16_LAUNCH(SRC_, F16_) hipLaunchKernelGGL((attn_decode_kv16_wave_kernel<SRC_, F16_>), wgrid, wblk, 0, a.st, a.qkv, a.ld_qkv, \
+#define KV16_LAUNCH(...) hipLaunchKernelGGL((attn_decode_kv16_wave_kernel<__VA_ARGS__>), wgrid, wblk, 0, a.st, a.qkv, a.ld_qkv, \
                                                   static_cast<u16*>(a.kc), static_cast<u16*>(a.vc), a.step, a.out, a.S, a.H, a.T, a.src, a.out16)
-        if (a.src) { if (a.f16) KV16_LAUNCH(true, true); else KV16_LAUNCH(true, false); }
+        if (a.q_only) { if (a.f16) KV16_LAUNCH(false, true, true); else KV16_LAUNCH(false, false, true); }
+        else if (a.src) { if (a.f16) KV16_LAUNCH(true, true); else KV16_LAUNCH(true, false); }
         else { if (a.f16) KV16_LAUNCH(false, true); else KV16_LAUNCH(false, false); }
 #undef KV16_LAUNCH
     } else {
+        if (a.q_only) { set_error("decode attention: the q-only variant exists for the 16-bit K/V cache only"); return RGRG_EINVAL; }
         const dim3 grid(a.S * a.H), blk(256);
         const int ni = a.ni ? a.ni : (a.S * a.H <= 4096 ? 9 : 2);
         if (ni != 9 && ni != 2) { set_error("decode attention: %d keys per group, the kernel is built for 9 and 2", ni); return RGRG_EINVAL; }
@@ -970,9 +988,11 @@
     return RGRG_OK;
 }
 
-static int launch_attention(rgrg_decoder* d, int l, int S, const int* src, unsigned short* att16, int frag_out = 0, int r0 = 0) {
+static int launch_attention(rgrg_decoder* d, int l, int S, const int* src, unsigned short* att16, int frag_out = 0, int r0 = 0,
+                            bool q_only = false) {
     const int D = d->D;
     AttnDecodeLaunch a{};
+    a.q_only = q_only;
     a.ld_qkv = 3 * D; a.step = d->step; a.S = S; a.H = d->H; a.T = d->T; a.src = src; a.kmask = d->key_mask_cur;
     a.frag_out = frag_out; a.st = d->stream; a.plane_elems = d->kv_kv_stride;
     a.fmt = kv_format(d, S);
@@ -1145,6 +1165,20 @@
     return RGRG_OK;
 }
 
+static bool step_ln_fold(const rgrg_decoder* d, int S) {
+    return kv_is_bf16(d, S) && d->xn16 && d->ln_fold && d->ln_stat && d->layers[0].c_attn.wb_ln && d->D == 1024;
+}
+static bool step_qkv_cache(const rgrg_decoder* d, int S, bool plain) {
+    const KvFormat f = kv_format(d, S);
+    return d->qkv_cache && plain && step_ln_fold(d, S) && (f == KV_BF16 || f == KV_F16) && d->kp_gemms != 1 && d->kp_gemms != 3 && !d->key_mask_cur;
+}
+static GemmLnFold cons_kv_cache(const rgrg_decoder* d, const GemmLnFold& cons, int l, int r0) {
+    GemmLnFold f = cons;
+    u16* kcr = reinterpret_cast<u16*>(d->kv) + (size_t)l * d->kv_layer_stride + (size_t)r0 * d->H * d->T * 64;
+    f.kv_k = kcr; f.kv_v = kcr + d->kv_kv_stride; f.kv_step = d->step; f.kv_H = d->H; f.kv_T = d->T;
+    return f;
+}
+
 int enqueue_step(rgrg_decoder* d, int S, bool count, const int* tok_override, const int* src, bool beam) {
     if (S <= decode_row_limit(d)) return enqueue_step_fused(d, S, count, tok_override, src, beam);
     if (count) { d->gemm_bytes_per_step = 0; d->gemm_flops_per_step = 0.0; d->gemm_launches_per_step = 0; }
@@ -1155,7 +1189,8 @@
     unsigned short* xn16 = (kv_is_bf16(d, S) && d->xn16) ? d->xn16 : nullptr;
     unsigned short* att16 = xn16 ? d->att16 : nullptr;
     unsigned short* ff16 = xn16 ? d->ff16 : nullptr;
-    const bool fold = xn16 && d->ln_fold && d->ln_stat && d->layers[0].c_attn.wb_ln && D == 1024;
+    const bool fold = step_ln_fold(d, S);
+    const bool qc = step_qkv_cache(d, S, !tok_override && !src);
     static const float cons_tag = 0.f;
     GemmLnFold prod{}, cons{};
     prod.Yb16 = xn16; prod.stats_out = d->ln_stat;
@@ -1184,9 +1219,10 @@
             const LayerW& w = d->layers[l];
             const float* ng = (l + 1 < d->n_layer) ? d->layers[l + 1].ln1_g : d->lnf_g;
             const float* nb = (l + 1 < d->n_layer) ? d->layers[l + 1].ln1_b : d->lnf_b;
-            if ((rc2 = linear(d, w.c_attn, xn, nullptr, d->qkv + 3 * o, rows, 3 * D, RGRG_ACT_NONE, count, xn16r, nullptr, cfr))) return rc2;
+            const GemmLnFold cons_kv = qc ? cons_kv_cache(d, cons_r, l, r0) : cons_r;
+            if ((rc2 = linear(d, w.c_attn, xn, nullptr, d->qkv + 3 * o, rows, 3 * D, RGRG_ACT_NONE, count, xn16r, nullptr, qc ? &cons_kv : cfr))) return rc2;
             if ((rc2 = trace_mark(d, r0, l * 8 + 0))) return rc2;
-            if ((rc2 = launch_attention(d, l, rows, src ? src + (size_t)r0 * d->T : nullptr, att16r, 0, r0))) return rc2;
+            if ((rc2 = launch_attention(d, l, rows, src ? src + (size_t)r0 * d->T : nullptr, att16r, 0, r0, qc))) return rc2;
             if ((rc2 = trace_mark(d, r0, l * 8 + 1))) return rc2;
             if ((rc2 = linear(d, w.attn_proj, d->att + o, x, x, rows, D, RGRG_ACT_NONE, count, att16r, nullptr, pfr))) return rc2;
             if ((rc2 = trace_mark(d, r0, l * 8 + 2))) return rc2;
@@ -1287,6 +1323,7 @@
     }
     if (const char* e = getenv("RGRG_GEMM_KP")) d->kp_gemms = atoi(e);
     if (const char* e = getenv("RGRG_W16_FUSED")) d->w16_fused = atoi(e) != 0;
+    if (const char* e = getenv("RGRG_QKV_CACHE")) d->qkv_cache = atoi(e) != 0;
     if (const char* e = getenv("RGRG_DECODE_CHAINS")) {
         const int v = atoi(e);
         d->chains = (v >= -MAX_CHAINS && v <= MAX_CHAINS && v != 0 && v != -1) ? v : 1;
@@ -1609,6 +1646,16 @@
     a.step = step_dev; a.out = out; a.out16 = out16; a.S = S; a.H = H; a.T = T_slots; a.src = src; a.kmask = kmask;
     a.fmt = kv16 ? (fp16 ? KV_F16 : KV_BF16) : KV_F32; a.f16 = fp16 ? 1 : 0; a.ni = ni; a.frag_out = frag_out ? 1 : 0; a.max_wgs = max_workgroups;
     a.st = as_stream(stream);
+    return launch_attn_decode(a);
+}
+
+extern "C" int rgrg_debug_attn_decode_qonly(const float* q, int ld_q, const void* kcache, const void* vcache, const int* step_dev, float* out,
+                                            uint16_t* out16, int S, int H, int T_slots, int fp16, int max_workgroups, void* stream) {
+    RGRG_CHECK_ARG(q && kcache && vcache && step_dev && S > 0 && H > 0 && T_slots >= 2 && ld_q >= H * 64 && (out || out16));
+    AttnDecodeLaunch a{};
+    a.qkv = q; a.ld_qkv = ld_q; a.kc = const_cast<void*>(kcache); a.vc = const_cast<void*>(vcache);
+    a.plane_elems = (size_t)S * H * T_slots * 64; a.step = step_dev; a.out = out; a.out16 = out16; a.S = S; a.H = H; a.T = T_slots;
+    a.fmt = fp16 ? KV_F16 : KV_BF16; a.f16 = fp16 ? 1 : 0; a.max_wgs = max_workgroups; a.st = as_stream(stream); a.q_only = true;
     return launch_attn_decode(a);
 }
 
@@ -1782,8 +1829,9 @@
     hipLaunchKernelGGL(set_int_kernel, dim3(1), dim3(64), 0, d->stream, d->step, nkeys - 2);
     int rc = RGRG_OK;
     unsigned short* att16 = (kv_is_bf16(d, S) && d->xn16) ? d->att16 : nullptr;
+    const bool qc = step_qkv_cache(d, S, true);
     for (int it = 0; it < iters && !rc; ++it)
-        for (int l = 0; l < d->n_layer && !rc; ++l) rc = launch_attention(d, l, S, nullptr, att16, 0, 0);
+        for (int l = 0; l < d->n_layer && !rc; ++l) rc = launch_attention(d, l, S, nullptr, att16, 0, 0, qc);
     hipLaunchKernelGGL(set_int_kernel, dim3(1), dim3(64), 0, d->stream, d->step, 0);
     d->stream = keep;
     return rc;
@@ -1837,7 +1885,8 @@
     unsigned short* xn16 = (bf && d->xn16) ? d->xn16 : nullptr;
     unsigned short* att16 = xn16 ? d->att16 : nullptr;
     unsigned short* ff16 = xn16 ? d->ff16 : nullptr;
-    const bool fold = xn16 && d->ln_fold && d->ln_stat && d->layers[0].c_attn.wb_ln && D == 1024;
+    const bool fold = step_ln_fold(d, S);
+    const bool qc = step_qkv_cache(d, S, true);
     static const float cons_tag = 0.f;
     GemmLnFold prod{}, cons{};
     prod.Yb16 = xn16; prod.stats_out = d->ln_stat;
@@ -1847,6 +1896,7 @@
     int rc = RGRG_OK;
     float tg = 0.f, ta = 0.f;
     d->gemm_bytes_per_step = 0; d->gemm_flops_per_step = 0.0; d->gemm_launches_per_step = 0;
+    if (qc) hipLaunchKernelGGL(set_int_kernel, dim3(1), dim3(64), 0, d->stream, d->step, nkeys - 2);
     for (int it = -1; it < iters && !rc; ++it) {
         const bool c = it == -1;
         if (it == 0) RGRG_HIP(hipEventRecord(e0, d->stream));
@@ -1869,7 +1919,8 @@
                     if ((rc2 = enqueue_layer_gemms(d, l, S, c, nullptr, d->x, d->x2, 1))) break;
                     continue;
                 }
-                if ((rc2 = linear(d, w.c_attn, d->xn + o, nullptr, d->qkv + 3 * o, rows, 3 * D, RGRG_ACT_NONE, c, xn16r, nullptr, cfr))) break;
+                const GemmLnFold cons_kv = qc ? cons_kv_cache(d, cons_r, l, r0) : cons_r;
+                if ((rc2 = linear(d, w.c_attn, d->xn + o, nullptr, d->qkv + 3 * o, rows, 3 * D, RGRG_ACT_NONE, c, xn16r, nullptr, qc ? &cons_kv : cfr))) break;
                 if ((rc2 = linear(d, w.attn_proj, d->att + o, d->x + o, d->h1 + o, rows, D, RGRG_ACT_NONE, c, att16r, nullptr, pfr))) break;
                 if ((rc2 = linear(d, w.c_fc, d->xn + o, nullptr, d->ff + 4 * o, rows, 4 * D, RGRG_ACT_GELU_NEW, c, xn16r, ff16r, cfr))) break;
                 if ((rc2 = linear(d, w.mlp_proj, d->ff + 4 * o, d->x + o, d->h1 + o, rows, D, RGRG_ACT_NONE, c, ff16r, nullptr, pfr))) break;
@@ -1900,7 +1951,7 @@
             rc = run_row_ranges(d, S, fused ? 1 : step_chains(d, S, true, fold), [&](int r0, int rows) -> int {
                 int rc2 = RGRG_OK;
                 for (int l = 0; l < d->n_layer && !rc2; ++l)
-                    rc2 = launch_attention(d, l, rows, nullptr, att16 ? att16 + (size_t)r0 * D : nullptr, fused ? 1 : 0, r0);
+                    rc2 = launch_attention(d, l, rows, nullptr, att16 ? att16 + (size_t)r0 * D : nullptr, fused ? 1 : 0, r0, qc);
                 return rc2;
             });
         }
diff --git a/rgrg_amd/csrc/decoder_internal.h b/rgrg_amd/csrc/decoder_internal.h
--- a/rgrg_amd/csrc/decoder_internal.h
+++ b/rgrg_amd/csrc/decoder_internal.h
@@ -158,6 +158,7 @@
     struct TraceMark { hipEvent_t ev; int r0; int tag; };
     std::vector<TraceMark>* trace = nullptr;
     bool w16_fused = true;
+    bool qkv_cache = true;
     int kp_gemms = 2;
     int gemm_launches_per_step = 0;
     const int* pos_override_cur = nullptr;
diff --git a/rgrg_amd/csrc/gemm_bf16.hip b/rgrg_amd/csrc/gemm_bf16.hip
--- a/rgrg_amd/csrc/gemm_bf16.hip
+++ b/rgrg_amd/csrc/gemm_bf16.hip
@@ -23,6 +23,9 @@
     float* stats_out = nullptr;
     const float* ln_stats = nullptr;
     const float* ln_colsum = nullptr;
+    u16 *kv_k = nullptr, *kv_v = nullptr;
+    const int* kv_step = nullptr;
+    int kv_H = 0, kv_T = 0;
     u16* Ypre16 = nullptr;
     const u16* G16 = nullptr;
     int gm = 0;
@@ -285,6 +288,7 @@
     constexpr int STAGE = (BM + BN) * 128;
     static_assert((NST - 2) * LPW < 64, "counted vmcnt out of range");
     static_assert(NST >= 2 && NST <= 4, "tail is written for up to 3 trailing tiles");
+    constexpr bool CONS = LNF >= 2, KVC = LNF == 3;
     extern __shared__ __attribute__((aligned(16))) unsigned char glds_smem[];
     const int tid = threadIdx.x, lane = tid & 63;
     const int wave = __builtin_amdgcn_readfirstlane(tid >> 6);
@@ -371,9 +375,9 @@
         for (int ni = 0; ni < NI; ++ni) {
             const int colc = min(n0 + wn * (BN / 2) + ni * 32 + ccol, p.N - 1);
             sh_pre[mi][ni] = p.shift ? p.shift[colc] : 0.f;
-            cs_pre[mi][ni] = LNF == 2 ? p.ln_colsum[colc] : 0.f;
-        }
-    constexpr bool PRE_R = MI * NI == 1 && LNF != 2;
+            cs_pre[mi][ni] = CONS ? p.ln_colsum[colc] : 0.f;
+        }
+    constexpr bool PRE_R = MI * NI == 1 && !CONS;
     float rv_pre[16];
 #pragma unroll
     for (int r = 0; r < 16; ++r) rv_pre[r] = 0.f;
@@ -391,7 +395,9 @@
 
     constexpr int TPR = 256 / BM, PER = 16 / TPR;
     f32x4 lsq[PER / 2];
-    if constexpr (LNF == 2) {
+    int kv_slot = 0;
+    if constexpr (KVC) kv_slot = *p.kv_step + 1;
+    if constexpr (CONS) {
         const int srow = min(m0 + tid / TPR, p.M - 1);
         const f32x4* sp = reinterpret_cast<const f32x4*>(p.ln_stats + ((size_t)srow * 16 + (tid % TPR) * PER) * 2);
 #pragma unroll
@@ -468,7 +474,7 @@
     }
 
     float2* row_stat = reinterpret_cast<float2*>(glds_smem + NST * STAGE);
-    if constexpr (LNF == 2) {
+    if constexpr (CONS) {
         static_assert(PER == 4 || PER == 8, "slot reduction is written for 64- and 128-row tiles");
         float ls1 = 0.f, ls2 = 0.f;
 #pragma unroll
@@ -500,14 +506,14 @@
             float rv[16];
 #pragma unroll
             for (int r = 0; r < 16; ++r) rv[r] = rv_pre[r];
-            if (!PRE_R && LNF != 2 && p.R) {
+            if (!PRE_R && !CONS && p.R) {
 #pragma unroll
                 for (int r = 0; r < 16; ++r) {
                     const int row = min(rbase + (r & 3) + 8 * (r >> 2), p.M - 1);
                     rv[r] = p.R[(size_t)row * p.ldy + colc];
                 }
             }
-            if (LNF != 2 && p.R16) {
+            if (!CONS && p.R16) {
 #pragma unroll
                 for (int r = 0; r < 16; ++r) {
                     const int row = min(rbase + (r & 3) + 8 * (r >> 2), p.M - 1);
@@ -515,7 +521,7 @@
                 }
             }
             float vv[16];
-            if constexpr (LNF == 2) {
+            if constexpr (CONS) {
                 const float cs = cs_pre[mi][ni];
                 const int lrow0 = wm * (BM / 2) + mi * 32 + crow4;
 #pragma unroll
@@ -548,7 +554,20 @@
 #pragma unroll
                 for (int r = 0; r < 16; ++r) vv[r] = apply_act_fast(acc[mi][ni][r] + sh + rv[r], p.act);
             }
-            if (col < p.N) {
+            bool to_cache = false;
+            if constexpr (KVC) to_cache = n0 + wn * (BN / 2) + ni * 32 >= p.kv_H * 64;
+            if (to_cache) {
+                const int Dm = p.kv_H * 64, c = col - Dm, isv = c >= Dm ? 1 : 0, ch = c - isv * Dm;
+                u16* plane = isv ? p.kv_v : p.kv_k;
+                const size_t o0 = ((size_t)(ch >> 6) * p.kv_T + kv_slot) * 64 + (ch & 63);
+                if (kv_slot < p.kv_T) {
+#pragma unroll
+                    for (int r = 0; r < 16; ++r) {
+                        const int row = rbase + (r & 3) + 8 * (r >> 2);
+                        if (row < p.M) plane[(size_t)row * p.kv_H * p.kv_T * 64 + o0] = (u16)to16<F16>(vv[r]);
+                    }
+                }
+            } else if (col < p.N) {
 #pragma unroll
                 for (int r = 0; r < 16; ++r) {
                     const int dr = (r & 3) + 8 * (r >> 2);
@@ -957,6 +976,7 @@
 #define RGRG_G_ATTR(...) RGRG_HIP(hipFuncSetAttribute(reinterpret_cast<const void*>(&gemm_bf16_glds_kernel<BM, BN, NST, __VA_ARGS__>), hipFuncAttributeMaxDynamicSharedMemorySize, lds))
     RGRG_G_ATTR(false, false, 0); RGRG_G_ATTR(true, false, 0); RGRG_G_ATTR(false, true, 0); RGRG_G_ATTR(true, true, 0);
     RGRG_G_ATTR(false, false, 1); RGRG_G_ATTR(false, true, 1); RGRG_G_ATTR(false, false, 2); RGRG_G_ATTR(false, true, 2);
+    RGRG_G_ATTR(false, false, 3); RGRG_G_ATTR(false, true, 3);
 #undef RGRG_G_ATTR
     return RGRG_OK;
 }
@@ -1003,6 +1023,7 @@
 #define RGRG_G_LAUNCH(CONV_, F16_, LNF_) hipLaunchKernelGGL((gemm_bf16_glds_kernel<BM, BN, NST, CONV_, F16_, LNF_>), dim3(mtiles * ntiles * ks), dim3(256), NST * (BM + BN) * 128 + BM * 16, st, p, mtiles, ntiles)
     if (p.cCin) { if (p.f16) RGRG_G_LAUNCH(true, true, 0); else RGRG_G_LAUNCH(true, false, 0); }
     else if (p.Yb16) { if (p.f16) RGRG_G_LAUNCH(false, true, 1); else RGRG_G_LAUNCH(false, false, 1); }
+    else if (p.ln_colsum && p.kv_k) { if (p.f16) RGRG_G_LAUNCH(false, true, 3); else RGRG_G_LAUNCH(false, false, 3); }
     else if (p.ln_colsum) { if (p.f16) RGRG_G_LAUNCH(false, true, 2); else RGRG_G_LAUNCH(false, false, 2); }
     else { if (p.f16) RGRG_G_LAUNCH(false, true, 0); else RGRG_G_LAUNCH(false, false, 0); }
 #undef RGRG_G_LAUNCH
@@ -1044,6 +1065,7 @@
 
 static int launch_glds(const GemmBf16Params& p, int tile, hipStream_t st) {
     int shape = tile & 15, nst = tile >> 4;
+    if (p.kv_k && shape >= 5) { set_error("bf16 GEMM: only the LDS-DMA kernel has the K/V-cache epilogue (tile %d)", tile); return RGRG_EINVAL; }
     switch (shape) {
         case 6: return launch_kp_cfg<128, 128, 2>(p, st);
         case 7: return launch_kp_cfg<64, 64, 4>(p, st);
@@ -1112,6 +1134,15 @@
         RGRG_CHECK_ARG(!ln->ln_colsum || (ln->ln_stats && K == 1024 && !R));
         p.Yb16 = reinterpret_cast<u16*>(ln->Yb16); p.stats_out = ln->stats_out;
         p.ln_stats = ln->ln_stats; p.ln_colsum = ln->ln_colsum;
+        if (ln->kv_k) {
+            RGRG_CHECK_ARG(ln->ln_colsum && ln->kv_v && ln->kv_step && ln->kv_H > 0 && ln->kv_T >= 2 && N == 3 * ln->kv_H * 64 && Y && !Y16 && !ln->kp &&
+                           ln->ksplit <= 1 && act == RGRG_ACT_NONE);
+            p.kv_k = reinterpret_cast<u16*>(ln->kv_k); p.kv_v = reinterpret_cast<u16*>(ln->kv_v);
+            p.kv_step = ln->kv_step; p.kv_H = ln->kv_H; p.kv_T = ln->kv_T;
+        }
+    } else if (ln && ln->kv_k) {
+        set_error("bf16 GEMM: the K/V-cache epilogue belongs to the folded-LayerNorm consumer");
+        return RGRG_EINVAL;
     }
     if (ln && ln->ksplit > 1) { p.ksplit = ln->ksplit; p.sk_ws = ln->sk_ws; p.sk_cnt = ln->sk_cnt; }
     if (ln && ln->cand_val) {
@@ -1217,6 +1248,18 @@
     GemmLnFold f{};
     f.Yb16 = Yb16; f.stats_out = stats_out; f.ln_stats = ln_stats; f.ln_colsum = ln_colsum;
     return launch_gemm_bf16w_ex(nullptr, A16, Wb, shift, R, Y, nullptr, M, N, K, ldy, act, as_stream(stream), fp16, &f);
+}
+
+extern "C" int rgrg_debug_linear_bf16_ln_kv(const uint16_t* A16, const uint16_t* Wb, const float* shift, float* Y, const float* ln_stats,
+                                            const float* ln_colsum, uint16_t* kcache, uint16_t* vcache, const int* step_dev, int M, int H,
+                                            int T_slots, int K, int ldy, int fp16, void* stream) {
+    int rc = init_gemm_bf16_attrs();
+    if (rc) return rc;
+    RGRG_CHECK_ARG(A16 && Wb && Y && ln_stats && ln_colsum && kcache && vcache && step_dev && H > 0);
+    GemmLnFold f{};
+    f.ln_stats = ln_stats; f.ln_colsum = ln_colsum;
+    f.kv_k = kcache; f.kv_v = vcache; f.kv_step = step_dev; f.kv_H = H; f.kv_T = T_slots;
+    return launch_gemm_bf16w_ex(nullptr, A16, Wb, shift, nullptr, Y, nullptr, M, 3 * H * 64, K, ldy, RGRG_ACT_NONE, as_stream(stream), fp16, &f);
 }
 
 extern "C" int rgrg_debug_linear_bf16_ln_kp(const uint16_t* A16, const uint16_t* Wb, const float* shift, const float* R, float* Y,
diff --git a/rgrg_amd/csrc/internal.h b/rgrg_amd/csrc/internal.h
--- a/rgrg_amd/csrc/internal.h
+++ b/rgrg_amd/csrc/internal.h
@@ -20,6 +20,9 @@
     float* cand_val = nullptr;
     int* cand_idx = nullptr;
     int kp = 0;
+    void *kv_k = nullptr, *kv_v = nullptr;
+    const int* kv_step = nullptr;
+    int kv_H = 0, kv_T = 0;
 };
 int init_gemm_bf16_attrs();
 bool gemm_bf16_cand_epilogue_ok(int M, int N, int K);
diff --git a/rgrg_amd/csrc/runtime.hip b/rgrg_amd/csrc/runtime.hip
--- a/rgrg_amd/csrc/runtime.hip
+++ b/rgrg_amd/csrc/runtime.hip
@@ -14,7 +14,7 @@
 }
 
 extern "C" const char* rgrg_last_error(void) { return rgrg::g_err; }
-extern "C" int rgrg_abi_version(void) { return 24; }
+extern "C" int rgrg_abi_version(void) { return 25; }
 extern "C" int rgrg_device_arch(int dev, char* buf, int buflen) {
     RGRG_CHECK_ARG(buf && buflen > 1);
     hipDeviceProp_t prop;
```

Result: faster. 88.18 images/sec (median of 6 runs) (+2.3%).
